# Zain-Jiang/Speech-Editing-Toolkit

Hardware: AMD Instinct MI355X
Metric: diffusion mel-frames/s (100-step p_sample, B=32/GPU, T=800) (higher is better)
Workload: dtype f32 (operands carried as 2 fp16 pieces, 3 MFMA products per term, fp32 accumulate: fp32-equivalent, see roofline.note)

## Files before the change

### speech-editing-toolkit_amd/csrc/common.h

```cpp
#pragma once
#include <hip/hip_runtime.h>
#include <stdint.h>
#include <stdio.h>

#include <atomic>

#include "set_amd.h"

typedef float f32x16 __attribute__((ext_vector_type(16)));
typedef float f32x4 __attribute__((ext_vector_type(4)));

extern thread_local char g_set_err[512];

static inline int set_fail(int code, const char *what, const char *detail) {
    snprintf(g_set_err, sizeof(g_set_err), "%s: %s", what, detail ? detail : "");
    return code;
}
static inline int set_check_launch(const char *what) {
    hipError_t e = hipGetLastError();
    if (e != hipSuccess) return set_fail(SET_E_LAUNCH, what, hipGetErrorString(e));
    return SET_OK;
}
#define SET_REQUIRE(cond, what)                                        \
    do {                                                               \
        if (!(cond)) return set_fail(SET_E_INVALID, what, #cond);      \
    } while (0)
#define SET_HIP(call, what)                                                        \
    do {                                                                           \
        hipError_t e__ = (call);                                                   \
        if (e__ != hipSuccess) return set_fail(SET_E_LAUNCH, what, hipGetErrorString(e__)); \
    } while (0)

struct SetDeviceOnce {
    std::atomic<uint64_t> done{0};
    template <typename F> int run(F &&f) {
        int dev = -1;
        const uint64_t bit = hipGetDevice(&dev) == hipSuccess && dev >= 0 && dev < 64 ? uint64_t(1) << dev : 0;
        if (done.load(std::memory_order_acquire) & bit) return SET_OK;
        const int rc = f();
        if (rc == SET_OK) done.fetch_or(bit, std::memory_order_release);
        return rc;
    }
};
template <typename... K>
static inline int set_lds_optin(SetDeviceOnce &once, int bytes, const char *what, K... kernels) {
    return once.run([&] {
        for (const void *k : {reinterpret_cast<const void *>(kernels)...})
            SET_HIP(hipFuncSetAttribute(k, hipFuncAttributeMaxDynamicSharedMemorySize, bytes), what);
        return SET_OK;
    });
}
static inline hipError_t set_cu_count(int *n_cu) {
    static std::atomic<int> cached[64];
    int dev = 0;
    hipError_t e = hipGetDevice(&dev);
    if (e != hipSuccess) return e;
    const bool slot = dev >= 0 && dev < 64;
    int n = slot ? cached[dev].load(std::memory_order_relaxed) : 0;
    if (n == 0) {
        e = hipDeviceGetAttribute(&n, hipDeviceAttributeMultiprocessorCount, dev);
        if (e != hipSuccess) return e;
        if (slot) cached[dev].store(n, std::memory_order_relaxed);
    }
    *n_cu = n;
    return hipSuccess;
}

const uint64_t *set_seed_delta_ptr();
static __global__ void __launch_bounds__(256) set_zero_words_kernel(unsigned *p, int64_t words) {
    const int64_t i = (int64_t)blockIdx.x * 256 + threadIdx.x;
    if (i < words) p[i] = 0u;
}
static inline bool set_aligned16(const void *a, const void *b, const void *c) {
    return ((reinterpret_cast<uintptr_t>(a) | reinterpret_cast<uintptr_t>(b) | reinterpret_cast<uintptr_t>(c)) & 15) == 0;
}
static inline hipError_t set_zero_async(void *p, size_t bytes, hipStream_t s) {
    const int64_t words = (int64_t)((bytes + 3) / 4);
    hipLaunchKernelGGL(set_zero_words_kernel, dim3((unsigned)((words + 255) / 256)), dim3(256), 0, s, reinterpret_cast<unsigned *>(p), words);
    return hipGetLastError();
}
static inline unsigned set_blocks(int64_t n, int per_block) { return (unsigned)((n + per_block - 1) / per_block); }

__device__ __forceinline__ float dev_softplus(float x) { return x > 20.0f ? x : log1pf(expf(x)); }
__device__ __forceinline__ float dev_sigmoid(float x) { return 1.0f / (1.0f + expf(-x)); }

__device__ __forceinline__ float dev_act(float v, int act, float p) {
    switch (act) {
        case SET_ACT_RELU: return v > 0.0f ? v : 0.0f;
        case SET_ACT_GELU: return 0.5f * v * (1.0f + erff(v * 0.70710678118654752440f));
        case SET_ACT_TANH: return tanhf(v);
        case SET_ACT_SOFTPLUS: return dev_softplus(v);
        case SET_ACT_MISH: return v * tanhf(dev_softplus(v));
        case SET_ACT_LRELU: return v > 0.0f ? v : v * p;
        default: return v;
    }
}
__device__ __forceinline__ float dev_pro(float v, int pro, float p) {
    switch (pro) {
        case SET_PRO_LRELU: return v > 0.0f ? v : v * p;
        case SET_PRO_DIV: return v / p;
        default: return v;
    }
}

__device__ __forceinline__ int mfma32_row(int reg, int lane) { return (reg & 3) + 8 * (reg >> 2) + 4 * (lane >> 5); }
__device__ __forceinline__ f32x16 mfma32(float a, float b, f32x16 c) {
    return __builtin_amdgcn_mfma_f32_32x32x2f32(a, b, c, 0, 0, 0);
}

typedef __amdgpu_buffer_rsrc_t rsrc_t;
__device__ __forceinline__ rsrc_t make_rsrc(const void *p) {
    return __builtin_amdgcn_make_buffer_rsrc(const_cast<void *>(p), (short)0, (int)0x7fffffff, (int)0x00020000);
}
constexpr unsigned BUF_OOB = 0x80000000u;
__device__ __forceinline__ float buf_load(rsrc_t r, unsigned voff, unsigned soff) {
    return __builtin_bit_cast(float, __builtin_amdgcn_raw_buffer_load_b32(r, (int)voff, (int)soff, 0));
}
__device__ __forceinline__ f32x4 buf_load4(rsrc_t r, unsigned voff, unsigned soff) {
    typedef unsigned u32x4 __attribute__((ext_vector_type(4)));
    return __builtin_bit_cast(f32x4, __builtin_amdgcn_raw_buffer_load_b128(r, (int)voff, (int)soff, 0));
}
__device__ __forceinline__ void buf_store4(f32x4 v, rsrc_t r, unsigned voff, unsigned soff) {
    typedef unsigned u32x4 __attribute__((ext_vector_type(4)));
    __builtin_amdgcn_raw_buffer_store_b128(__builtin_bit_cast(u32x4, v), r, (int)voff, (int)soff, 0);
}
__device__ __forceinline__ void buf_store(float v, rsrc_t r, unsigned voff, unsigned soff) {
    __builtin_amdgcn_raw_buffer_store_b32(__builtin_bit_cast(unsigned, v), r, (int)voff, (int)soff, 0);
}
__device__ __forceinline__ f32x4 buf_load4_stream(rsrc_t r, unsigned voff, unsigned soff) {
    typedef unsigned u32x4 __attribute__((ext_vector_type(4)));
    return __builtin_bit_cast(f32x4, __builtin_amdgcn_raw_buffer_load_b128(r, (int)voff, (int)soff, 2));
}
__device__ __forceinline__ void buf_store4_stream(f32x4 v, rsrc_t r, unsigned voff, unsigned soff) {
    typedef unsigned u32x4 __attribute__((ext_vector_type(4)));
    __builtin_amdgcn_raw_buffer_store_b128(__builtin_bit_cast(u32x4, v), r, (int)voff, (int)soff, 16);
}
__device__ __forceinline__ void buf_atomic_add(float v, rsrc_t r, unsigned voff, unsigned soff) {
    (void)__builtin_amdgcn_raw_ptr_buffer_atomic_fadd_f32(v, r, (int)voff, (int)soff, 0);
}
__device__ __forceinline__ void buf_store_agent(float v, rsrc_t r, unsigned voff, unsigned soff) {
    __builtin_amdgcn_raw_buffer_store_b32(__builtin_bit_cast(unsigned, v), r, (int)voff, (int)soff, 16);
}

__device__ __forceinline__ int ld_agent(const int *p) { return __hip_atomic_load(p, __ATOMIC_RELAXED, __HIP_MEMORY_SCOPE_AGENT); }
constexpr unsigned STACK_SPIN_LIMIT = 1u << 22;
constexpr unsigned SPLIT_SPIN_LIMIT = 1u << 20;

__device__ __forceinline__ void split2_f16(float a, float b, unsigned &p0, unsigned &p1) {
    typedef _Float16 h2_t __attribute__((ext_vector_type(2)));
    typedef float f2_t __attribute__((ext_vector_type(2)));
    const f2_t v = {a, b};
    const h2_t h0 = __builtin_convertvector(v, h2_t);
    const h2_t h1 = __builtin_convertvector(v - __builtin_convertvector(h0, f2_t), h2_t);
    p0 = __builtin_bit_cast(unsigned, h0);
    p1 = __builtin_bit_cast(unsigned, h1);
}

template <int RB> struct AVec;
template <> struct AVec<1> { typedef float type; };
template <> struct AVec<2> { typedef float type __attribute__((ext_vector_type(2))); };
template <> struct AVec<4> { typedef float type __attribute__((ext_vector_type(4))); };

template <int RB>
__device__ __forceinline__ float avec_get(const typename AVec<RB>::type &v, int r) {
    if constexpr (RB == 1) return v; else return v[r];
}

template <int RB, int NCB, int GS>
struct KOps {
    typename AVec<RB>::type A[GS];
    float B[GS][NCB];
};

template <int RB, int NCB, int GS, typename Adv>
__device__ __forceinline__ void gemm_groups(f32x16 (&acc)[RB][NCB], const typename AVec<RB>::type *&wp, const float *&bp,
                                            int rstep, int ng, Adv advance) {
    KOps<RB, NCB, GS> P, Q;
    auto load_step = [&](KOps<RB, NCB, GS> &o, int u) {
        o.A[u] = wp[u * 64];
#pragma unroll
        for (int cb = 0; cb < NCB; ++cb) o.B[u][cb] = bp[u * rstep + 32 * cb];
    };
    auto mma_step = [&](const KOps<RB, NCB, GS> &o, int u) {
        __builtin_amdgcn_s_setprio(1);
#pragma unroll
        for (int r = 0; r < RB; ++r)
#pragma unroll
            for (int cb = 0; cb < NCB; ++cb) acc[r][cb] = mfma32(avec_get<RB>(o.A[u], r), o.B[u][cb], acc[r][cb]);
        __builtin_amdgcn_s_setprio(0);
    };
#pragma unroll
    for (int u = 0; u < GS; ++u) load_step(P, u);
    for (int g = 0; g < ng; g += 2) {
        advance(g);
#pragma unroll
        for (int u = 0; u < GS; ++u) {
            load_step(Q, u);
            __builtin_amdgcn_sched_barrier(0);
            mma_step(P, u);
            __builtin_amdgcn_sched_barrier(0);
        }
        if (g + 2 < ng) advance(g + 1);
#pragma unroll
        for (int u = 0; u < GS; ++u) {
            load_step(P, u);
            __builtin_amdgcn_sched_barrier(0);
            mma_step(Q, u);
            __builtin_amdgcn_sched_barrier(0);
        }
    }
}
```

### speech-editing-toolkit_amd/csrc/diffnet.hip

```cpp
#include <stdlib.h>

#include "common.h"
#include "boundary_x2.h"

namespace {

constexpr int DC = 256;
constexpr int NT = 64;
constexpr int KS1 = 3 * DC / 2;
constexpr int KS2 = DC / 2;

__device__ __forceinline__ int urow16(int r) { return (r & 3) + 8 * (r >> 2); }

__device__ __forceinline__ int layer_row(int w, int rb, int i) {
    return (rb < 2 ? 64 * w + 32 * rb : DC + 64 * w + 32 * (rb - 2)) + i;
}

__device__ __forceinline__ float fast_sigmoid(float x) { return __builtin_amdgcn_rcpf(1.0f + __expf(-x)); }
__device__ __forceinline__ float fast_tanh(float x) { return 1.0f - 2.0f * __builtin_amdgcn_rcpf(1.0f + __expf(2.0f * x)); }

struct LayerTile {
    const float *xin;
    float *xout;
    float *skp;
    const float *cpb;
    const float *dstep;
    int64_t d_cs;
    const float *w1p, *b_dil, *w2p, *b_out;
    int T, t0, dil, first;
    uint64_t *dbg;
    int o, nvalid, halo_l, halo_r;
    unsigned x_bs4, cp_bs4;
    float *sy, *sz;
};

__device__ __forceinline__ int wn_pair_q(int p, int d) { return 2 * d * (p / d) + (p % d); }

__device__ __forceinline__ unsigned wn_voff(const LayerTile &a, int q, unsigned slab4) {
    const bool side = q >= a.o;
    return 4u * (unsigned)(a.t0 + q - (side ? a.T : 0)) + (side ? slab4 : 0u);
}

template <int NCB, int GS, bool AGENT = false>
__device__ __forceinline__ void layer_tile(const LayerTile &a, float *smem) {
    constexpr int NTt = 32 * NCB;
    const int tid = threadIdx.x;
    const int lane = tid & 63;
    const int w = __builtin_amdgcn_readfirstlane(tid >> 6);
    const int half = lane >> 5, l31 = lane & 31;
    const int t0 = a.t0;
    const int dil = a.dil;
    const int XW = NTt + 2 * dil;
    const int T = a.T;
    const float *xin = a.xin;
    uint64_t *dbg = a.dbg;
#define PHASE_STAMP(i) \
    if (dbg && tid == 0) dbg[i] = __builtin_amdgcn_s_memtime();
    PHASE_STAMP(0)

    unsigned lo[NCB];
    bool tv[NCB];
#pragma unroll
    for (int cb = 0; cb < NCB; ++cb) {
        lo[cb] = 4u * (unsigned)(4 * half * T + min(t0 + 32 * cb + l31, T - 1));
        tv[cb] = t0 + 32 * cb + l31 < T;
    }
    const unsigned lb = 16u * (unsigned)half;
    const unsigned T4 = 4u * (unsigned)T;
    const rsrc_t rxin = make_rsrc(xin), rskp = make_rsrc(a.skp), rxout = make_rsrc(a.xout), rcp = make_rsrc(a.cpb),
                 rbd = make_rsrc(a.b_dil), rbo = make_rsrc(a.b_out);

    f32x16 acc[4][NCB];
#pragma unroll
    for (int rb = 0; rb < 4; ++rb)
#pragma unroll
        for (int r = 0; r < 16; ++r) {
            const unsigned ur = (unsigned)layer_row(w, rb, urow16(r));
            const float bias = buf_load(rbd, lb, 4u * ur);
#pragma unroll
            for (int cb = 0; cb < NCB; ++cb) acc[rb][cb][r] = bias + buf_load(rcp, lo[cb], ur * T4);
        }
    {
        const int tA = t0 - dil + lane;
        const int tB = t0 - dil + 64 + lane;
        const bool vA = tA >= 0 && tA < T;
        const bool vB = tB >= 0 && tB < T;
        const unsigned cA = 4u * (unsigned)min(max(tA, 0), T - 1), cB = 4u * (unsigned)min(max(tB, 0), T - 1);
        const bool laneA = lane < XW;
        const bool laneB = 64 + lane < XW;
        for (int r0 = 0; r0 < 64; r0 += 16) {
            float xa[16], xb[16], dd[16];
#pragma unroll
            for (int u = 0; u < 16; ++u) {
                const int c = 64 * w + r0 + u;
                xa[u] = buf_load(rxin, cA, (unsigned)c * T4);
                if constexpr (NCB == 2) xb[u] = buf_load(rxin, cB, (unsigned)c * T4);
                dd[u] = a.dstep[(int64_t)c * a.d_cs];
            }
#pragma unroll
            for (int u = 0; u < 16; ++u) {
                const int c = 64 * w + r0 + u;
                if (laneA) smem[c * XW + lane] = vA ? xa[u] + dd[u] : 0.0f;
                if constexpr (NCB == 2) {
                    if (laneB) smem[c * XW + 64 + lane] = vB ? xb[u] + dd[u] : 0.0f;
                }
            }
        }
    }
    __syncthreads();
    PHASE_STAMP(1)

    {
        const f32x4 *wp = reinterpret_cast<const f32x4 *>(a.w1p) + (int64_t)w * KS1 * 64 + lane;
        const float *bp = smem + half * XW + l31;
        const int rstep = 2 * XW;
        constexpr int GPT = 128 / GS;
        gemm_groups<4, NCB, GS>(acc, wp, bp, rstep, KS1 / GS, [&](int g) {
            wp += GS * 64;
            bp += GS * rstep;
            if ((g % GPT) == GPT - 1) bp += dil - 128 * rstep;
        });
    }
    PHASE_STAMP(2)

#pragma unroll
    for (int rb = 0; rb < 2; ++rb)
#pragma unroll
        for (int r = 0; r < 16; ++r)
#pragma unroll
            for (int cb = 0; cb < NCB; ++cb) {
                const float z = fast_sigmoid(acc[rb][cb][r]) * fast_tanh(acc[rb + 2][cb][r]);
                acc[rb][cb][r] = tv[cb] ? z : 0.0f;
            }
    PHASE_STAMP(3)
    __syncthreads();
#pragma unroll
    for (int rb = 0; rb < 2; ++rb)
#pragma unroll
        for (int cb = 0; cb < NCB; ++cb)
#pragma unroll
            for (int r = 0; r < 16; ++r) {
                const int c = 64 * w + 32 * rb + mfma32_row(r, lane);
                smem[c * NTt + cb * 32 + l31] = acc[rb][cb][r];
            }
    __builtin_amdgcn_sched_barrier(0);
    const bool first = a.first != 0;
#pragma unroll
    for (int rb = 0; rb < 4; ++rb) {
#pragma unroll
        for (int r = 0; r < 16; ++r) {
            const unsigned ur = (unsigned)layer_row(w, rb, urow16(r));
            const float bias = buf_load(rbo, lb, 4u * ur);
#pragma unroll
            for (int cb = 0; cb < NCB; ++cb) {
                const float sv = rb < 2 ? buf_load(rxin, lo[cb], ur * T4) : buf_load(rskp, lo[cb], (ur - DC) * T4);
                acc[rb][cb][r] = (rb >= 2 && first) ? bias : bias + sv;
            }
        }
        if (rb == 1) __builtin_amdgcn_sched_barrier(0);
    }
    __syncthreads();
    PHASE_STAMP(4)

    {
        const f32x4 *wp = reinterpret_cast<const f32x4 *>(a.w2p) + (int64_t)w * KS2 * 64 + lane;
        const float *bp = smem + half * NTt + l31;
        constexpr int rstep = 2 * NTt;
        gemm_groups<4, NCB, GS>(acc, wp, bp, rstep, KS2 / GS, [&](int) {
            wp += GS * 64;
            bp += GS * rstep;
        });
    }
    PHASE_STAMP(5)

#pragma unroll
    for (int cb = 0; cb < NCB; ++cb) {
        if (tv[cb]) {
#pragma unroll
            for (int rb = 0; rb < 4; ++rb)
#pragma unroll
                for (int r = 0; r < 16; ++r) {
                    const unsigned ur = (unsigned)layer_row(w, rb, urow16(r));
                    const float v = acc[rb][cb][r] * (rb < 2 ? 0.70710678118654752440f : 1.0f);
                    const unsigned so = rb < 2 ? ur * T4 : (ur - DC) * T4;
                    if constexpr (AGENT) buf_store_agent(v, rb < 2 ? rxout : rskp, lo[cb], so);
                    else buf_store(v, rb < 2 ? rxout : rskp, lo[cb], so);
                }
        }
    }
    PHASE_STAMP(6)
#undef PHASE_STAMP
}

__global__ void __launch_bounds__(256, 2) diffnet_layer_kernel(SetDiffnetLayerArgs a) {
    extern __shared__ __attribute__((aligned(16))) float smem[];
    const int b = blockIdx.y;
    LayerTile lt;
    lt.xin = a.x_in + (int64_t)b * DC * a.T;
    lt.xout = a.x_out + (int64_t)b * DC * a.T;
    lt.skp = a.skip + (int64_t)b * DC * a.T;
    lt.cpb = a.condproj + (int64_t)b * a.cp_bs;
    lt.dstep = a.dstep + (int64_t)b * a.d_bs;
    lt.d_cs = a.d_cs;
    lt.w1p = a.w1p; lt.b_dil = a.b_dil; lt.w2p = a.w2p; lt.b_out = a.b_out;
    lt.T = a.T; lt.t0 = blockIdx.x * NT; lt.dil = a.dil; lt.first = a.first;
    lt.dbg = a.dbg_clock ? a.dbg_clock + ((int64_t)blockIdx.y * gridDim.x + blockIdx.x) * 8 : nullptr;
    layer_tile<2, 4>(lt, smem);
}

constexpr int WN_NT = 64;
constexpr int WN_MAXD = 8;
constexpr int WN_XW = WN_NT + 2 * WN_MAXD;
constexpr int WN_KS = DC / 2;
constexpr int WN_GS = 2;

__device__ __forceinline__ void wino_init(const LayerTile &a, f32x16 (&m)[2][4]) {
    const int lane = threadIdx.x & 63;
    const int w = __builtin_amdgcn_readfirstlane(threadIdx.x >> 6);
    const int half = lane >> 5, l31 = lane & 31;
    const int T = a.T;
    const int qe0 = wn_pair_q(l31, a.dil);
    const int qe = min(qe0, a.nvalid - 1), qo = min(qe0 + a.dil, a.nvalid - 1);
    const unsigned rowh = 16u * (unsigned)half * (unsigned)T;
    const unsigned loe = rowh + wn_voff(a, qe, a.cp_bs4), loo = rowh + wn_voff(a, qo, a.cp_bs4);
    const unsigned lb = 16u * (unsigned)half;
    const rsrc_t rcp = make_rsrc(a.cpb), rb = make_rsrc(a.b_dil);
#pragma unroll
    for (int rf = 0; rf < 2; ++rf) {
        m[rf][1] = (f32x16){0};
        m[rf][2] = (f32x16){0};
#pragma unroll
        for (int r = 0; r < 16; ++r) {
            const unsigned ur = (unsigned)(rf * DC + 32 * w + urow16(r));
            const float bias = buf_load(rb, lb, 4u * ur);
            m[rf][0][r] = bias + buf_load(rcp, loe, 4u * ur * (unsigned)T);
            m[rf][3][r] = -(bias + buf_load(rcp, loo, 4u * ur * (unsigned)T));
        }
    }
}

constexpr int WN_ZS_OFF = DC * WN_XW;

template <bool UNIT_DIL>
__device__ __forceinline__ void wino_main(const LayerTile &a, f32x16 (&m)[2][4], float *smem, uint64_t *ph, int *s_task,
                                          int claimed) {
    typedef float f32x2 __attribute__((ext_vector_type(2)));
    const int tid = threadIdx.x;
#ifdef SET_WINO_PHASES
#define WPH(k) { const uint64_t t_ = __builtin_amdgcn_s_memtime(); ph[k] += t_ - ph[9]; ph[9] = t_; }
#else
#define WPH(k)
#endif
    const int lane = tid & 63;
    const int w = __builtin_amdgcn_readfirstlane(tid >> 6);
    const int half = lane >> 5, l31 = lane & 31;
    const int t0 = a.t0, T = a.T;
    const unsigned T4 = 4u * (unsigned)T;
    float *zs = smem + WN_ZS_OFF;
    constexpr int XW = UNIT_DIL ? WN_NT + 4 : WN_XW;
    const int d = UNIT_DIL ? 1 : a.dil, qe = UNIT_DIL ? 2 * l31 : wn_pair_q(l31, d);
    const bool tve = qe < a.nvalid, tvo = qe + d < a.nvalid;
    const rsrc_t rxin = make_rsrc(a.xin), rskp = make_rsrc(a.skp), rxout = make_rsrc(a.xout);

    {
        const int qA = lane;
        const int qB = lane < d ? lane - d : 64 + lane - d;
        const bool isB = lane < 2 * d;
        const bool vA = qA < a.nvalid;
        const bool vB = isB && (qB < 0 ? (d == 1 ? a.halo_l != 0 : a.t0 + qB >= 0)
                                       : (d == 1 ? a.halo_r != 0 : a.t0 + qB < a.T));
        const unsigned cA = wn_voff(a, min(qA, a.nvalid - 1), a.x_bs4);
        const unsigned cB = vB ? wn_voff(a, qB, a.x_bs4) : cA;
        const int colA = qA + d + (qA >= a.o ? 2 : 0), colB = qB + d + (qB >= a.o ? 2 : 0);
        const bool gap = a.o <= 64;
        for (int r0 = 0; r0 < 32; r0 += 16) {
            float xa[16], xb[16], dd[16];
#pragma unroll
            for (int u = 0; u < 16; ++u) {
                const int c = 32 * w + r0 + u;
                xa[u] = buf_load(rxin, cA, (unsigned)c * T4);
                xb[u] = buf_load(rxin, cB, (unsigned)c * T4);
                dd[u] = a.dstep[(int64_t)c * a.d_cs];
            }
#pragma unroll
            for (int u = 0; u < 16; ++u) {
                const int c = 32 * w + r0 + u;
                smem[c * XW + colA] = vA ? xa[u] + dd[u] : 0.0f;
                if (isB) smem[c * XW + colB] = vB ? xb[u] + dd[u] : 0.0f;
                if (gap && lane >= 32 && lane < 34) smem[c * XW + a.o + lane - 31] = 0.0f;
            }
        }
    }
    __syncthreads();
    WPH(1)

    {
        const rsrc_t rw = make_rsrc(a.w1p);
        const unsigned wv = 32u * (unsigned)lane;
        unsigned ws = (unsigned)w * (WN_KS * 64 * 8 * 4);
        const float *bpf = smem + half * XW + qe + (qe >= a.o ? 2 : 0);
        const f32x2 *bp = reinterpret_cast<const f32x2 *>(bpf);
        struct Ops { f32x4 A[WN_GS][2]; f32x2 D[WN_GS][2]; };
        Ops P, Q;
        auto load_step = [&](Ops &o, int u) {
            o.A[u][0] = buf_load4(rw, wv, ws + (unsigned)u * 2048u);
            o.A[u][1] = buf_load4(rw, wv + 16u, ws + (unsigned)u * 2048u);
            if (UNIT_DIL) {
                o.D[u][0] = bp[u * XW];
                o.D[u][1] = bp[u * XW + 1];
            } else {
                const float *q = bpf + u * 2 * XW;
                o.D[u][0] = (f32x2){q[0], q[d]};
                o.D[u][1] = (f32x2){q[2 * d], q[3 * d]};
            }
        };
        auto mma_step = [&](const Ops &o, int u) {
            const float d0 = o.D[u][0][0], d1 = o.D[u][0][1], d2 = o.D[u][1][0], d3 = o.D[u][1][1];
            const float D1 = d0 - d2, D2 = d1 + d2, D3 = d2 - d1, D4 = d1 - d3;
            __builtin_amdgcn_s_setprio(1);
            m[0][0] = mfma32(o.A[u][0][0], D1, m[0][0]);
            m[0][1] = mfma32(o.A[u][0][1], D2, m[0][1]);
            m[0][2] = mfma32(o.A[u][0][2], D3, m[0][2]);
            m[0][3] = mfma32(o.A[u][0][3], D4, m[0][3]);
            m[1][0] = mfma32(o.A[u][1][0], D1, m[1][0]);
            m[1][1] = mfma32(o.A[u][1][1], D2, m[1][1]);
            m[1][2] = mfma32(o.A[u][1][2], D3, m[1][2]);
            m[1][3] = mfma32(o.A[u][1][3], D4, m[1][3]);
            __builtin_amdgcn_s_setprio(0);
        };
        constexpr int NG = WN_KS / WN_GS;
#pragma unroll
        for (int u = 0; u < WN_GS; ++u) load_step(P, u);
        for (int g = 0; g < NG; g += 2) {
            ws += WN_GS * 2048u;
            bp += WN_GS * XW;
            bpf += WN_GS * 2 * XW;
#pragma unroll
            for (int u = 0; u < WN_GS; ++u) {
                load_step(Q, u);
                __builtin_amdgcn_sched_barrier(0);
                mma_step(P, u);
                __builtin_amdgcn_sched_barrier(0);
            }
            if (g + 2 < NG) { ws += WN_GS * 2048u; bp += WN_GS * XW; bpf += WN_GS * 2 * XW; }
#pragma unroll
            for (int u = 0; u < WN_GS; ++u) {
                load_step(P, u);
                __builtin_amdgcn_sched_barrier(0);
                mma_step(Q, u);
                __builtin_amdgcn_sched_barrier(0);
            }
        }
    }

    WPH(2)
    {
        const bool save = a.sy != nullptr;
        const rsrc_t rsy = make_rsrc(save ? a.sy : a.xin), rsz = make_rsrc(save ? a.sz : a.xin);
        const unsigned rowh_s = 16u * (unsigned)half * (unsigned)T;
        const unsigned se = rowh_s + wn_voff(a, min(qe, a.nvalid - 1), 0u), so_ = rowh_s + wn_voff(a, min(qe + d, a.nvalid - 1), 0u);
#pragma unroll
        for (int r = 0; r < 16; ++r) {
            const float g0 = m[0][0][r] + m[0][1][r] + m[0][2][r], g1 = m[0][1][r] - m[0][2][r] - m[0][3][r];
            const float f0 = m[1][0][r] + m[1][1][r] + m[1][2][r], f1 = m[1][1][r] - m[1][2][r] - m[1][3][r];
            const float z0 = tve ? fast_sigmoid(g0) * fast_tanh(f0) : 0.0f;
            const float z1 = tvo ? fast_sigmoid(g1) * fast_tanh(f1) : 0.0f;
            const int c = 32 * w + mfma32_row(r, lane);
            if (UNIT_DIL) {
                *reinterpret_cast<f32x2 *>(zs + c * WN_NT + qe) = (f32x2){z0, z1};
            } else {
                zs[c * WN_NT + qe] = z0;
                zs[c * WN_NT + qe + d] = z1;
            }
            if (save) {
                const unsigned ur = (unsigned)(32 * w + urow16(r));
                if (tve) {
                    buf_store(g0, rsy, se, ur * T4);
                    buf_store(f0, rsy, se, (ur + DC) * T4);
                    buf_store(z0, rsz, se, ur * T4);
                }
                if (tvo) {
                    buf_store(g1, rsy, so_, ur * T4);
                    buf_store(f1, rsy, so_, (ur + DC) * T4);
                    buf_store(z1, rsz, so_, ur * T4);
                }
            }
        }
    }
    __builtin_amdgcn_sched_barrier(0);

    const unsigned rowh = 16u * (unsigned)half * (unsigned)T;
    const unsigned lo0 = rowh + wn_voff(a, min(l31, a.nvalid - 1), a.x_bs4), lo1 = rowh + wn_voff(a, min(32 + l31, a.nvalid - 1), a.x_bs4);
    const bool tv0 = l31 < a.nvalid, tv1 = 32 + l31 < a.nvalid;
    const bool first = a.first != 0;
    f32x16 prev[2][2];
#pragma unroll
    for (int rb = 0; rb < 2; ++rb)
#pragma unroll
        for (int r = 0; r < 16; ++r) {
            const unsigned ur = (unsigned)(32 * w + urow16(r));
            prev[rb][0][r] = buf_load(rb == 0 ? rxin : rskp, lo0, ur * T4);
            prev[rb][1][r] = buf_load(rb == 0 ? rxin : rskp, lo1, ur * T4);
        }
    __builtin_amdgcn_sched_barrier(0);

    f32x16 acc[2][2];
    {
        const rsrc_t rbo = make_rsrc(a.b_out);
#pragma unroll
        for (int rb = 0; rb < 2; ++rb)
#pragma unroll
            for (int r = 0; r < 16; ++r) {
                const float bias = buf_load(rbo, 16u * (unsigned)half, 4u * (unsigned)(rb * DC + 32 * w + urow16(r)));
                acc[rb][0][r] = bias;
                acc[rb][1][r] = bias;
            }
    }
    if (tid == 0) s_task[0] = claimed;
    __syncthreads();
    WPH(3)
    {
        const AVec<2>::type *wp = reinterpret_cast<const AVec<2>::type *>(a.w2p) + (int64_t)w * WN_KS * 64 + lane;
        const float *bp = zs + half * WN_NT + l31;
        constexpr int rstep = 2 * WN_NT;
        gemm_groups<2, 2, 8>(acc, wp, bp, rstep, WN_KS / 8, [&](int) {
            wp += 8 * 64;
            bp += 8 * rstep;
        });
    }
    WPH(4)
#pragma unroll
    for (int cb = 0; cb < 2; ++cb) {
        if (cb == 0 ? tv0 : tv1) {
            const unsigned so = cb == 0 ? lo0 : lo1;
#pragma unroll
            for (int rb = 0; rb < 2; ++rb)
#pragma unroll
                for (int r = 0; r < 16; ++r) {
                    const unsigned ur = (unsigned)(32 * w + urow16(r));
                    const float v = (rb == 1 && first) ? acc[rb][cb][r] : acc[rb][cb][r] + prev[rb][cb][r];
                    buf_store_agent(v * (rb == 0 ? 0.70710678118654752440f : 1.0f), rb == 0 ? rxout : rskp, so, ur * T4);
                }
        }
    }
    WPH(5)
#undef WPH
}

template <int NCB, int GS, int WPS>
__global__ void __launch_bounds__(256, WPS) diffnet_stack_kernel(SetDiffnetStackArgs a, int tiles_per_utt, int ntiles,
                                                                int ntasks, int task_slot) {
    constexpr int NTt = 32 * NCB;
    extern __shared__ __attribute__((aligned(16))) float smem[];
    int *s_task = reinterpret_cast<int *>(smem + task_slot);
    int *counter = a.sync_ws, *abort_flag = a.sync_ws + 1, *done = a.sync_ws + 4;
    const int tid = threadIdx.x;
    uint64_t wait_ticks = 0, fence_ticks = 0;
    for (;;) {
        __syncthreads();
        if (tid == 0) {
            const uint64_t tw0 = __builtin_amdgcn_s_memtime();
            int n = atomicAdd(counter, 1);
            if (n < ntasks && n >= ntiles) {
                const int l = n / ntiles, i = n - l * ntiles, j = i % tiles_per_utt;
                unsigned spins = 0;
                const int *f0 = done + i, *fl = done + (j > 0 ? i - 1 : i), *fr = done + (j < tiles_per_utt - 1 ? i + 1 : i);
                for (;;) {
                    const int v0 = ld_agent(f0), v1 = ld_agent(fl), v2 = ld_agent(fr);
                    if (min(v0, min(v1, v2)) >= l) break;
                    __builtin_amdgcn_s_sleep(8);
                    if (++spins > STACK_SPIN_LIMIT || ld_agent(abort_flag) != 0) {
                        __hip_atomic_store(abort_flag, 1, __ATOMIC_RELAXED, __HIP_MEMORY_SCOPE_AGENT);
                        if (a.err_flag) __hip_atomic_store(a.err_flag, 1, __ATOMIC_RELAXED, __HIP_MEMORY_SCOPE_AGENT);
                        n = ntasks;
                        break;
                    }
                }
                __builtin_amdgcn_fence(__ATOMIC_ACQUIRE, "agent");
            }
            wait_ticks += __builtin_amdgcn_s_memtime() - tw0;
            *s_task = n;
        }
        __syncthreads();
        const int n = __builtin_amdgcn_readfirstlane(*s_task);
        if (n >= ntasks) {
            if (tid == 0) {
                atomicAdd(a.sync_ws + 2, (int)(wait_ticks >> 10));
                atomicAdd(a.sync_ws + 3, (int)(fence_ticks >> 10));
            }
            break;
        }
        const int l = n / ntiles, i = n - l * ntiles;
        const int b = i / tiles_per_utt, j = i - b * tiles_per_utt;
        LayerTile lt;
        const float *xi = (l & 1) ? a.xb : a.xa;
        float *xo = (l & 1) ? a.xa : a.xb;
        lt.xin = xi + (int64_t)b * DC * a.T;
        lt.xout = xo + (int64_t)b * DC * a.T;
        lt.skp = a.skip + (int64_t)b * DC * a.T;
        lt.cpb = a.condproj + (int64_t)l * a.cp_ls + (int64_t)b * a.cp_bs;
        lt.dstep = a.dstep + (int64_t)l * a.d_ls + (int64_t)b * a.d_bs;
        lt.d_cs = a.d_cs;
        lt.w1p = a.w1p_all + (int64_t)l * (512 * 768);
        lt.w2p = a.w2p_all + (int64_t)l * (512 * 256);
        lt.b_dil = a.b_dil_all + (int64_t)l * 512;
        lt.b_out = a.b_out_all + (int64_t)l * 512;
        lt.T = a.T; lt.t0 = j * NTt; lt.dil = 1 << (l % a.dilation_cycle_length); lt.first = (l == 0);
        lt.dbg = nullptr;
        layer_tile<NCB, GS, true>(lt, smem);
        asm volatile("s_waitcnt vmcnt(0)" ::: "memory");
        __syncthreads();
        if (tid == 0) {
            const uint64_t tf0 = __builtin_amdgcn_s_memtime();
            __hip_atomic_store(done + i, l + 1, __ATOMIC_RELAXED, __HIP_MEMORY_SCOPE_AGENT);
            fence_ticks += __builtin_amdgcn_s_memtime() - tf0;
        }
    }
}

constexpr int SP_XW = 32 + 2 * WN_MAXD;
constexpr int SP_LDS_FLOATS = DC * SP_XW + 64 * 32 + 4;

__device__ __forceinline__ void split_preload(float (&A)[64], const float *wp) {
#pragma unroll
    for (int u = 0; u < 64; ++u) A[u] = wp[u * 64];
}

template <int KS>
__device__ __forceinline__ void split_gemm(f32x16 &acc, const float *wp, float (&Ap)[64], const float *bq, int rstep,
                                           int tap_jump) {
    static_assert(KS % 128 == 0, "two 64-k-step sets per iteration");
    float Aq[64], Bv[8];
#pragma unroll
    for (int u = 0; u < 4; ++u) {
        Bv[u] = *bq;
        bq += rstep;
    }
    for (int g = 0; g < KS / 64; g += 2) {
        const float *wq = wp + (int64_t)(g + 1) * 64 * 64;
#pragma unroll
        for (int u = 0; u < 64; ++u) {
            Aq[u] = wq[u * 64];
            Bv[(u + 4) & 7] = *bq;
            bq += rstep;
            __builtin_amdgcn_sched_barrier(0);
            acc = mfma32(Ap[u], Bv[u & 7], acc);
            __builtin_amdgcn_sched_barrier(0);
        }
        const float *wn = wp + (int64_t)(g + 2 < KS / 64 ? g + 2 : g) * 64 * 64;
#pragma unroll
        for (int u = 0; u < 64; ++u) {
            Ap[u] = wn[u * 64];
            Bv[(u + 4) & 7] = *bq;
            bq += rstep;
            if (u == 59) bq += tap_jump;
            __builtin_amdgcn_sched_barrier(0);
            acc = mfma32(Aq[u], Bv[u & 7], acc);
            __builtin_amdgcn_sched_barrier(0);
        }
    }
}

__device__ uint64_t *g_split_phase_buf = nullptr;

__device__ __forceinline__ bool split_wait(const int *f0, const int *f1, const int *f2, int want, int *abort_flag,
                                           int *err_flag) {
    unsigned spins = 0;
    for (;;) {
        const int v0 = ld_agent(f0), v1 = ld_agent(f1), v2 = ld_agent(f2);
        if (min(v0, min(v1, v2)) >= want) break;
        __builtin_amdgcn_s_sleep(1);
        if (++spins > SPLIT_SPIN_LIMIT || ld_agent(abort_flag) != 0) {
            __hip_atomic_store(abort_flag, 1, __ATOMIC_RELAXED, __HIP_MEMORY_SCOPE_AGENT);
            if (err_flag) __hip_atomic_store(err_flag, 1, __ATOMIC_RELAXED, __HIP_MEMORY_SCOPE_AGENT);
            return false;
        }
    }
    __builtin_amdgcn_fence(__ATOMIC_ACQUIRE, "agent");
    return true;
}

__global__ void __launch_bounds__(256, 2) diffnet_stack_split_kernel(SetDiffnetStackArgs a, int tiles_per_utt, int ntiles,
                                                                    int fault_tile) {
    extern __shared__ __attribute__((aligned(16))) float smem[];
    float *gs = smem + DC * SP_XW;
    int *s_ok = reinterpret_cast<int *>(gs + 64 * 32);
    int *abort_flag = a.sync_ws + 1, *ready = a.sync_ws + 4, *zcnt = a.sync_ws + 4 + ntiles;
    const int tid = threadIdx.x, lane = tid & 63, half = lane >> 5, l31 = lane & 31;
    const int j = __builtin_amdgcn_readfirstlane(tid >> 6);
    const int i = blockIdx.x >> 2, h = blockIdx.x & 3;
    const int b = i / tiles_per_utt, jt = i - b * tiles_per_utt;
    const int T = a.T, t0 = jt * 32;
    const int il = jt > 0 ? i - 1 : i, ir = jt < tiles_per_utt - 1 ? i + 1 : i;
    const unsigned T4 = 4u * (unsigned)T;
    const unsigned lo = 4u * (unsigned)(4 * half * T + min(t0 + l31, T - 1));
    const bool tv = t0 + l31 < T;
    const unsigned lb = 16u * (unsigned)half;
    const rsrc_t rz = make_rsrc(a.z_ws + (int64_t)i * (DC * 32));
    const rsrc_t rskp = make_rsrc(a.skip + (int64_t)b * DC * T);
    const int vr = 4 * h + j;
    uint64_t *dbg = (blockIdx.x == 5 && tid == 0) ? g_split_phase_buf : nullptr;
    uint64_t tprev = dbg ? __builtin_amdgcn_s_memtime() : 0;
#define SP_PHASE(p)                                           \
    if (dbg) {                                                \
        const uint64_t tn = __builtin_amdgcn_s_memtime();     \
        dbg[p] += tn - tprev;                                 \
        tprev = tn;                                           \
    }
    for (int l = 0; l < a.L; ++l) {
        const int dil = 1 << (l % a.dilation_cycle_length), XW = 32 + 2 * dil;
        const rsrc_t rxin = make_rsrc(((l & 1) ? a.xb : a.xa) + (int64_t)b * DC * T);
        const rsrc_t rxout = make_rsrc(((l & 1) ? a.xa : a.xb) + (int64_t)b * DC * T);
        const rsrc_t rcp = make_rsrc(a.condproj + (int64_t)l * a.cp_ls + (int64_t)b * a.cp_bs);
        const rsrc_t rbd = make_rsrc(a.b_dil_all + (int64_t)l * 512), rbo = make_rsrc(a.b_out_all + (int64_t)l * 512);
        const float *dstep = a.dstep + (int64_t)l * a.d_ls + (int64_t)b * a.d_bs;
        f32x16 acc[1][1];
#pragma unroll
        for (int r = 0; r < 16; ++r) {
            const unsigned ur = (unsigned)layer_row(h, j, urow16(r));
            acc[0][0][r] = buf_load(rbd, lb, 4u * ur) + buf_load(rcp, lo, ur * T4);
        }
        float Ap[64];
        const float *wp1 = a.w1s_all + (int64_t)l * (512 * 768) + (int64_t)vr * KS1 * 64 + lane;
        split_preload(Ap, wp1);
        if (tid == 0) *s_ok = (l == 0 || split_wait(ready + i, ready + il, ready + ir, 4 * l, abort_flag, a.err_flag)) ? 1 : 0;
        __syncthreads();
        if (__builtin_amdgcn_readfirstlane(*s_ok) == 0) return;
        SP_PHASE(0)
        {
            const int tA = t0 - dil + lane;
            const bool vA = tA >= 0 && tA < T, laneA = lane < XW;
            const unsigned cA = 4u * (unsigned)min(max(tA, 0), T - 1);
            float xa[64];
            const float dv = dstep[(int64_t)(64 * j + lane) * a.d_cs];
#pragma unroll
            for (int u = 0; u < 64; ++u) xa[u] = buf_load(rxin, cA, (unsigned)(64 * j + u) * T4);
#pragma unroll
            for (int u = 0; u < 64; ++u) {
                const float dd = __builtin_bit_cast(float, __builtin_amdgcn_readlane(__builtin_bit_cast(int, dv), u));
                if (laneA) smem[(64 * j + u) * XW + lane] = vA ? xa[u] + dd : 0.0f;
            }
        }
        __syncthreads();
        SP_PHASE(1)
        split_gemm<KS1>(acc[0][0], wp1, Ap, smem + half * XW + l31, 2 * XW, dil - 128 * 2 * XW);
        SP_PHASE(2)
        if (j >= 2) {
#pragma unroll
            for (int r = 0; r < 16; ++r) gs[(32 * (j - 2) + mfma32_row(r, lane)) * 32 + l31] = fast_tanh(acc[0][0][r]);
        }
        __syncthreads();
        if (j < 2) {
#pragma unroll
            for (int r = 0; r < 16; ++r) {
                const float z = fast_sigmoid(acc[0][0][r]) * gs[(32 * j + mfma32_row(r, lane)) * 32 + l31];
                buf_store_agent(tv ? z : 0.0f, rz, 4u * (unsigned)(4 * half * 32 + l31),
                                4u * 32u * (unsigned)(64 * h + 32 * j + urow16(r)));
            }
        }
        asm volatile("s_waitcnt vmcnt(0)" ::: "memory");
        __syncthreads();
        if (tid == 0) __hip_atomic_fetch_add(zcnt + i, 1, __ATOMIC_RELAXED, __HIP_MEMORY_SCOPE_AGENT);
        SP_PHASE(3)
        {
            const rsrc_t rsv = make_rsrc(j < 2 ? ((l & 1) ? a.xb : a.xa) + (int64_t)b * DC * T : a.skip + (int64_t)b * DC * T);
            float bias[16], sv[16];
#pragma unroll
            for (int r = 0; r < 16; ++r) {
                bias[r] = buf_load(rbo, lb, 4u * (unsigned)layer_row(h, j, urow16(r)));
                sv[r] = buf_load(rsv, lo, (unsigned)(64 * h + 32 * (j & 1) + urow16(r)) * T4);
            }
            if (j >= 2 && l == 0) {
#pragma unroll
                for (int r = 0; r < 16; ++r) acc[0][0][r] = bias[r];
            } else {
#pragma unroll
                for (int r = 0; r < 16; ++r) acc[0][0][r] = bias[r] + sv[r];
            }
        }
        const float *wp2 = a.w2s_all + (int64_t)l * (512 * 256) + (int64_t)vr * KS2 * 64 + lane;
        split_preload(Ap, wp2);
        if (tid == 0) *s_ok = split_wait(zcnt + i, zcnt + i, zcnt + i, 4 * (l + 1), abort_flag, a.err_flag) ? 1 : 0;
        __syncthreads();
        if (__builtin_amdgcn_readfirstlane(*s_ok) == 0) return;
        SP_PHASE(4)
        {
            f32x4 zv[8];
#pragma unroll
            for (int k = 0; k < 8; ++k) zv[k] = buf_load4(rz, 16u * (unsigned)tid, 4096u * (unsigned)k);
#pragma unroll
            for (int k = 0; k < 8; ++k) *reinterpret_cast<f32x4 *>(smem + 4 * tid + 1024 * k) = zv[k];
        }
        __syncthreads();
        SP_PHASE(5)
        split_gemm<KS2>(acc[0][0], wp2, Ap, smem + half * 32 + l31, 64, 0);
        SP_PHASE(6)
        if (tv && j < 2) {
#pragma unroll
            for (int r = 0; r < 16; ++r)
                buf_store_agent(acc[0][0][r] * 0.70710678118654752440f, rxout, lo, (unsigned)layer_row(h, j, urow16(r)) * T4);
        } else if (tv) {
#pragma unroll
            for (int r = 0; r < 16; ++r)
                buf_store(acc[0][0][r], rskp, lo, (unsigned)(layer_row(h, j, urow16(r)) - DC) * T4);
        }
        asm volatile("s_waitcnt vmcnt(0)" ::: "memory");
        __syncthreads();
        if (tid == 0 && !(l == 0 && i == fault_tile && h == 0))
            __hip_atomic_fetch_add(ready + i, 1, __ATOMIC_RELAXED, __HIP_MEMORY_SCOPE_AGENT);
        SP_PHASE(7)
    }
#undef SP_PHASE
}

template <bool UNIT_DIL>
__global__ void __launch_bounds__(512, 2) diffnet_stack_wino_kernel(SetDiffnetStackArgs a, int tiles_per_utt, int ntiles,
                                                                    int ntasks, int concat, int fault_tile) {
    extern __shared__ __attribute__((aligned(16))) float smem[];
    int *s_task = reinterpret_cast<int *>(smem + WN_ZS_OFF + DC * WN_NT);
    int *counter = a.sync_ws, *abort_flag = a.sync_ws + 1, *done = a.sync_ws + 4;
    const int tid = threadIdx.x;
    uint64_t wait_ticks = 0, fence_ticks = 0;
    if (tid == 0) s_task[0] = atomicAdd(counter, 1);
    __syncthreads();
    int n = __builtin_amdgcn_readfirstlane(s_task[0]);
    int l = 0, i = 0, j = 0;
    LayerTile lt;
    auto decode = [&](int task) {
        l = task / ntiles;
        i = task - l * ntiles;
        int b;
        if (concat) {
            const int64_t f0 = (int64_t)WN_NT * i, F = (int64_t)a.B * a.T;
            b = (int)(f0 / a.T);
            j = i;
            lt.t0 = (int)(f0 - (int64_t)b * a.T);
            lt.o = (a.T - lt.t0 <= WN_NT && b + 1 < a.B) ? a.T - lt.t0 : (1 << 20);
            lt.nvalid = (int)min((int64_t)WN_NT, (b + 1 < a.B ? F : (int64_t)(b + 1) * a.T) - f0);
            lt.halo_l = lt.t0 > 0;
            lt.halo_r = f0 + WN_NT < F;
        } else {
            b = i / tiles_per_utt;
            j = i - b * tiles_per_utt;
            lt.t0 = j * WN_NT;
            lt.o = 1 << 20;
            lt.nvalid = min(WN_NT, a.T - lt.t0);
            lt.halo_l = lt.t0 > 0;
            lt.halo_r = lt.t0 + WN_NT < a.T;
        }
        lt.x_bs4 = 4u * (unsigned)DC * (unsigned)a.T;
        lt.cp_bs4 = 4u * (unsigned)a.cp_bs;
        const int64_t slab = (int64_t)a.B * DC * a.T;
        const float *xi = a.x_all ? a.x_all + l * slab : ((l & 1) ? a.xb : a.xa);
        float *xo = a.x_all ? a.x_all + (l + 1) * slab : ((l & 1) ? a.xa : a.xb);
        lt.xin = xi + (int64_t)b * DC * a.T;
        lt.xout = xo + (int64_t)b * DC * a.T;
        lt.skp = a.skip + (int64_t)b * DC * a.T;
        lt.sy = a.save_y ? a.save_y + 2 * l * slab + (int64_t)b * 2 * DC * a.T : nullptr;
        lt.sz = a.save_z ? a.save_z + l * slab + (int64_t)b * DC * a.T : nullptr;
        lt.cpb = a.condproj + (int64_t)l * a.cp_ls + (int64_t)b * a.cp_bs;
        lt.dstep = a.dstep + (int64_t)l * a.d_ls + (int64_t)b * a.d_bs;
        lt.d_cs = a.d_cs;
        lt.w1p = a.w1w_all + (int64_t)l * (512 * 256 * 4);
        lt.w2p = a.w2w_all + (int64_t)l * (512 * 256);
        lt.b_dil = a.b_dil_all + (int64_t)l * 512;
        lt.b_out = a.b_out_all + (int64_t)l * 512;
        lt.T = a.T; lt.dil = UNIT_DIL ? 1 : 1 << (l % a.dilation_cycle_length); lt.first = (l == 0);
        lt.dbg = nullptr;
    };
#ifdef SET_WINO_PHASES
    uint64_t ph[10] = {0, 0, 0, 0, 0, 0, 0, 0, 0, 0};
    ph[9] = __builtin_amdgcn_s_memtime();
#else
    uint64_t *ph = nullptr;
#endif
    int i_done = -1, l_done = 0;
    auto publish = [&]() {
        asm volatile("s_waitcnt vmcnt(0)" ::: "memory");
#ifdef SET_WINO_PHASES
        { const uint64_t t_ = __builtin_amdgcn_s_memtime(); ph[0] += t_ - ph[9]; ph[9] = t_; }
#endif
        __syncthreads();
#ifdef SET_WINO_PHASES
        { const uint64_t t_ = __builtin_amdgcn_s_memtime(); ph[6] += t_ - ph[9]; ph[9] = t_; }
#endif
        if (tid == 0 && i_done >= 0) {
            const uint64_t tf0 = __builtin_amdgcn_s_memtime();
            if (!(l_done == 0 && i_done == fault_tile))
                __hip_atomic_store(done + i_done, l_done + 1, __ATOMIC_RELAXED, __HIP_MEMORY_SCOPE_AGENT);
            fence_ticks += __builtin_amdgcn_s_memtime() - tf0;
        }
    };
    while (n < ntasks) {
        decode(n);
        f32x16 m[2][4];
        wino_init(lt, m);
        __builtin_amdgcn_sched_barrier(0);
        publish();
        int claimed = 0;
        if (tid == 0) {
            int ok_all = 1;
            if (l > 0) {
                const uint64_t tw0 = __builtin_amdgcn_s_memtime();
                unsigned spins = 0;
                const int *f0 = done + i, *fl = done + (j > 0 ? i - 1 : i), *fr = done + (j < tiles_per_utt - 1 ? i + 1 : i);
                for (;;) {
                    const int v0 = ld_agent(f0), v1 = ld_agent(fl), v2 = ld_agent(fr);
                    if (min(v0, min(v1, v2)) >= l) break;
                    __builtin_amdgcn_s_sleep(8);
                    if (++spins > STACK_SPIN_LIMIT || ld_agent(abort_flag) != 0) {
                        __hip_atomic_store(abort_flag, 1, __ATOMIC_RELAXED, __HIP_MEMORY_SCOPE_AGENT);
                        if (a.err_flag) __hip_atomic_store(a.err_flag, 1, __ATOMIC_RELAXED, __HIP_MEMORY_SCOPE_AGENT);
                        ok_all = 0;
                        break;
                    }
                }
                __builtin_amdgcn_fence(__ATOMIC_ACQUIRE, "agent");
                wait_ticks += __builtin_amdgcn_s_memtime() - tw0;
            }
            s_task[1] = ok_all;
            claimed = atomicAdd(counter, 1);
        }
        __syncthreads();
        if (__builtin_amdgcn_readfirstlane(s_task[1]) == 0) {
            i_done = -1;
            break;
        }
#ifdef SET_WINO_PHASES
        { const uint64_t t_ = __builtin_amdgcn_s_memtime(); ph[8] += t_ - ph[9]; ph[9] = t_; }
#endif
        wino_main<UNIT_DIL>(lt, m, smem, ph, s_task, claimed);
        i_done = i;
        l_done = l;
        n = __builtin_amdgcn_readfirstlane(s_task[0]);
    }
    publish();
#ifdef SET_WINO_PHASES
    if (tid == 0)
        for (int k = 0; k < 9; ++k) atomicAdd(a.sync_ws + 4 + ntiles + k, (int)(ph[k] >> 10));
#endif
    if (tid == 0) {
        atomicAdd(a.sync_ws + 2, (int)(wait_ticks >> 10));
        atomicAdd(a.sync_ws + 3, (int)(fence_ticks >> 10));
    }
}

__global__ void __launch_bounds__(256) pack_diffnet_layer_kernel(const float *w_dil, const float *w_out, float *w1p,
                                                                 float *w2p, int64_t wd_ls = 0, int64_t wo_ls = 0) {
    const int64_t idx = (int64_t)blockIdx.x * 256 + threadIdx.x;
    const int64_t n1 = (int64_t)4 * KS1 * 64 * 4, n2 = (int64_t)4 * KS2 * 64 * 4;
    w_dil += (int64_t)blockIdx.y * wd_ls;
    w_out += (int64_t)blockIdx.y * wo_ls;
    w1p += (int64_t)blockIdx.y * n1;
    w2p += (int64_t)blockIdx.y * n2;
    if (idx < n1) {
        const int rb = (int)(idx & 3), lane = (int)((idx >> 2) & 63);
        const int ks = (int)((idx >> 8) % KS1), w = (int)((idx >> 8) / KS1);
        const int tap = ks >> 7, cp = ks & 127;
        const int row = layer_row(w, rb, lane & 31), c = 2 * cp + (lane >> 5);
        w1p[idx] = w_dil[((int64_t)row * DC + c) * 3 + tap];
    } else if (idx < n1 + n2) {
        const int64_t j = idx - n1;
        const int rb = (int)(j & 3), lane = (int)((j >> 2) & 63);
        const int ks = (int)((j >> 8) % KS2), w = (int)((j >> 8) / KS2);
        const int row = layer_row(w, rb, lane & 31), c = 2 * ks + (lane >> 5);
        w2p[j] = w_out[(int64_t)row * DC + c];
    }
}

__global__ void __launch_bounds__(256) pack_diffnet_wino_kernel(const float *w_dil, const float *w_out, float *w1w,
                                                                float *w2w, int64_t wd_ls = 0, int64_t wo_ls = 0) {
    const int64_t idx = (int64_t)blockIdx.x * 256 + threadIdx.x;
    const int64_t n1 = (int64_t)8 * WN_KS * 64 * 8, n2 = (int64_t)8 * WN_KS * 64 * 2;
    w_dil += (int64_t)blockIdx.y * wd_ls;
    w_out += (int64_t)blockIdx.y * wo_ls;
    w1w += (int64_t)blockIdx.y * n1;
    w2w += (int64_t)blockIdx.y * n2;
    if (idx < n1) {
        const int e = (int)(idx & 7), lane = (int)((idx >> 3) & 63);
        const int ks = (int)((idx >> 9) % WN_KS), w = (int)((idx >> 9) / WN_KS);
        const int rf = e >> 2, p = e & 3;
        const int row = rf * DC + 32 * w + (lane & 31), c = 2 * ks + (lane >> 5);
        const float *g = w_dil + ((int64_t)row * DC + c) * 3;
        const double g0 = g[0], g1 = g[1], g2 = g[2];
        const double v = p == 0 ? g0 : (p == 1 ? 0.5 * (g0 + g1 + g2) : (p == 2 ? 0.5 * (g0 - g1 + g2) : g2));
        w1w[idx] = (float)v;
    } else if (idx < n1 + n2) {
        const int64_t j = idx - n1;
        const int rb = (int)(j & 1), lane = (int)((j >> 1) & 63);
        const int ks = (int)((j >> 7) % WN_KS), w = (int)((j >> 7) / WN_KS);
        const int row = rb * DC + 32 * w + (lane & 31), c = 2 * ks + (lane >> 5);
        w2w[j] = w_out[(int64_t)row * DC + c];
    }
}

}

extern "C" int64_t set_diffnet_w1w_size(void) { return (int64_t)512 * 256 * 4; }
extern "C" int set_pack_diffnet_layer_wino(const float *w_dil, const float *w_out, float *w1w, float *w2w, void *stream) {
    SET_REQUIRE(w_dil && w_out && w1w && w2w, "set_pack_diffnet_layer_wino");
    const int64_t total = set_diffnet_w1w_size() + (int64_t)512 * 256;
    hipLaunchKernelGGL(pack_diffnet_wino_kernel, dim3(set_blocks(total, 256)), dim3(256), 0, (hipStream_t)stream, w_dil,
                       w_out, w1w, w2w);
    return set_check_launch("set_pack_diffnet_layer_wino");
}

extern "C" int64_t set_diffnet_w1p_size(void) { return (int64_t)512 * 768; }
extern "C" int64_t set_diffnet_w2p_size(void) { return (int64_t)512 * 256; }

extern "C" int set_pack_diffnet_layers(const float *w_dil, const float *w_out, int64_t wd_ls, int64_t wo_ls, float *w1p, float *w2p,
                                       float *w1w, float *w2w, int32_t L, void *stream) {
    SET_REQUIRE(w_dil && w_out && w1p && w2p && L > 0 && L <= 65535 && (w1w == nullptr) == (w2w == nullptr), "set_pack_diffnet_layers");
    SET_REQUIRE((int64_t)8 * WN_KS * 64 * 8 == set_diffnet_w1w_size() && (int64_t)8 * WN_KS * 64 * 2 == (int64_t)512 * 256 &&
                    (int64_t)4 * KS1 * 64 * 4 == set_diffnet_w1p_size() && (int64_t)4 * KS2 * 64 * 4 == set_diffnet_w2p_size(),
                "set_pack_diffnet_layers(image sizes)");
    const int64_t total = set_diffnet_w1p_size() + set_diffnet_w2p_size();
    hipLaunchKernelGGL(pack_diffnet_layer_kernel, dim3(set_blocks(total, 256), L), dim3(256), 0, (hipStream_t)stream, w_dil, w_out, w1p,
                       w2p, wd_ls, wo_ls);
    int rc = set_check_launch("set_pack_diffnet_layers");
    if (rc != SET_OK || w1w == nullptr) return rc;
    const int64_t totw = set_diffnet_w1w_size() + (int64_t)512 * 256;
    hipLaunchKernelGGL(pack_diffnet_wino_kernel, dim3(set_blocks(totw, 256), L), dim3(256), 0, (hipStream_t)stream, w_dil, w_out, w1w,
                       w2w, wd_ls, wo_ls);
    return set_check_launch("set_pack_diffnet_layers(wino)");
}
extern "C" int set_pack_diffnet_layer(const float *w_dil, const float *w_out, float *w1p, float *w2p, void *stream) {
    SET_REQUIRE(w_dil && w_out && w1p && w2p, "set_pack_diffnet_layer");
    const int64_t total = set_diffnet_w1p_size() + set_diffnet_w2p_size();
    hipLaunchKernelGGL(pack_diffnet_layer_kernel, dim3(set_blocks(total, 256)), dim3(256), 0, (hipStream_t)stream,
                       w_dil, w_out, w1p, w2p);
    return set_check_launch("set_pack_diffnet_layer");
}

extern "C" int set_diffnet_layer(const SetDiffnetLayerArgs *args, void *stream) {
    SET_REQUIRE(args != nullptr, "set_diffnet_layer");
    const SetDiffnetLayerArgs &a = *args;
    SET_REQUIRE(a.x_in && a.condproj && a.dstep && a.w1p && a.b_dil && a.w2p && a.b_out && a.x_out && a.skip,
                "set_diffnet_layer");
    SET_REQUIRE(a.B > 0 && a.T > 0 && a.dil >= 1, "set_diffnet_layer");
    SET_REQUIRE(a.x_in != a.x_out, "set_diffnet_layer(x_in must not alias x_out)");
    if (a.dil > 8) return set_fail(SET_E_UNSUPPORTED, "set_diffnet_layer", "dilation > 8 (LDS tile > 80 KiB)");
    const size_t lds = (size_t)DC * (NT + 2 * a.dil) * sizeof(float);
    static SetDeviceOnce lds_once;
    if (int rc = set_lds_optin(lds_once, 96 * 1024, "set_diffnet_layer(attr)", diffnet_layer_kernel)) return rc;
    dim3 grid((a.T + NT - 1) / NT, a.B);
    hipLaunchKernelGGL(diffnet_layer_kernel, grid, dim3(256), lds, (hipStream_t)stream, a);
    return set_check_launch("set_diffnet_layer");
}

extern "C" int set_debug_split_phase_buffer(uint64_t *buf) {
    SET_HIP(hipMemcpyToSymbol(HIP_SYMBOL(g_split_phase_buf), &buf, sizeof(buf)), "set_debug_split_phase_buffer");
    return SET_OK;
}

extern "C" int64_t set_sizeof_diffnet_stack_args(void) { return (int64_t)sizeof(SetDiffnetStackArgs); }

static bool split_f32_pinned() {
    const char *e = getenv("SET_AMD_SPLIT_F32");
    return e && atoi(e) != 0;
}
static int x3_mode_of_images(int images) { return (images & 4) ? 3 : ((images & 8) ? 2 : 0); }

static int stack_variant(int B, int T, int dcl, bool have_wino, bool have_split, int x3_mode, int n_cu) {
    const bool have_x3 = x3_mode == 2 || x3_mode == 3;
    const int64_t tiles64 = (int64_t)B * ((T + 63) / 64);
    const int64_t split_blocks = 4 * (int64_t)B * ((T + 31) / 32);
    const bool split_one_per_cu = have_x3 && !split_f32_pinned();
    const bool split_fits = have_split && dcl <= 4 && split_blocks <= (split_one_per_cu ? 1 : 2) * (int64_t)n_cu;
    const bool split_pays = split_blocks <= (int64_t)(have_x3 ? 1 : 2) * n_cu;
    int split_env = 1;
    if (const char *e = getenv("SET_AMD_SPLIT")) split_env = atoi(e);
    if (split_fits && (split_env == 2 || (split_env == 1 && !getenv("SET_AMD_WINO") && split_pays))) return 3;
    int x3_env = 1;
    if (const char *e = getenv("SET_AMD_X3")) x3_env = atoi(e);
    if (have_x3 && dcl <= 4 && (x3_env == 2 || (x3_env == 1 && !getenv("SET_AMD_WINO") && tiles64 >= 8)))
        return x3_mode == 3 ? 4 : 5;
    int ncb = tiles64 < 3 * n_cu ? 1 : 2;
    if (const char *e = getenv("SET_AMD_STACK_NCB")) ncb = atoi(e) == 2 ? 2 : 1;
    const bool wino_ok = have_wino && (1 << (dcl - 1)) <= WN_MAXD;
    bool wino = wino_ok && 25 * tiles64 >= 17 * n_cu;
    if (const char *e = getenv("SET_AMD_WINO")) wino = wino_ok && (atoi(e) == 2 || (wino && atoi(e) != 0));
    return wino ? 2 : (ncb == 1 ? 1 : 0);
}
extern "C" int set_diffnet_stack_variant(int B, int T, int dilation_cycle_length, int images) {
    int n_cu = 256;
    (void)set_cu_count(&n_cu);
    return stack_variant(B, T, dilation_cycle_length, (images & 1) != 0, (images & 2) != 0, x3_mode_of_images(images), n_cu);
}

int set_launch_diffnet_stack_x3(const SetDiffnetStackArgs &a, int n_cu, int fault_tile, hipStream_t s);
int set_x3_winograd_selected(int x3_mode, int B, int T, int dilation_cycle_length, int n_cu);
extern "C" int set_diffnet_stack_x3_winograd(int B, int T, int dilation_cycle_length, int images) {
    int n_cu = 256;
    (void)set_cu_count(&n_cu);
    const int x3_mode = x3_mode_of_images(images);
    if (stack_variant(B, T, dilation_cycle_length, (images & 1) != 0, (images & 2) != 0, x3_mode, n_cu) != 5) return 0;
    return set_x3_winograd_selected(x3_mode, B, T, dilation_cycle_length, n_cu);
}
int set_launch_diffnet_stack_split_x2(const SetDiffnetStackArgs &a, int fault_tile, hipStream_t s);

extern "C" int set_diffnet_stack(const SetDiffnetStackArgs *args, void *stream) {
    SET_REQUIRE(args != nullptr, "set_diffnet_stack");
    const SetDiffnetStackArgs &a = *args;
    SET_REQUIRE(a.xa && a.xb && a.skip && a.condproj && a.dstep && a.w1p_all && a.w2p_all && a.b_dil_all &&
                    a.b_out_all && a.sync_ws,
                "set_diffnet_stack");
    SET_REQUIRE(a.B > 0 && a.T > 0 && a.L > 0 && a.dilation_cycle_length >= 1 && a.dilation_cycle_length <= 4,
                "set_diffnet_stack");
    hipStream_t s = (hipStream_t)stream;
    static SetDeviceOnce lds_once;
    if (int rc = set_lds_optin(lds_once, 150 * 1024, "set_diffnet_stack(attr)", diffnet_stack_kernel<1, 8, 2>, diffnet_stack_kernel<2, 4, 2>,
                               diffnet_stack_wino_kernel<true>, diffnet_stack_wino_kernel<false>, diffnet_stack_split_kernel))
        return rc;
    int n_cu = 0;
    SET_HIP(set_cu_count(&n_cu), "set_diffnet_stack");
    const bool plain = !a.x_all && !a.save_y && !a.save_z;
    const int variant = stack_variant(a.B, a.T, a.dilation_cycle_length, a.w1w_all && a.w2w_all,
                                      a.w1s_all && a.w2s_all && a.z_ws && plain, (a.wx3_all && plain) ? a.x3_mode : 0, n_cu);
    int fault_tile = -1;
    if (const char *e = getenv("SET_AMD_FAULT_TILE")) fault_tile = atoi(e);
    if (variant >= 4) return set_launch_diffnet_stack_x3(a, n_cu, fault_tile, s);
    if (variant == 3 && a.wx3_all && a.x3_mode == 2 && !split_f32_pinned())
        return set_launch_diffnet_stack_split_x2(a, fault_tile, s);
    if (variant == 3) {
        const int tiles = (a.T + 31) / 32, nt = a.B * tiles;
        SET_HIP(set_zero_async(a.sync_ws, (size_t)(4 + 2 * nt) * sizeof(int32_t), s), "set_diffnet_stack(memset)");
        hipLaunchKernelGGL(diffnet_stack_split_kernel, dim3(4 * nt), dim3(256), (size_t)SP_LDS_FLOATS * sizeof(float), s, a,
                           tiles, nt, fault_tile);
        return set_check_launch("set_diffnet_stack");
    }
    const bool wino = variant == 2;
    const int ncb = variant == 1 ? 1 : 2;
    const int ntt = 32 * ncb;
    int tiles_per_utt = (a.T + ntt - 1) / ntt;
    int ntiles = a.B * tiles_per_utt;
    bool concat = wino && a.dilation_cycle_length == 1 && a.T % 2 == 0 && a.T >= WN_NT &&
                  (int64_t)a.cp_bs * 4 < (1ll << 31) && a.d_bs == 0 && !a.save_y && !a.save_z;
    if (concat) {
        ntiles = (int)(((int64_t)a.B * a.T + WN_NT - 1) / WN_NT);
        tiles_per_utt = ntiles;
    }
    const int64_t ntasks64 = (int64_t)ntiles * a.L;
    SET_REQUIRE(ntasks64 < (1ll << 30), "set_diffnet_stack(task count)");
    const int max_dil = 1 << (a.dilation_cycle_length - 1);
    const int task_slot = DC * (ntt + 2 * max_dil);
    const size_t lds = (size_t)(task_slot + 4) * sizeof(float);
    SET_HIP(set_zero_async(a.sync_ws, (size_t)(4 + ntiles + (wino ? 12 : 0)) * sizeof(int32_t), s),
            "set_diffnet_stack(memset)");
    const int wps = wino ? 1 : 2;
    int grid = wps * n_cu;
    if (grid > ntiles * 4 / 5) grid = ntiles * 4 / 5;
    if (grid < n_cu) grid = n_cu < ntiles ? n_cu : ntiles;
    if (const char *e = getenv("SET_AMD_STACK_GRID")) grid = atoi(e) > 0 ? atoi(e) : grid;
    if ((int64_t)grid > ntasks64) grid = (int)ntasks64;
    if (grid < 1) grid = 1;
    if (wino) {
        if (a.dilation_cycle_length == 1)
            hipLaunchKernelGGL(diffnet_stack_wino_kernel<true>, dim3(grid), dim3(512),
                               (size_t)(WN_ZS_OFF + DC * WN_NT + 4) * sizeof(float), s, a, tiles_per_utt, ntiles,
                               (int)ntasks64, concat ? 1 : 0, fault_tile);
        else
            hipLaunchKernelGGL(diffnet_stack_wino_kernel<false>, dim3(grid), dim3(512),
                               (size_t)(WN_ZS_OFF + DC * WN_NT + 4) * sizeof(float), s, a, tiles_per_utt, ntiles,
                               (int)ntasks64, 0, fault_tile);
    } else if (ncb == 1)
        hipLaunchKernelGGL((diffnet_stack_kernel<1, 8, 2>), dim3(grid), dim3(256), lds, s, a, tiles_per_utt, ntiles,
                           (int)ntasks64, task_slot);
    else
        hipLaunchKernelGGL((diffnet_stack_kernel<2, 4, 2>), dim3(grid), dim3(256), lds, s, a, tiles_per_utt, ntiles,
                           (int)ntasks64, task_slot);
    return set_check_launch("set_diffnet_stack");
}

namespace {
__global__ void __launch_bounds__(256) gate_kernel(const float *y, float *z, int B, int C, int T) {
    const int64_t i = (int64_t)blockIdx.x * 256 + threadIdx.x;
    if (i >= (int64_t)B * C * T) return;
    const int64_t ct = i % ((int64_t)C * T);
    const int64_t b = i / ((int64_t)C * T);
    const float *yb = y + b * 2 * C * T;
    z[i] = dev_sigmoid(yb[ct]) * tanhf(yb[(int64_t)C * T + ct]);
}
__global__ void __launch_bounds__(256) res_skip_kernel(const float *x_in, const float *o, float *x_out, float *skip,
                                                       int B, int C, int T, int first) {
    const int64_t i = (int64_t)blockIdx.x * 256 + threadIdx.x;
    if (i >= (int64_t)B * C * T) return;
    const int64_t ct = i % ((int64_t)C * T);
    const int64_t b = i / ((int64_t)C * T);
    const float *ob = o + b * 2 * C * T;
    x_out[i] = (x_in[i] + ob[ct]) / 1.41421356237309504880f;
    const float s = ob[(int64_t)C * T + ct];
    skip[i] = first ? s : skip[i] + s;
}
__global__ void __launch_bounds__(256) sinusoid_kernel(const float *t, float *out, int dim, int n) {
    const int64_t i = (int64_t)blockIdx.x * 256 + threadIdx.x;
    if (i >= (int64_t)dim * n) return;
    const int j = (int)(i / n), k = (int)(i % n);
    const int half = dim / 2;
    const int jj = j < half ? j : j - half;
    const float e = (float)(9.210340371976184 / (double)(half - 1));
    const float freq = expf((float)jj * -e);
    const float ang = t[k] * freq;
    out[i] = j < half ? sinf(ang) : cosf(ang);
}


__global__ void __launch_bounds__(256) randn_kernel(float *out, int64_t n, uint64_t seed, uint64_t offset, const uint64_t *seed_delta) {
    const int64_t q = (int64_t)blockIdx.x * 256 + threadIdx.x;
    if (q * 4 >= n) return;
    if (seed_delta) seed += *seed_delta;
    float z[4];
    randn4(seed, offset + (uint64_t)q, z);
#pragma unroll
    for (int k = 0; k < 4; ++k)
        if (q * 4 + k < n) out[q * 4 + k] = z[k];
}

__global__ void __launch_bounds__(256) posterior_kernel(const float *x0, const float *x_t, const float *eps,
                                                        const float *coef4, int64_t coef_bs, float *x_prev,
                                                        int64_t per_batch, int64_t n, uint64_t seed,
                                                        uint64_t offset, const uint64_t *seed_delta) {
    const int64_t q = (int64_t)blockIdx.x * 256 + threadIdx.x;
    if (q * 4 >= n) return;
    if (seed_delta) seed += *seed_delta;
    float z[4];
    if (!eps) randn4(seed, offset + (uint64_t)q, z);
#pragma unroll
    for (int k = 0; k < 4; ++k) {
        const int64_t i = q * 4 + k;
        if (i >= n) break;
        const float *cf = coef4 + (i / per_batch) * coef_bs;
        const float mean = cf[0] * x0[i] + cf[1] * x_t[i];
        const float e = eps ? eps[i] : z[k];
        x_prev[i] = mean + cf[3] * expf(0.5f * cf[2]) * e;
    }
}

__global__ void __launch_bounds__(256) q_sample_kernel(const float *x_start, const float *eps, const float *ab2,
                                                       const float *nonpad, float *x_t, int B, int M, int T) {
    const int64_t i = (int64_t)blockIdx.x * 256 + threadIdx.x;
    if (i >= (int64_t)B * M * T) return;
    const int t = (int)(i % T);
    const int b = (int)(i / ((int64_t)M * T));
    float v = ab2[2 * b] * x_start[i] + ab2[2 * b + 1] * eps[i];
    if (nonpad) v *= nonpad[(int64_t)b * T + t];
    x_t[i] = v;
}

__global__ void __launch_bounds__(64) selftest_mfma_kernel(float *max_err) {
    constexpr int K = 8;
    const int lane = threadIdx.x;
    auto Af = [](int i, int k) { return 0.25f * (float)((i * 7 + k * 3) % 11) - 1.0f; };
    auto Bf = [](int k, int j) { return 0.125f * (float)((k * 5 + j * 13) % 17) - 0.75f; };
    f32x16 acc = {0};
    for (int k0 = 0; k0 < K; k0 += 2) {
        const int k = k0 + (lane >> 5);
        acc = mfma32(Af(lane & 31, k), Bf(k, lane & 31), acc);
    }
    float err = 0.0f;
    for (int r = 0; r < 16; ++r) {
        const int row = mfma32_row(r, lane), col = lane & 31;
        float ref = 0.0f;
        for (int k = 0; k < K; ++k) ref = fmaf(Af(row, k), Bf(k, col), ref);
        err = fmaxf(err, fabsf(ref - acc[r]));
    }
    for (int off = 32; off > 0; off >>= 1) err = fmaxf(err, __shfl_xor(err, off));
    if (lane == 0) *max_err = err;
}
}

extern "C" int set_gate(const float *y, float *z, int32_t B, int32_t C, int32_t T, void *stream) {
    SET_REQUIRE(y && z && B > 0 && C > 0 && T > 0, "set_gate");
    hipLaunchKernelGGL(gate_kernel, dim3(set_blocks((int64_t)B * C * T, 256)), dim3(256), 0, (hipStream_t)stream, y, z,
                       B, C, T);
    return set_check_launch("set_gate");
}
extern "C" int set_res_skip(const float *x_in, const float *o, float *x_out, float *skip, int32_t B, int32_t C,
                            int32_t T, int32_t first, void *stream) {
    SET_REQUIRE(x_in && o && x_out && skip && B > 0 && C > 0 && T > 0, "set_res_skip");
    hipLaunchKernelGGL(res_skip_kernel, dim3(set_blocks((int64_t)B * C * T, 256)), dim3(256), 0, (hipStream_t)stream,
                       x_in, o, x_out, skip, B, C, T, first);
    return set_check_launch("set_res_skip");
}
extern "C" int set_sinusoid_embed(const float *t, float *out, int32_t dim, int32_t n, void *stream) {
    SET_REQUIRE(t && out && dim >= 4 && (dim % 2) == 0 && n > 0, "set_sinusoid_embed");
    hipLaunchKernelGGL(sinusoid_kernel, dim3(set_blocks((int64_t)dim * n, 256)), dim3(256), 0, (hipStream_t)stream, t,
                       out, dim, n);
    return set_check_launch("set_sinusoid_embed");
}
static const uint64_t *g_seed_delta = nullptr;
const uint64_t *set_seed_delta_ptr() { return g_seed_delta; }
extern "C" int set_rng_seed_delta(const uint64_t *dev_word) {
    g_seed_delta = dev_word;
    return SET_OK;
}

extern "C" int set_randn(float *out, int64_t n, uint64_t seed, uint64_t offset, void *stream) {
    SET_REQUIRE(out && n > 0, "set_randn");
    hipLaunchKernelGGL(randn_kernel, dim3(set_blocks((n + 3) / 4, 256)), dim3(256), 0, (hipStream_t)stream, out, n,
                       seed, offset, g_seed_delta);
    return set_check_launch("set_randn");
}
extern "C" int set_posterior_step(const float *x0, const float *x_t, const float *eps, const float *coef4,
                                  int64_t coef_bs, float *x_prev, int32_t B, int64_t per_batch, uint64_t seed,
                                  uint64_t offset, void *stream) {
    SET_REQUIRE(x0 && x_t && coef4 && x_prev && B > 0 && per_batch > 0, "set_posterior_step");
    const int64_t n = (int64_t)B * per_batch;
    hipLaunchKernelGGL(posterior_kernel, dim3(set_blocks((n + 3) / 4, 256)), dim3(256), 0, (hipStream_t)stream, x0,
                       x_t, eps, coef4, coef_bs, x_prev, per_batch, n, seed, offset, g_seed_delta);
    return set_check_launch("set_posterior_step");
}
extern "C" int set_q_sample(const float *x_start, const float *eps, const float *ab2, const float *nonpad, float *x_t,
                            int32_t B, int32_t M, int32_t T, void *stream) {
    SET_REQUIRE(x_start && eps && ab2 && x_t && B > 0 && M > 0 && T > 0, "set_q_sample");
    hipLaunchKernelGGL(q_sample_kernel, dim3(set_blocks((int64_t)B * M * T, 256)), dim3(256), 0, (hipStream_t)stream,
                       x_start, eps, ab2, nonpad, x_t, B, M, T);
    return set_check_launch("set_q_sample");
}
extern "C" int set_selftest_mfma(float *max_err_host, void *stream) {
    SET_REQUIRE(max_err_host != nullptr, "set_selftest_mfma");
    float *d = nullptr;
    SET_HIP(hipMalloc(&d, sizeof(float)), "set_selftest_mfma");
    hipLaunchKernelGGL(selftest_mfma_kernel, dim3(1), dim3(64), 0, (hipStream_t)stream, d);
    int rc = set_check_launch("set_selftest_mfma");
    if (rc == SET_OK) {
        hipError_t e = hipMemcpyAsync(max_err_host, d, sizeof(float), hipMemcpyDeviceToHost, (hipStream_t)stream);
        if (e == hipSuccess) e = hipStreamSynchronize((hipStream_t)stream);
        if (e != hipSuccess) rc = set_fail(SET_E_LAUNCH, "set_selftest_mfma", hipGetErrorString(e));
    }
    (void)hipFree(d);
    return rc;
}

struct BoundaryArgs {
    const float *skip;
    float *x;
    const float *eps;
    const float *coef4;
    const float *w_skip_p, *b_skip, *w_outp_p, *b_outp, *w_in_p, *b_in;
    float *xin_next;
    float inv_div;
    float div;
    uint64_t seed, quad_offset;
    int T, M, MP;
};
constexpr int BD_LD = 64;

__global__ void __launch_bounds__(256, 2) diffnet_boundary_kernel(BoundaryArgs a) {
    extern __shared__ __attribute__((aligned(16))) float smem[];
    const int tid = threadIdx.x, lane = tid & 63;
    const int w = __builtin_amdgcn_readfirstlane(tid >> 6);
    const int half = lane >> 5, l31 = lane & 31;
    const int b = blockIdx.y, t0 = blockIdx.x * 64, T = a.T, M = a.M;
    {
        const rsrc_t rs = make_rsrc(a.skip + (int64_t)b * DC * T);
        const unsigned vo = 4u * (unsigned)min(t0 + lane, T - 1);
        const bool tv = t0 + lane < T;
        for (int r0 = 0; r0 < 64; r0 += 16) {
            float v[16];
#pragma unroll
            for (int u = 0; u < 16; ++u) v[u] = buf_load(rs, vo, 4u * (unsigned)(64 * w + r0 + u) * (unsigned)T);
#pragma unroll
            for (int u = 0; u < 16; ++u) smem[(64 * w + r0 + u) * BD_LD + lane] = tv ? v[u] / a.div : 0.0f;
        }
    }
    __syncthreads();
    f32x16 acc[2][1][2];
#pragma unroll
    for (int i = 0; i < 2; ++i) {
        acc[i][0][0] = (f32x16){0};
        acc[i][0][1] = (f32x16){0};
        const float *wp = a.w_skip_p + (int64_t)(2 * w + i) * (DC / 2) * 64 + lane;
        const float *bp = smem + half * BD_LD + l31;
        gemm_groups<1, 2, 8>(acc[i], wp, bp, 2 * BD_LD, (DC / 2) / 8, [&](int) {
            wp += 8 * 64;
            bp += 8 * 2 * BD_LD;
        });
    }
    __syncthreads();
#pragma unroll
    for (int i = 0; i < 2; ++i)
#pragma unroll
        for (int r = 0; r < 16; ++r) {
            const int row = 32 * (2 * w + i) + mfma32_row(r, lane);
            const float bias = a.b_skip[row];
#pragma unroll
            for (int cb = 0; cb < 2; ++cb) smem[row * BD_LD + 32 * cb + l31] = fmaxf(acc[i][0][cb][r] + bias, 0.0f);
        }
    __syncthreads();
    const int rbn = (M + 31) / 32;
    f32x16 xo[1][2];
    xo[0][0] = (f32x16){0};
    xo[0][1] = (f32x16){0};
    if (w < rbn) {
        const float *wp = a.w_outp_p + (int64_t)w * (DC / 2) * 64 + lane;
        const float *bp = smem + half * BD_LD + l31;
        gemm_groups<1, 2, 8>(xo, wp, bp, 2 * BD_LD, (DC / 2) / 8, [&](int) {
            wp += 8 * 64;
            bp += 8 * 2 * BD_LD;
        });
    }
    __syncthreads();
    if (w < rbn) {
#pragma unroll
        for (int r = 0; r < 16; ++r) {
            const int row = 32 * w + mfma32_row(r, lane);
            const float bias = a.b_outp[min(row, M - 1)];
#pragma unroll
            for (int cb = 0; cb < 2; ++cb) smem[row * BD_LD + 32 * cb + l31] = row < M ? xo[0][cb][r] + bias : 0.0f;
        }
    }
    __syncthreads();
    {
        const float c1 = a.coef4[0], c2 = a.coef4[1], sig = a.coef4[3] * expf(0.5f * a.coef4[2]);
        float *xb = a.x + (int64_t)b * M * T;
        const float *eb = a.eps ? a.eps + (int64_t)b * M * T : nullptr;
        for (int qi = tid; qi < a.MP * 16; qi += 256) {
            const int m = qi >> 4, tq = qi & 15, t = t0 + 4 * tq;
            float *cell = smem + m * BD_LD + 4 * tq;
            if (m < M && t < T) {
                const int64_t i = (int64_t)m * T + t;
                const f32x4 xt = *reinterpret_cast<const f32x4 *>(xb + i);
                float z[4];
                if (eb) {
                    const f32x4 e4 = *reinterpret_cast<const f32x4 *>(eb + i);
                    z[0] = e4[0]; z[1] = e4[1]; z[2] = e4[2]; z[3] = e4[3];
                } else {
                    randn4(a.seed, a.quad_offset + (uint64_t)(((int64_t)b * M * T + i) >> 2), z);
                }
                f32x4 o;
#pragma unroll
                for (int k = 0; k < 4; ++k) {
                    const float mean = c1 * cell[k] + c2 * xt[k];
                    o[k] = mean + sig * z[k];
                }
                *reinterpret_cast<f32x4 *>(xb + i) = o;
                *reinterpret_cast<f32x4 *>(cell) = o;
            } else {
                *reinterpret_cast<f32x4 *>(cell) = (f32x4){0.0f, 0.0f, 0.0f, 0.0f};
            }
        }
    }
    if (!a.xin_next) return;
    __syncthreads();
#pragma unroll
    for (int i = 0; i < 2; ++i) {
        acc[i][0][0] = (f32x16){0};
        acc[i][0][1] = (f32x16){0};
        const float *wp = a.w_in_p + (int64_t)(2 * w + i) * (a.MP / 2) * 64 + lane;
        const float *bp = smem + half * BD_LD + l31;
        gemm_groups<1, 2, 4>(acc[i], wp, bp, 2 * BD_LD, (a.MP / 2) / 4, [&](int) {
            wp += 4 * 64;
            bp += 4 * 2 * BD_LD;
        });
    }
    const rsrc_t ro = make_rsrc(a.xin_next + (int64_t)b * DC * T);
    float bin[2][16];
#pragma unroll
    for (int i = 0; i < 2; ++i)
#pragma unroll
        for (int r = 0; r < 16; ++r) bin[i][r] = (a.b_in + 32 * (2 * w + i) + urow16(r))[4 * half];
#pragma unroll
    for (int cb = 0; cb < 2; ++cb) {
        if (t0 + 32 * cb + l31 < T) {
            const unsigned so = 4u * (unsigned)(4 * half * T + t0 + 32 * cb + l31);
#pragma unroll
            for (int i = 0; i < 2; ++i)
#pragma unroll
                for (int r = 0; r < 16; ++r) {
                    const int ur = 32 * (2 * w + i) + urow16(r);
                    buf_store(fmaxf(acc[i][0][cb][r] + bin[i][r], 0.0f), ro, so, 4u * (unsigned)ur * (unsigned)T);
                }
        }
    }
}

struct BoundaryX2Args {
    BoundaryArgs g;
    const unsigned short *w_skip_x2, *w_outp_x2, *w_in_x2;
    int32_t *err_flag;
};

__global__ void __launch_bounds__(256, 2) diffnet_boundary_x2_kernel(BoundaryX2Args ax) {
    const BoundaryArgs &a = ax.g;
    extern __shared__ __attribute__((aligned(16))) unsigned char bl[];
    const int tid = threadIdx.x, lane = tid & 63;
    const int w = __builtin_amdgcn_readfirstlane(tid >> 6);
    const int half = lane >> 5, l31 = lane & 31;
    const int b = blockIdx.y, t0 = blockIdx.x * 64, T = a.T, M = a.M;
    const unsigned lane16 = 16u * (unsigned)lane;
    const unsigned T4 = 4u * (unsigned)T;
    float amax = 0.0f;
    {
        const int f = lane, cg = w;
        const rsrc_t rs = make_rsrc(a.skip + (int64_t)b * DC * T);
        const unsigned vo = 4u * (unsigned)min(t0 + f, T - 1);
        const bool tv = t0 + f < T;
        for (int c0 = 0; c0 < 64; c0 += 16) {
            float v[16];
#pragma unroll
            for (int u = 0; u < 16; ++u) v[u] = buf_load(rs, vo, (unsigned)(64 * cg + c0 + u) * T4);
#pragma unroll
            for (int q8 = 0; q8 < 2; ++q8) {
                bx_u32x4 u0, u1;
#pragma unroll
                for (int e = 0; e < 4; ++e) {
                    unsigned short p0[2], p1[2];
#pragma unroll
                    for (int k = 0; k < 2; ++k) {
                        const float sv = v[8 * q8 + 2 * e + k] / a.div;
                        const float x = tv ? sv : 0.0f;
                        amax = fmaxf(amax, fabsf(x));
                        bx_split(x, p0[k], p1[k]);
                    }
                    u0[e] = (unsigned)p0[0] | ((unsigned)p0[1] << 16);
                    u1[e] = (unsigned)p1[0] | ((unsigned)p1[1] << 16);
                }
                *reinterpret_cast<bx_u32x4 *>(bl + f * BX_XR + (64 * cg + c0 + 8 * q8) * 2) = u0;
                *reinterpret_cast<bx_u32x4 *>(bl + BX_PIECE + f * BX_XR + (64 * cg + c0 + 8 * q8) * 2) = u1;
            }
        }
    }
    __syncthreads();
    auto bfrag256 = [&](int ks, int cb) { return (unsigned)((cb * 32 + l31) * BX_XR + (ks * 16 + half * 8) * 2); };
    {
        const rsrc_t rw = make_rsrc(ax.w_skip_x2);
        const float inv = reinterpret_cast<const float *>(ax.w_skip_x2 + (DC / 32) * (DC / 16) * 1024)[1];
        f32x16 acc[2][2];
#pragma unroll
        for (int i = 0; i < 2; ++i)
#pragma unroll
            for (int cb = 0; cb < 2; ++cb) acc[i][cb] = (f32x16){0};
        bx_gemm<2>(acc, rw, lane16, 2 * w, DC / 16, DC / 16, bl, BX_PIECE, bfrag256);
        __syncthreads();
#pragma unroll
        for (int i = 0; i < 2; ++i)
#pragma unroll
            for (int cb = 0; cb < 2; ++cb)
#pragma unroll
                for (int g = 0; g < 4; ++g) {
                    unsigned short p0[4], p1[4];
#pragma unroll
                    for (int e = 0; e < 4; ++e) {
                        const int row = 32 * (2 * w + i) + 8 * g + 4 * half + e;
                        const float h = fmaxf(acc[i][cb][4 * g + e] * inv + a.b_skip[row], 0.0f);
                        amax = fmaxf(amax, h);
                        bx_split(h, p0[e], p1[e]);
                    }
                    const unsigned off = (unsigned)((cb * 32 + l31) * BX_XR + (32 * (2 * w + i) + 8 * g + 4 * half) * 2);
                    bx_u32x2 u;
                    u[0] = (unsigned)p0[0] | ((unsigned)p0[1] << 16); u[1] = (unsigned)p0[2] | ((unsigned)p0[3] << 16);
                    *reinterpret_cast<bx_u32x2 *>(bl + off) = u;
                    u[0] = (unsigned)p1[0] | ((unsigned)p1[1] << 16); u[1] = (unsigned)p1[2] | ((unsigned)p1[3] << 16);
                    *reinterpret_cast<bx_u32x2 *>(bl + BX_PIECE + off) = u;
                }
    }
    __syncthreads();
    float *xs = reinterpret_cast<float *>(bl);
    {
        const int rbn = (M + 31) / 32;
        f32x16 xo[1][2];
        xo[0][0] = (f32x16){0};
        xo[0][1] = (f32x16){0};
        const float inv = reinterpret_cast<const float *>(ax.w_outp_x2 + ((M + 31) / 32) * (DC / 16) * 1024)[1];
        if (w < rbn) bx_gemm<1>(xo, make_rsrc(ax.w_outp_x2), lane16, w, DC / 16, DC / 16, bl, BX_PIECE, bfrag256);
        __syncthreads();
        if (w < 3) {
#pragma unroll
            for (int r = 0; r < 16; ++r) {
                const int row = 32 * w + mfma32_row(r, lane);
                const float bias = a.b_outp[min(row, M - 1)];
#pragma unroll
                for (int cb = 0; cb < 2; ++cb) xs[row * 64 + 32 * cb + l31] = (w < rbn && row < M) ? xo[0][cb][r] * inv + bias : 0.0f;
            }
        }
    }
    __syncthreads();
    {
        const float c1 = a.coef4[0], c2 = a.coef4[1], sig = a.coef4[3] * expf(0.5f * a.coef4[2]);
        float *xb = a.x + (int64_t)b * M * T;
        const float *eb = a.eps ? a.eps + (int64_t)b * M * T : nullptr;
        for (int qi = tid; qi < 96 * 16; qi += 256) {
            const int m = qi >> 4, tq = qi & 15, t = t0 + 4 * tq;
            float *cell = xs + m * 64 + 4 * tq;
            if (m < M && t < T) {
                const int64_t i = (int64_t)m * T + t;
                const f32x4 xt = *reinterpret_cast<const f32x4 *>(xb + i);
                float z[4];
                if (eb) {
                    const f32x4 e4 = *reinterpret_cast<const f32x4 *>(eb + i);
                    z[0] = e4[0]; z[1] = e4[1]; z[2] = e4[2]; z[3] = e4[3];
                } else {
                    randn4(a.seed, a.quad_offset + (uint64_t)(((int64_t)b * M * T + i) >> 2), z);
                }
                f32x4 o;
#pragma unroll
                for (int k = 0; k < 4; ++k) {
                    const float mean = c1 * cell[k] + c2 * xt[k];
                    o[k] = mean + sig * z[k];
                }
                *reinterpret_cast<f32x4 *>(xb + i) = o;
                *reinterpret_cast<f32x4 *>(cell) = o;
            } else {
                *reinterpret_cast<f32x4 *>(cell) = (f32x4){0.0f, 0.0f, 0.0f, 0.0f};
            }
        }
    }
    if (!a.xin_next) {
        if (!(amax < 32768.0f) && ax.err_flag) __hip_atomic_store(ax.err_flag, 2, __ATOMIC_RELAXED, __HIP_MEMORY_SCOPE_AGENT);
        return;
    }
    __syncthreads();
    unsigned char *xp = bl + BX_PIECE;
    constexpr unsigned XP_PIECE = 64 * BX_PR;
    {
        const int f = lane, cg = w;
#pragma unroll
        for (int q8 = 0; q8 < 3; ++q8) {
            bx_u32x4 u0, u1;
#pragma unroll
            for (int e = 0; e < 4; ++e) {
                unsigned short p0[2], p1[2];
#pragma unroll
                for (int k = 0; k < 2; ++k) {
                    const float x = xs[(24 * cg + 8 * q8 + 2 * e + k) * 64 + f];
                    amax = fmaxf(amax, fabsf(x));
                    bx_split(x, p0[k], p1[k]);
                }
                u0[e] = (unsigned)p0[0] | ((unsigned)p0[1] << 16);
                u1[e] = (unsigned)p1[0] | ((unsigned)p1[1] << 16);
            }
            *reinterpret_cast<bx_u32x4 *>(xp + f * BX_PR + (24 * cg + 8 * q8) * 2) = u0;
            *reinterpret_cast<bx_u32x4 *>(xp + XP_PIECE + f * BX_PR + (24 * cg + 8 * q8) * 2) = u1;
        }
    }
    if (!(amax < 32768.0f) && ax.err_flag) __hip_atomic_store(ax.err_flag, 2, __ATOMIC_RELAXED, __HIP_MEMORY_SCOPE_AGENT);
    __syncthreads();
    {
        const int ngin = ((M + 31) / 32) * 2;
        const float inv = reinterpret_cast<const float *>(ax.w_in_x2 + (DC / 32) * ngin * 1024)[1];
        f32x16 acc[2][2];
#pragma unroll
        for (int i = 0; i < 2; ++i)
#pragma unroll
            for (int cb = 0; cb < 2; ++cb) acc[i][cb] = (f32x16){0};
        bx_gemm<2>(acc, make_rsrc(ax.w_in_x2), lane16, 2 * w, ngin, ngin, xp, XP_PIECE,
                   [&](int ks, int cb) { return (unsigned)((cb * 32 + l31) * BX_PR + (ks * 16 + half * 8) * 2); });
        const rsrc_t ro = make_rsrc(a.xin_next + (int64_t)b * DC * T);
        float bin[2][16];
#pragma unroll
        for (int i = 0; i < 2; ++i)
#pragma unroll
            for (int r = 0; r < 16; ++r) bin[i][r] = (a.b_in + 32 * (2 * w + i) + urow16(r))[4 * half];
#pragma unroll
        for (int cb = 0; cb < 2; ++cb) {
            if (t0 + 32 * cb + l31 < T) {
                const unsigned so = 4u * (unsigned)(4 * half * T + t0 + 32 * cb + l31);
#pragma unroll
                for (int i = 0; i < 2; ++i)
#pragma unroll
                    for (int r = 0; r < 16; ++r) {
                        const int ur = 32 * (2 * w + i) + urow16(r);
                        buf_store(fmaxf(acc[i][cb][r] * inv + bin[i][r], 0.0f), ro, so, 4u * (unsigned)ur * (unsigned)T);
                    }
            }
        }
    }
}

static bool boundary_fusable(const SetDiffLoopArgs &a) {
    if (const char *e = getenv("SET_AMD_FUSED_BOUNDARY"))
        if (atoi(e) == 0) return false;
    return a.T % 4 == 0 && a.M <= 96 && a.M >= 2 && ((a.M + 15) / 16 * 16 / 2) % 8 == 0;
}

static int launch_boundary(const SetDiffLoopArgs &a, int Bg, const float *skip, float *x, const float *eps, int sid,
                           uint64_t quad_offset, float *xin_next, bool x2, hipStream_t s) {
    static SetDeviceOnce lds_once;
    if (int rc = set_lds_optin(lds_once, 80 * 1024, "boundary(attr)", diffnet_boundary_kernel, diffnet_boundary_x2_kernel)) return rc;
    BoundaryArgs g = {};
    g.skip = skip; g.x = x; g.eps = eps; g.coef4 = a.coef4 + 4 * sid;
    g.w_skip_p = a.w_skip_p; g.b_skip = a.b_skip; g.w_outp_p = a.w_outp_p; g.b_outp = a.b_outp;
    g.w_in_p = a.w_in_p; g.b_in = a.b_in; g.xin_next = xin_next;
    g.div = sqrtf((float)a.L); g.seed = a.seed; g.quad_offset = quad_offset;
    g.T = a.T; g.M = a.M; g.MP = (a.M + 15) / 16 * 16;
    if (x2) {
        BoundaryX2Args gx = {};
        gx.g = g;
        gx.w_skip_x2 = reinterpret_cast<const unsigned short *>(a.w_skip_x2);
        gx.w_outp_x2 = reinterpret_cast<const unsigned short *>(a.w_outp_x2);
        gx.w_in_x2 = reinterpret_cast<const unsigned short *>(a.w_in_x2);
        gx.err_flag = a.err_flag;
        hipLaunchKernelGGL(diffnet_boundary_x2_kernel, dim3((a.T + 63) / 64, Bg), dim3(256), (size_t)2 * BX_PIECE, s, gx);
    } else {
        hipLaunchKernelGGL(diffnet_boundary_kernel, dim3((a.T + 63) / 64, Bg), dim3(256), (size_t)DC * BD_LD * sizeof(float), s, g);
    }
    return set_check_launch("set_diffusion_loop(boundary)");
}

static SetConv1dArgs conv1x1_args(const float *in, const float *wp, const float *bias, float *out, int B, int Cin,
                                  int Cout, int T) {
    SetConv1dArgs c = {};
    c.in = in; c.w = wp; c.bias = bias; c.out = out;
    c.in_bs = (int64_t)Cin * T; c.in_cs = T; c.out_bs = (int64_t)Cout * T; c.out_cs = T;
    c.B = B; c.Cin = Cin; c.Cout = Cout; c.K = 1; c.dil = 1; c.pad = 0;
    c.T_in = T; c.T_iter = T; c.T_out = T; c.out_stride = 1; c.out_off = 0;
    c.alpha = 1.0f; c.impl = SET_IMPL_MFMA;
    return c;
}

static hipStream_t g_aux_streams[8] = {nullptr};
static int aux_stream(int i, hipStream_t *out) {
    if (!g_aux_streams[i]) SET_HIP(hipStreamCreateWithFlags(&g_aux_streams[i], hipStreamNonBlocking), "aux stream");
    *out = g_aux_streams[i];
    return SET_OK;
}

static int diffusion_chain(const SetDiffLoopArgs &a, int g, int b0, int Bg, hipStream_t s, hipEvent_t *ev) {
    const int T = a.T, M = a.M, L = a.L;
    const int64_t per_batch = (int64_t)M * T;
    float *x = a.x + (int64_t)b0 * per_batch;
    float *ws_x0 = a.ws_x0 + (int64_t)b0 * DC * T, *ws_x1 = a.ws_x1 + (int64_t)b0 * DC * T;
    float *ws_skip = a.ws_skip + (int64_t)b0 * DC * T, *ws_h = a.ws_h + (int64_t)b0 * DC * T;
    float *ws_x0pred = a.ws_x0pred + (int64_t)b0 * per_batch;
    const float *condproj = a.condproj ? a.condproj + (int64_t)b0 * L * 512 * T : nullptr;
    const int tiles_per_utt = (T + NT - 1) / NT;
    int32_t *sync_ws = a.sync_ws ? a.sync_ws + 16 * (int64_t)g + 2 * (int64_t)b0 * ((T + 31) / 32) : nullptr;
    const uint64_t quads_before = (uint64_t)((int64_t)b0 * per_batch / 4);
    const uint64_t quads_total = (uint64_t)(((int64_t)a.B * per_batch + 3) / 4);
    int rc = SET_OK;
    const bool fused_boundary = boundary_fusable(a);
    const bool bf16_loop = a.img16_all != nullptr;
    int n_cu = 0;
    SET_HIP(set_cu_count(&n_cu), "set_diffusion_loop");
    bool boundary_x2 = false;
    if (a.persistent && !bf16_loop && fused_boundary && a.w_skip_x2 && a.w_outp_x2 && a.w_in_x2 && a.wx3_all && a.x3_mode == 2 &&
        a.M <= 96) {
        const int v = stack_variant(Bg, T, a.dilation_cycle_length, a.w1w_all && a.w2w_all, a.w1s_all && a.w2s_all && a.z_ws,
                                    a.x3_mode, n_cu);
        boundary_x2 = v == 5 || (v == 3 && !split_f32_pinned());
    }
    if (bf16_loop && fused_boundary && a.w_skip_x2 && a.w_outp_x2 && a.w_in_x2 && a.M <= 96) boundary_x2 = true;
    if (const char *e = getenv("SET_AMD_BOUNDARY_X2")) boundary_x2 = boundary_x2 && atoi(e) != 0;
    for (int k = 0; k < a.steps && rc == SET_OK; ++k) {
        const int sid = a.steps - 1 - k;
        if (!fused_boundary || k == 0) {
            SetConv1dArgs cin = conv1x1_args(x, a.w_in_p, a.b_in, ws_x0, Bg, M, DC, T);
            cin.act = SET_ACT_RELU;
            rc = set_conv1d(&cin, s);
            if (rc != SET_OK) break;
        }
        float *cur = ws_x0, *nxt = ws_x1;
        if (ev) (void)hipEventRecord(ev[2 * k], s);
        if (a.persistent && !bf16_loop) {
            SetDiffnetStackArgs sa = {};
            sa.xa = ws_x0; sa.xb = ws_x1; sa.skip = ws_skip;
            sa.condproj = condproj; sa.cp_bs = (int64_t)L * 512 * T; sa.cp_ls = (int64_t)512 * T;
            sa.dstep = a.dstep + sid; sa.d_bs = 0; sa.d_cs = a.steps; sa.d_ls = (int64_t)DC * a.steps;
            sa.w1p_all = a.w1p_all; sa.w2p_all = a.w2p_all; sa.b_dil_all = a.b_dil_all; sa.b_out_all = a.b_out_all;
            sa.w1w_all = a.w1w_all; sa.w2w_all = a.w2w_all;
            sa.w1s_all = a.w1s_all; sa.w2s_all = a.w2s_all; sa.wx3_all = a.wx3_all; sa.x3_mode = a.x3_mode;
            sa.z_ws = a.z_ws ? a.z_ws + (int64_t)b0 * DC * 32 * ((T + 31) / 32) : nullptr;
            sa.err_flag = a.err_flag;
            sa.sync_ws = sync_ws;
            sa.B = Bg; sa.T = T; sa.L = L; sa.dilation_cycle_length = a.dilation_cycle_length;
            rc = set_diffnet_stack(&sa, s);
        }
        int fuse = 1;
        if (bf16_loop && a.bf16_ws && a.dilation_cycle_length <= 2) {
            fuse = set_diffnet_layers_bf16_plan(Bg, T, L, a.dilation_cycle_length);
            if (const char *e = getenv("SET_AMD_BF16_FUSE")) fuse = atoi(e) < 1 ? 1 : (atoi(e) > 16 ? 16 : atoi(e));
            if (fuse > 1 && a.bf16_ws_floats < set_diffnet_layers_bf16_scratch_floats(a.B, T, 0, fuse, a.dilation_cycle_length)) fuse = 1;
        }
        for (int l = 0; l < L && rc == SET_OK && bf16_loop && fuse > 1; l += fuse) {
            SetDiffnetLayersBf16Args fa = {};
            fa.x_in = cur; fa.x_out = nxt; fa.skip = ws_skip;
            fa.cond = a.cond + (int64_t)b0 * 192 * T;
            fa.dstep = a.dstep + sid; fa.d_bs = 0; fa.d_cs = a.steps; fa.d_ls = (int64_t)DC * a.steps;
            fa.img = reinterpret_cast<const uint16_t *>(a.img16_all) + (int64_t)l * set_diffnet_layer_bf16_image_size();
            fa.b_dil = a.b_dil_all + (int64_t)l * 512; fa.b_cond = a.b_cond_all + (int64_t)l * 512; fa.b_out = a.b_out_all + (int64_t)l * 512;
            const int64_t per_utt = set_diffnet_layers_bf16_scratch_floats(1, T, 0, fuse, a.dilation_cycle_length);
            fa.scratch = a.bf16_ws + (int64_t)b0 * per_utt; fa.scratch_floats = (int64_t)Bg * per_utt;
            fa.B = Bg; fa.T = T; fa.l0 = l; fa.nl = L - l < fuse ? L - l : fuse; fa.dilation_cycle_length = a.dilation_cycle_length;
            fa.first = (l == 0);
            rc = set_diffnet_layers_fwd_bf16(&fa, s);
            float *tmp = cur; cur = nxt; nxt = tmp;
        }
        for (int l = 0; l < L && rc == SET_OK && bf16_loop && fuse == 1; ++l) {
            SetDiffnetLayerBf16Args la = {};
            la.x_in = cur; la.x_out = nxt; la.skip = ws_skip;
            la.cond = a.cond + (int64_t)b0 * 192 * T;
            la.dstep = a.dstep + (int64_t)l * DC * a.steps + sid;
            la.d_bs = 0; la.d_cs = a.steps;
            la.img = reinterpret_cast<const uint16_t *>(a.img16_all) + (int64_t)l * set_diffnet_layer_bf16_image_size();
            la.b_dil = a.b_dil_all + (int64_t)l * 512; la.b_cond = a.b_cond_all + (int64_t)l * 512;
            la.b_out = a.b_out_all + (int64_t)l * 512;
            la.B = Bg; la.T = T; la.dil = 1 << (l % a.dilation_cycle_length); la.first = (l == 0);
            rc = set_diffnet_layer_fwd_bf16(&la, s);
            float *tmp = cur; cur = nxt; nxt = tmp;
        }
        for (int l = 0; l < L && rc == SET_OK && !a.persistent && !bf16_loop; ++l) {
            SetDiffnetLayerArgs la = {};
            la.x_in = cur; la.x_out = nxt; la.skip = ws_skip;
            la.condproj = condproj + (int64_t)l * 512 * T;
            la.cp_bs = (int64_t)L * 512 * T;
            la.dstep = a.dstep + (int64_t)l * DC * a.steps + sid;
            la.d_bs = 0; la.d_cs = a.steps;
            la.w1p = a.w1p_all + (int64_t)l * (512 * 768); la.b_dil = a.b_dil_all + (int64_t)l * 512;
            la.w2p = a.w2p_all + (int64_t)l * (512 * 256); la.b_out = a.b_out_all + (int64_t)l * 512;
            la.B = Bg; la.T = T; la.dil = 1 << (l % a.dilation_cycle_length); la.first = (l == 0);
            rc = set_diffnet_layer(&la, s);
            float *tmp = cur; cur = nxt; nxt = tmp;
        }
        if (ev) (void)hipEventRecord(ev[2 * k + 1], s);
        if (rc != SET_OK) break;
        const float *eps = a.noise ? a.noise + (int64_t)k * a.B * per_batch + (int64_t)b0 * per_batch : nullptr;
        if (fused_boundary) {
            rc = launch_boundary(a, Bg, ws_skip, x, eps, sid, (uint64_t)(k + 1) * quads_total + quads_before,
                                 k + 1 < a.steps ? ws_x0 : nullptr, boundary_x2, s);
            continue;
        }
        SetConv1dArgs cs = conv1x1_args(ws_skip, a.w_skip_p, a.b_skip, ws_h, Bg, DC, DC, T);
        cs.pro = SET_PRO_DIV; cs.pro_param = sqrtf((float)L); cs.act = SET_ACT_RELU;
        rc = set_conv1d(&cs, s);
        if (rc != SET_OK) break;
        SetConv1dArgs co = conv1x1_args(ws_h, a.w_outp_p, a.b_outp, ws_x0pred, Bg, DC, M, T);
        rc = set_conv1d(&co, s);
        if (rc != SET_OK) break;
        rc = set_posterior_step(ws_x0pred, x, eps, a.coef4 + 4 * sid, 0, x, Bg, per_batch, a.seed,
                                (uint64_t)(k + 1) * quads_total + quads_before, s);
    }
    return rc;
}

extern "C" int set_diffusion_loop(const SetDiffLoopArgs *args, void *stream) {
    SET_REQUIRE(args != nullptr, "set_diffusion_loop");
    const SetDiffLoopArgs &a = *args;
    SET_REQUIRE(a.B > 0 && a.T > 0 && a.M > 0 && a.L > 0 && a.steps > 0 && a.dilation_cycle_length >= 1,
                "set_diffusion_loop");
    SET_REQUIRE(a.x && a.dstep && a.coef4 && a.w_in_p && a.b_in && a.b_dil_all && a.b_out_all && a.w_skip_p && a.b_skip &&
                    a.w_outp_p && a.b_outp, "set_diffusion_loop");
    if (a.img16_all) {
        SET_REQUIRE(a.cond && a.b_cond_all, "set_diffusion_loop(bf16 loop needs cond and b_cond_all)");
    } else {
        SET_REQUIRE(a.condproj && a.w1p_all && a.w2p_all, "set_diffusion_loop");
        SET_REQUIRE(!a.persistent || a.sync_ws, "set_diffusion_loop(persistent needs sync_ws)");
    }
    SET_REQUIRE(a.ws_x0 && a.ws_x1 && a.ws_skip && a.ws_h && a.ws_x0pred, "set_diffusion_loop");
    hipStream_t s = (hipStream_t)stream;
    const int64_t per_batch = (int64_t)a.M * a.T;
    int G = a.n_groups < 1 ? 1 : (a.n_groups > 8 ? 8 : a.n_groups);
    if (G > a.B) G = a.B;
    if (per_batch % 4 != 0) G = 1;
    const bool timing = a.layer_span_ms != nullptr;
    hipEvent_t *ev = nullptr;
    if (timing) {
        ev = new hipEvent_t[(size_t)2 * a.steps * G];
        for (int i = 0; i < 2 * a.steps * G; ++i) SET_HIP(hipEventCreate(&ev[i]), "set_diffusion_loop(event)");
    }
    hipEvent_t loop_ev[2] = {nullptr, nullptr};
    if (a.loop_ms) {
        SET_HIP(hipEventCreate(&loop_ev[0]), "set_diffusion_loop(event)");
        SET_HIP(hipEventCreate(&loop_ev[1]), "set_diffusion_loop(event)");
        (void)hipEventRecord(loop_ev[0], s);
    }
    int rc = SET_OK;
    if (G == 1) {
        rc = diffusion_chain(a, 0, 0, a.B, s, ev);
    } else {
        hipEvent_t fork = nullptr, join[8] = {nullptr};
        SET_HIP(hipEventCreateWithFlags(&fork, hipEventDisableTiming), "set_diffusion_loop(fork)");
        SET_HIP(hipEventRecord(fork, s), "set_diffusion_loop(fork)");
        for (int g = 0; g < G && rc == SET_OK; ++g) {
            const int b0 = (int)((int64_t)a.B * g / G), b1 = (int)((int64_t)a.B * (g + 1) / G);
            hipStream_t sg;
            rc = aux_stream(g, &sg);
            if (rc != SET_OK) break;
            SET_HIP(hipStreamWaitEvent(sg, fork, 0), "set_diffusion_loop(fork wait)");
            rc = diffusion_chain(a, g, b0, b1 - b0, sg, ev ? ev + (size_t)2 * a.steps * g : nullptr);
            SET_HIP(hipEventCreateWithFlags(&join[g], hipEventDisableTiming), "set_diffusion_loop(join)");
            SET_HIP(hipEventRecord(join[g], sg), "set_diffusion_loop(join)");
            SET_HIP(hipStreamWaitEvent(s, join[g], 0), "set_diffusion_loop(join wait)");
        }
        (void)hipEventDestroy(fork);
        for (int g = 0; g < G; ++g)
            if (join[g]) (void)hipEventDestroy(join[g]);
    }
    if (a.loop_ms) (void)hipEventRecord(loop_ev[1], s);
    if (timing || a.loop_ms) {
        if (rc == SET_OK) {
            hipError_t e = hipStreamSynchronize(s);
            if (e != hipSuccess) rc = set_fail(SET_E_LAUNCH, "set_diffusion_loop(sync)", hipGetErrorString(e));
        }
        if (rc == SET_OK && timing) {
            for (int k = 0; k < a.steps; ++k) {
                float acc_ms = 0.0f;
                for (int g = 0; g < G; ++g) {
                    float ms = 0.0f;
                    (void)hipEventElapsedTime(&ms, ev[(size_t)2 * a.steps * g + 2 * k], ev[(size_t)2 * a.steps * g + 2 * k + 1]);
                    acc_ms += ms;
                }
                a.layer_span_ms[k] = acc_ms / (float)G;
            }
        }
        if (rc == SET_OK && a.loop_ms) (void)hipEventElapsedTime(a.loop_ms, loop_ev[0], loop_ev[1]);
    }
    if (ev) {
        for (int i = 0; i < 2 * a.steps * G; ++i) (void)hipEventDestroy(ev[i]);
        delete[] ev;
    }
    if (loop_ev[0]) { (void)hipEventDestroy(loop_ev[0]); (void)hipEventDestroy(loop_ev[1]); }
    return rc;
}

extern "C" int64_t set_sizeof_conv1d_args(void) { return (int64_t)sizeof(SetConv1dArgs); }
extern "C" int64_t set_sizeof_diffnet_layer_args(void) { return (int64_t)sizeof(SetDiffnetLayerArgs); }
extern "C" int64_t set_sizeof_diff_loop_args(void) { return (int64_t)sizeof(SetDiffLoopArgs); }
```

### speech-editing-toolkit_amd/csrc/diffnet_x3.hip

```cpp
#include <stdio.h>
#include <stdlib.h>

#include "common.h"

typedef __bf16 bf16x8_t __attribute__((ext_vector_type(8)));
typedef unsigned u32x4_t __attribute__((ext_vector_type(4)));
typedef unsigned u32x2_t __attribute__((ext_vector_type(2)));

__device__ uint64_t *g_x3_phase_buf = nullptr;
#ifndef SET_X3_PROBE
#define SET_X3_PROBE 0
#endif

namespace {

constexpr int XC = 256;
constexpr int X_MAXD = 8;
constexpr int XR = XC * 2 + 16;
constexpr int X_KS1 = 48;
constexpr int X_KS2 = 16;
constexpr float RSQRT2 = 0.70710678118654752440f;

__device__ __forceinline__ unsigned short f2bf(float x) { return __builtin_bit_cast(unsigned short, (__bf16)x); }
__device__ __forceinline__ float bf2f(unsigned short u) { return __builtin_bit_cast(float, (unsigned)u << 16); }
__device__ __forceinline__ void split3(float a, unsigned short &p0, unsigned short &p1, unsigned short &p2) {
    p0 = f2bf(a);
    const float r1 = a - bf2f(p0);
    p1 = f2bf(r1);
    p2 = f2bf(r1 - bf2f(p1));
}
typedef _Float16 f16x8_t __attribute__((ext_vector_type(8)));
__device__ __forceinline__ unsigned short f2h(float x) { return __builtin_bit_cast(unsigned short, (_Float16)x); }
__device__ __forceinline__ float h2f(unsigned short u) { return (float)__builtin_bit_cast(_Float16, u); }

struct SplitBf16x3 {
    static constexpr int NP = 3, NPROD = 6, MODE = 3, PF = 2, PF2 = 1;
    static __device__ __forceinline__ constexpr int qa(int t) { return t == 0 ? 2 : (t == 1 || t == 3) ? 1 : 0; }
    static __device__ __forceinline__ constexpr int qb(int t) { return t == 2 ? 2 : (t == 1 || t == 4) ? 1 : 0; }
    static __device__ __forceinline__ void split(float a, unsigned short (&p)[3]) { split3(a, p[0], p[1], p[2]); }
    static __device__ __forceinline__ f32x16 mma(u32x4_t a, u32x4_t b, f32x16 c) {
        return __builtin_amdgcn_mfma_f32_32x32x16_bf16(__builtin_bit_cast(bf16x8_t, a), __builtin_bit_cast(bf16x8_t, b), c, 0, 0, 0);
    }
};
struct SplitF16x2 {
    static constexpr int NP = 2, NPROD = 3, MODE = 2, PF = 4, PF2 = 2;
    static __device__ __forceinline__ constexpr int qa(int t) { return t == 0 ? 1 : 0; }
    static __device__ __forceinline__ constexpr int qb(int t) { return t == 1 ? 1 : 0; }
    static __device__ __forceinline__ void split(float a, unsigned short (&p)[2]) {
        p[0] = f2h(a);
        p[1] = f2h(a - h2f(p[0]));
    }
    static __device__ __forceinline__ void split2(float a, float b, unsigned (&p)[2]) { split2_f16(a, b, p[0], p[1]); }
    static __device__ __forceinline__ f32x16 mma(u32x4_t a, u32x4_t b, f32x16 c) {
        return __builtin_amdgcn_mfma_f32_32x32x16_f16(__builtin_bit_cast(f16x8_t, a), __builtin_bit_cast(f16x8_t, b), c, 0, 0, 0);
    }
};
template <typename S> constexpr int64_t x_n1() { return 8LL * X_KS1 * 2 * S::NP * 512; }
template <typename S> constexpr int64_t x_n2() { return 8LL * X_KS2 * 2 * S::NP * 512; }
constexpr int X_KSV = 32;
template <typename S> constexpr int64_t x_nv() { return S::MODE == 2 ? 8LL * X_KSV * 4 * S::NP * 512 + 8 : 0; }
template <typename S> constexpr int64_t x_nimg() { return x_n1<S>() + x_n2<S>() + 8 + x_nv<S>(); }
__device__ __forceinline__ u32x4_t buf_load_u4(rsrc_t r, unsigned voff, unsigned soff) {
    return __builtin_amdgcn_raw_buffer_load_b128(r, (int)voff, (int)soff, 0);
}
__device__ __forceinline__ float fsig(float x) { return __builtin_amdgcn_rcpf(1.0f + __expf(-x)); }
__device__ __forceinline__ float ftanh(float x) { return 1.0f - 2.0f * __builtin_amdgcn_rcpf(1.0f + __expf(2.0f * x)); }
__device__ __forceinline__ int urow(int r) { return (r & 3) + 8 * (r >> 2); }
constexpr int X_NT = 2;
__device__ __forceinline__ float buf_load_nt(rsrc_t r, unsigned voff, unsigned soff) {
    return __builtin_bit_cast(float, __builtin_amdgcn_raw_buffer_load_b32(r, (int)voff, (int)soff, X_NT));
}

template <typename S>
__global__ void __launch_bounds__(256) pack_layer_x3_kernel(const float *wdil, const float *wout, unsigned short *img, float s1, float s2) {
    const int64_t idx = (int64_t)blockIdx.x * 256 + threadIdx.x;
    constexpr int64_t n1 = x_n1<S>() / S::NP, n2 = x_n2<S>() / S::NP;
    constexpr int64_t nv = x_nv<S>() > 0 ? (x_nv<S>() - 8) / S::NP : 0;
    if (idx == 0) {
        float *tail = reinterpret_cast<float *>(img + x_n1<S>() + x_n2<S>());
        tail[0] = s1; tail[1] = 1.0f / s1; tail[2] = s2; tail[3] = 1.0f / s2;
        if (nv > 0) {
            float *tw = reinterpret_cast<float *>(img + x_nimg<S>() - 8);
            tw[0] = 0.5f * s1; tw[1] = 1.0f / (0.5f * s1); tw[2] = 0.0f; tw[3] = 0.0f;
        }
    }
    if (idx >= n1 + n2 + nv) return;
    if (idx >= n1 + n2) {
        int64_t r = idx - n1 - n2;
        const int e = r & 7; r >>= 3;
        const int l = r & 63; r >>= 6;
        const int mb = r & 3; r >>= 2;
        const int ks = (int)(r % X_KSV), w = (int)(r / X_KSV);
        const int row = (mb >= 2 ? XC : 0) + 32 * w + 16 * (mb & 1) + (l & 15), k = 8 * (l >> 4) + e;
        const int plane = ks >> 3, c = 32 * (ks & 7) + k;
        const float *g = wdil + ((int64_t)row * XC + c) * 3;
        const double g0 = g[0], g1 = g[1], gg2 = g[2];
        const double u = plane == 0 ? 0.5 * (g0 + g1 + gg2) : (plane == 1 ? 0.5 * (g0 - g1 + gg2) : (plane == 2 ? g0 : -gg2));
        unsigned short p[S::NP];
        S::split((0.5f * s1) * (float)u, p);
        unsigned short *base = img + x_n1<S>() + x_n2<S>() + 8 + ((((int64_t)w * X_KSV + ks) * 4 + mb) * S::NP) * 512 + l * 8 + e;
#pragma unroll
        for (int q = 0; q < S::NP; ++q) base[q * 512] = p[q];
        return;
    }
    const bool g2 = idx >= n1;
    int64_t r = g2 ? idx - n1 : idx;
    const int e = r & 7; r >>= 3;
    const int l = r & 63; r >>= 6;
    const int rb = r & 1; r >>= 1;
    const int nks = g2 ? X_KS2 : X_KS1;
    const int ks = (int)(r % nks), w = (int)(r / nks);
    const int row = (rb ? XC : 0) + 32 * w + (l & 31), k = 8 * (l >> 5) + e;
    const float v = g2 ? s2 * wout[(int64_t)row * XC + 16 * ks + k] : s1 * wdil[((int64_t)row * XC + 16 * (ks % 16) + k) * 3 + ks / 16];
    unsigned short p[S::NP];
    S::split(v, p);
    unsigned short *base = img + (g2 ? x_n1<S>() : 0) + ((((int64_t)w * nks + ks) * 2 + rb) * S::NP) * 512 + l * 8 + e;
#pragma unroll
    for (int q = 0; q < S::NP; ++q) base[q * 512] = p[q];
}

template <typename S, int NKS, int NU, int NCB, int PF, typename BF>
__device__ __forceinline__ void gemm_x3(f32x16 (&acc)[NU][2][NCB], rsrc_t img, unsigned lane16, unsigned abase, unsigned ustride,
                                        const unsigned char *lds, unsigned piece_bytes, BF bfrag) {
    constexpr int NP = S::NP;
    static_assert(NKS % PF == 0, "k-steps must be a multiple of the prefetch distance");
    u32x4_t A[PF][NU][2][NP];
#pragma unroll
    for (int p = 0; p < PF; ++p)
#pragma unroll
        for (int u = 0; u < NU; ++u)
#pragma unroll
            for (int rb = 0; rb < 2; ++rb)
#pragma unroll
                for (int q = 0; q < NP; ++q)
                    A[p][u][rb][q] = buf_load_u4(img, lane16, abase + (unsigned)u * ustride + (unsigned)(((p * 2 + rb) * NP + q) * 1024));
    for (int kb = 0; kb < NKS; kb += PF) {
#pragma unroll
        for (int p = 0; p < PF; ++p) {
            const int ks = kb + p;
            u32x4_t Bv[NCB][NP];
#pragma unroll
            for (int cb = 0; cb < NCB; ++cb) {
                const unsigned bo = bfrag(ks, cb);
#pragma unroll
                for (int q = 0; q < NP; ++q) Bv[cb][q] = *reinterpret_cast<const u32x4_t *>(lds + q * piece_bytes + bo);
            }
            __builtin_amdgcn_sched_barrier(0);
            __builtin_amdgcn_s_setprio(1);
#pragma unroll
            for (int t = 0; t < S::NPROD; ++t)
#pragma unroll
                for (int u = 0; u < NU; ++u)
#pragma unroll
                    for (int rb = 0; rb < 2; ++rb)
#pragma unroll
                        for (int cb = 0; cb < NCB; ++cb)
                            acc[u][rb][cb] = S::mma(A[p][u][rb][S::qa(t)], Bv[cb][S::qb(t)], acc[u][rb][cb]);
            __builtin_amdgcn_s_setprio(0);
            const int kn = min(ks + PF, NKS - 1);
#pragma unroll
            for (int u = 0; u < NU; ++u)
#pragma unroll
                for (int rb = 0; rb < 2; ++rb)
#pragma unroll
                    for (int q = 0; q < NP; ++q)
                        A[p][u][rb][q] = buf_load_u4(img, lane16, abase + (unsigned)u * ustride + (unsigned)(((kn * 2 + rb) * NP + q) * 1024));
            __builtin_amdgcn_sched_barrier(0);
        }
    }
}

template <typename S, int NCB>
constexpr size_t x3_lds_bytes(int max_dil) {
    return (size_t)S::NP * (size_t)(NCB * (32 + 2 * max_dil) * XR) + NCB * XC * sizeof(float) + 16;
}

struct X3Tile {
    const float *xin;
    float *xout, *skp;
    const float *cp;
    const float *dstep;
    int64_t cp_bs, d_bs, d_cs;
    const unsigned short *img;
    const float *b_dil, *b_out;
    int32_t *err_flag;
    int T, dil, first;
    int q0, nbu, Q;
};

struct X3Col {
    int b, t0;
    bool ok;
};
__device__ __forceinline__ X3Col x3_col(const X3Tile &a, int cb) {
    const int q = a.q0 + cb, qc = min(q, a.Q - 1);
    X3Col c;
    c.b = qc / a.nbu;
    c.t0 = (qc - c.b * a.nbu) * 32;
    c.ok = q < a.Q;
    return c;
}

template <int NP>
__device__ __forceinline__ void pack8(const unsigned short (&p)[8][NP], u32x4_t (&u)[NP]) {
#pragma unroll
    for (int q = 0; q < NP; ++q)
#pragma unroll
        for (int e = 0; e < 4; ++e) u[q][e] = (unsigned)p[2 * e][q] | ((unsigned)p[2 * e + 1][q] << 16);
}

template <int NU, int NCB>
__device__ __forceinline__ void x3_init(const X3Tile &a, f32x16 (&acc)[NU][2][NCB]) {
    const int lane = threadIdx.x & 63;
    const int w = __builtin_amdgcn_readfirstlane(threadIdx.x >> 6);
    const int half = lane >> 5, l31 = lane & 31;
    const int T = a.T;
    const unsigned T4 = 4u * (unsigned)T;
#pragma unroll
    for (int cb = 0; cb < NCB; ++cb) {
        const X3Col c = x3_col(a, cb);
        const rsrc_t rcp = make_rsrc(a.cp + (int64_t)c.b * a.cp_bs);
        const unsigned vo4 = 4u * (unsigned)(4 * half * T + min(c.t0 + l31, T - 1));
#pragma unroll
        for (int u = 0; u < NU; ++u)
#pragma unroll
            for (int rb = 0; rb < 2; ++rb) {
                const float *bd = a.b_dil + (rb ? XC : 0) + 32 * (NU * w + u);
#pragma unroll
                for (int r = 0; r < 16; ++r) {
                    const unsigned ur = (unsigned)((rb ? XC : 0) + 32 * (NU * w + u) + urow(r));
                    const float blo = bd[urow(r)], bhi = bd[urow(r) + 4];
                    acc[u][rb][cb][r] = (half ? bhi : blo) + buf_load_nt(rcp, vo4, ur * T4);
                }
            }
    }
}

template <typename S, int NU, int NCB>
__device__ __forceinline__ void x3_main(const X3Tile &a, f32x16 (&acc)[NU][2][NCB], unsigned char *lds, unsigned piece_bytes, uint64_t *dbg,
                                        uint64_t &tprev) {
#define X3_PHASE(p)                                           \
    if (dbg) {                                                \
        const uint64_t tn = __builtin_amdgcn_s_memtime();     \
        dbg[p] += tn - tprev;                                 \
        tprev = tn;                                           \
    }
    X3_PHASE(0)
    constexpr int NP = S::NP;
    constexpr int NW = 8 / NU, NT = 64 * NW;
    const int tid = threadIdx.x, lane = tid & 63;
    const int w = __builtin_amdgcn_readfirstlane(tid >> 6);
    const int half = lane >> 5, l31 = lane & 31;
    const int T = a.T, d = a.dil;
    const int RB = 32 + 2 * d;
    float *dsh = reinterpret_cast<float *>(lds + NP * piece_bytes);
    const unsigned T4 = 4u * (unsigned)T;
    const rsrc_t rw = make_rsrc(a.img);
    const unsigned lane16 = 16u * (unsigned)lane;
    auto row0 = [&](int u, int rb) { return (rb ? XC : 0) + 32 * (NU * w + u); };
    const float *sc = reinterpret_cast<const float *>(a.img + x_n1<S>() + x_n2<S>());
    const float s1 = sc[0], is1 = sc[1], s2 = sc[2], is2 = sc[3];
    bool tv[NCB];
    unsigned vo4[NCB];
    int64_t ub[NCB];
#pragma unroll
    for (int cb = 0; cb < NCB; ++cb) {
        const X3Col c = x3_col(a, cb);
        const int t = c.t0 + l31;
        tv[cb] = c.ok && t < T;
        vo4[cb] = 4u * (unsigned)(4 * half * T + min(t, T - 1));
        ub[cb] = (int64_t)c.b * XC * T;
    }

    {
        constexpr int NCG = (NW / NCB) * 2, CHG = XC / NCG, CPT = CHG < 32 ? CHG : 32, NPASS = CHG / CPT;
        const int cbs = w % NCB, fr = lane & 31, cg = (w / NCB) * 2 + (lane >> 5);
        const X3Col c = x3_col(a, cbs);
        const rsrc_t rx = make_rsrc(a.xin + (int64_t)c.b * XC * T);
#pragma unroll
        for (int i0 = 0; i0 < XC * NCB; i0 += NT) {
            const int idx = i0 + tid;
            if (NT <= XC * NCB || idx < XC * NCB) {
                const X3Col cd = x3_col(a, idx >> 8);
                dsh[idx] = a.dstep[(int64_t)cd.b * a.d_bs + (int64_t)(idx & 255) * a.d_cs];
            }
        }
        float amax = 0.0f;
        auto put = [&](int jj, int ch0, const float (&v)[CPT], bool valid) {
#pragma unroll
            for (int q8 = 0; q8 < CPT / 8; ++q8) {
                unsigned short p[8][NP];
                const f32x4 d0 = *reinterpret_cast<const f32x4 *>(dsh + XC * cbs + ch0 + 8 * q8);
                const f32x4 d1 = *reinterpret_cast<const f32x4 *>(dsh + XC * cbs + ch0 + 8 * q8 + 4);
#pragma unroll
                for (int e = 0; e < 8; ++e) {
                    const int ch = 8 * q8 + e;
                    const float xs = v[ch] + (e < 4 ? d0[e & 3] : d1[e & 3]);
                    const float xv = valid ? xs : 0.0f;
                    if constexpr (S::MODE == 2) amax = fmaxf(amax, fabsf(xv));
                    S::split(xv, p[e]);
                }
                u32x4_t u[NP];
                pack8<NP>(p, u);
#pragma unroll
                for (int q = 0; q < NP; ++q)
                    *reinterpret_cast<u32x4_t *>(lds + q * piece_bytes + (cbs * RB + jj) * XR + (ch0 + 8 * q8) * 2) = u[q];
            }
        };
        const int t = c.t0 - d + fr, th = c.t0 - d + 32 + fr;
        const bool tvx = c.ok && t >= 0 && t < T, has_h = fr < 2 * d, tvh = c.ok && th >= 0 && th < T;
#pragma unroll
        for (int ps = 0; ps < NPASS; ++ps) {
            const int ch0 = CHG * cg + CPT * ps;
            const unsigned cgo = (unsigned)ch0 * T4;
            const unsigned vox = 4u * (unsigned)min(max(t, 0), T - 1) + cgo, voh = 4u * (unsigned)min(max(th, 0), T - 1) + cgo;
            float vx[CPT], vh[CPT];
#pragma unroll
            for (int k = 0; k < CPT; ++k) vx[k] = buf_load(rx, vox, (unsigned)k * T4);
            if (has_h) {
#pragma unroll
                for (int k = 0; k < CPT; ++k) vh[k] = buf_load(rx, voh, (unsigned)k * T4);
            }
            if (ps == 0) __syncthreads();
            put(fr, ch0, vx, tvx);
            if (has_h) put(32 + fr, ch0, vh, tvh);
        }
        if constexpr (S::MODE == 2) {
            if (!(amax < 32768.0f) && a.err_flag) __hip_atomic_store(a.err_flag, 2, __ATOMIC_RELAXED, __HIP_MEMORY_SCOPE_AGENT);
        }
    }
    if constexpr (NU != 1) x3_init<NU, NCB>(a, acc);
#pragma unroll
    for (int u = 0; u < NU; ++u)
#pragma unroll
        for (int rb = 0; rb < 2; ++rb)
#pragma unroll
            for (int cb = 0; cb < NCB; ++cb)
#pragma unroll
                for (int r = 0; r < 16; ++r) acc[u][rb][cb][r] *= s1;
    __syncthreads();
    X3_PHASE(1)

    gemm_x3<S, X_KS1, NU, NCB, (NU == 1 ? S::PF : S::PF2)>(
        acc, rw, lane16, (unsigned)(NU * w * X_KS1 * 2 * NP * 1024), (unsigned)(X_KS1 * 2 * NP * 1024), lds, piece_bytes, [&](int ks, int cb) {
            return (unsigned)((cb * RB + l31 + (ks >> 4) * d) * XR + ((ks & 15) * 16 + half * 8) * 2);
        });
    X3_PHASE(2)

    float xres[NU][NCB][16];
    auto load_xres = [&]() {
#pragma unroll
        for (int cb = 0; cb < NCB; ++cb) {
            const rsrc_t rx = make_rsrc(a.xin + ub[cb]);
#pragma unroll
            for (int u = 0; u < NU; ++u)
#pragma unroll
                for (int r = 0; r < 16; ++r) xres[u][cb][r] = buf_load(rx, vo4[cb], (unsigned)(row0(u, 0) + urow(r)) * T4);
        }
    };
    if constexpr (NU == 1) load_xres();
    __syncthreads();
    X3_PHASE(8)
#pragma unroll
    for (int u = 0; u < NU; ++u)
#pragma unroll
        for (int cb = 0; cb < NCB; ++cb)
#pragma unroll
            for (int g = 0; g < 4; ++g) {
                unsigned short p[4][NP];
#pragma unroll
                for (int e = 0; e < 4; ++e) {
                    const int r = 4 * g + e;
                    const float zz = fsig(acc[u][0][cb][r] * is1) * ftanh(acc[u][1][cb][r] * is1);
                    const float z = tv[cb] ? zz : 0.0f;
                    S::split(z, p[e]);
                }
                const unsigned off = (unsigned)((cb * 32 + l31) * XR + (32 * (NU * w + u) + 8 * g + 4 * half) * 2);
#pragma unroll
                for (int q = 0; q < NP; ++q) {
                    u32x2_t uu;
                    uu[0] = (unsigned)p[0][q] | ((unsigned)p[1][q] << 16);
                    uu[1] = (unsigned)p[2][q] | ((unsigned)p[3][q] << 16);
                    *reinterpret_cast<u32x2_t *>(lds + q * piece_bytes + off) = uu;
                }
            }
    X3_PHASE(9)
    if constexpr (NU != 1) load_xres();
#pragma unroll
    for (int u = 0; u < NU; ++u)
#pragma unroll
        for (int rb = 0; rb < 2; ++rb) {
            const float *bo = a.b_out + row0(u, rb);
#pragma unroll
            for (int r = 0; r < 16; ++r) {
                const float blo = bo[urow(r)], bhi = bo[urow(r) + 4];
                const float bias = half ? bhi : blo;
#pragma unroll
                for (int cb = 0; cb < NCB; ++cb) acc[u][rb][cb][r] = (rb == 0 ? bias + xres[u][cb][r] : bias) * s2;
            }
        }
    float sk[NU][NCB][16];
    auto load_sk = [&]() {
#pragma unroll
        for (int cb = 0; cb < NCB; ++cb) {
            const rsrc_t rsk = make_rsrc(a.skp + ub[cb]);
#pragma unroll
            for (int u = 0; u < NU; ++u)
#pragma unroll
                for (int r = 0; r < 16; ++r) sk[u][cb][r] = buf_load_nt(rsk, vo4[cb], (unsigned)(32 * (NU * w + u) + urow(r)) * T4);
        }
    };
    if constexpr (NU == 1) load_sk();
    X3_PHASE(10)
    __syncthreads();
    X3_PHASE(3)

    gemm_x3<S, X_KS2, NU, NCB, (NU == 1 ? S::PF : S::PF2)>(
        acc, rw, lane16, (unsigned)(x_n1<S>() * 2 + NU * w * X_KS2 * 2 * NP * 1024), (unsigned)(X_KS2 * 2 * NP * 1024), lds, piece_bytes,
        [&](int ks, int cb) { return (unsigned)((cb * 32 + l31) * XR + (ks * 16 + half * 8) * 2); });
    X3_PHASE(4)

#pragma unroll
    for (int cb = 0; cb < NCB; ++cb) {
        if (tv[cb]) {
            const rsrc_t rxo = make_rsrc(a.xout + ub[cb]);
#pragma unroll
            for (int u = 0; u < NU; ++u)
#pragma unroll
                for (int r = 0; r < 16; ++r)
                    buf_store_agent((acc[u][0][cb][r] * is2) * RSQRT2, rxo, vo4[cb], (unsigned)(row0(u, 0) + urow(r)) * T4);
        }
    }
    const bool first = a.first != 0;
    if constexpr (NU != 1) {
        if (!first) load_sk();
    }
#pragma unroll
    for (int cb = 0; cb < NCB; ++cb) {
        if (tv[cb]) {
            const rsrc_t rsk = make_rsrc(a.skp + ub[cb]);
#pragma unroll
            for (int u = 0; u < NU; ++u)
#pragma unroll
                for (int r = 0; r < 16; ++r)
                    buf_store_agent(first ? acc[u][1][cb][r] * is2 : acc[u][1][cb][r] * is2 + sk[u][cb][r], rsk, vo4[cb],
                                    (unsigned)(32 * (NU * w + u) + urow(r)) * T4);
        }
    }
}
#undef X3_PHASE

template <typename S, int NU, int NCB>
__global__ void __launch_bounds__(512 / NU, NU) diffnet_stack_x3_kernel(SetDiffnetStackArgs a, int tiles_per_utt, int ntiles, int ntasks,
                                                                        unsigned piece_bytes, int fault_tile) {
    extern __shared__ __attribute__((aligned(16))) unsigned char lds[];
    int *s_task = reinterpret_cast<int *>(lds + S::NP * piece_bytes + NCB * XC * sizeof(float));
    int *counter = a.sync_ws, *abort_flag = a.sync_ws + 1, *done = a.sync_ws + 4;
    const int tid = threadIdx.x;
    uint64_t *dbg = (SET_X3_PROBE && blockIdx.x == 0 && tid == 0) ? g_x3_phase_buf : nullptr;
    uint64_t tprev = dbg ? __builtin_amdgcn_s_memtime() : 0;
    if (tid == 0) s_task[0] = atomicAdd(counter, 1);
    __syncthreads();
    int n = __builtin_amdgcn_readfirstlane(s_task[0]);
    int i_done = -1, l_done = 0;
    while (n < ntasks) {
        const int l = n / ntiles, i = n - l * ntiles, j = i;
        X3Tile lt;
        lt.xin = (l & 1) ? a.xb : a.xa;
        lt.xout = (l & 1) ? a.xa : a.xb;
        lt.skp = a.skip;
        lt.cp = a.condproj + (int64_t)l * a.cp_ls; lt.cp_bs = a.cp_bs;
        lt.dstep = a.dstep + (int64_t)l * a.d_ls; lt.d_bs = a.d_bs; lt.d_cs = a.d_cs;
        lt.img = reinterpret_cast<const unsigned short *>(a.wx3_all) + (int64_t)l * x_nimg<S>();
        lt.b_dil = a.b_dil_all + (int64_t)l * 512;
        lt.b_out = a.b_out_all + (int64_t)l * 512;
        lt.err_flag = a.err_flag;
        lt.T = a.T; lt.dil = 1 << (l % a.dilation_cycle_length); lt.first = (l == 0);
        lt.nbu = (a.T + 31) / 32; lt.Q = a.B * lt.nbu; lt.q0 = i * NCB;
        f32x16 acc[NU][2][NCB];
        if constexpr (NU == 1) x3_init<NU, NCB>(lt, acc);
        __builtin_amdgcn_sched_barrier(0);
        const int *f0 = done + i, *fl = done + (j > 0 ? i - 1 : i), *fr = done + (j < tiles_per_utt - 1 ? i + 1 : i);
        int peek = l, claimed = 0;
        if (tid == 0) {
            if (l > 0) peek = min(ld_agent(f0), min(ld_agent(fl), ld_agent(fr)));
            claimed = atomicAdd(counter, 1);
        }
        if (dbg) { const uint64_t tn = __builtin_amdgcn_s_memtime(); dbg[11] += tn - tprev; tprev = tn; }
        asm volatile("s_waitcnt vmcnt(0)" ::: "memory");
        if (dbg) { const uint64_t tn = __builtin_amdgcn_s_memtime(); dbg[12] += tn - tprev; tprev = tn; }
        if (tid == 0) {
            if (peek >= l) __builtin_amdgcn_fence(__ATOMIC_ACQUIRE, "agent");
            s_task[0] = claimed;
            s_task[1] = peek >= l ? 1 : 2;
        }
        __syncthreads();
        if (tid == 0 && i_done >= 0 && !(l_done == 0 && i_done == fault_tile))
            __hip_atomic_store(done + i_done, l_done + 1, __ATOMIC_RELAXED, __HIP_MEMORY_SCOPE_AGENT);
        i_done = -1;
        if (__builtin_amdgcn_readfirstlane(s_task[1]) == 2) {
            if (tid == 0) {
                int ok = 1;
                unsigned spins = 0;
                for (;;) {
                    const int v0 = ld_agent(f0), v1 = ld_agent(fl), v2 = ld_agent(fr);
                    if (min(v0, min(v1, v2)) >= l) break;
                    __builtin_amdgcn_s_sleep(8);
                    if (++spins > STACK_SPIN_LIMIT || ld_agent(abort_flag) != 0) {
                        __hip_atomic_store(abort_flag, 1, __ATOMIC_RELAXED, __HIP_MEMORY_SCOPE_AGENT);
                        if (a.err_flag) __hip_atomic_store(a.err_flag, 1, __ATOMIC_RELAXED, __HIP_MEMORY_SCOPE_AGENT);
                        ok = 0;
                        break;
                    }
                }
                __builtin_amdgcn_fence(__ATOMIC_ACQUIRE, "agent");
                s_task[2] = ok;
            }
            __syncthreads();
            if (__builtin_amdgcn_readfirstlane(s_task[2]) == 0) break;
        }
        const int n_next = __builtin_amdgcn_readfirstlane(s_task[0]);
        x3_main<S, NU, NCB>(lt, acc, lds, piece_bytes, dbg, tprev);
        i_done = i;
        l_done = l;
        n = n_next;
        if (dbg) {
            const uint64_t tn = __builtin_amdgcn_s_memtime();
            dbg[5] += tn - tprev;
            dbg[7] += 1;
            tprev = tn;
        }
    }
    asm volatile("s_waitcnt vmcnt(0)" ::: "memory");
    __syncthreads();
    if (tid == 0 && i_done >= 0 && !(l_done == 0 && i_done == fault_tile))
        __hip_atomic_store(done + i_done, l_done + 1, __ATOMIC_RELAXED, __HIP_MEMORY_SCOPE_AGENT);
}

template <typename S, int NU, int NCB>
int launch_x3(const SetDiffnetStackArgs &a, int n_cu, int fault_tile, hipStream_t s) {
    static SetDeviceOnce lds_once;
    if (int rc = set_lds_optin(lds_once, 160 * 1024, "set_diffnet_stack(x3 attr)", diffnet_stack_x3_kernel<S, NU, NCB>)) return rc;
    const int Q = a.B * ((a.T + 31) / 32);
    const int ntiles = (Q + NCB - 1) / NCB, tiles_per_utt = ntiles;
    const int64_t ntasks64 = (int64_t)ntiles * a.L;
    SET_REQUIRE(ntasks64 < (1ll << 30), "set_diffnet_stack(task count)");
    SET_REQUIRE((int64_t)2 * XC * a.T * 4 < ((int64_t)1 << 31), "set_diffnet_stack(split-operand kernel: T too large)");
    const int max_dil = 1 << (a.dilation_cycle_length - 1);
    const unsigned piece_bytes = (unsigned)(NCB * (32 + 2 * max_dil) * XR);
    const size_t ldsz = x3_lds_bytes<S, NCB>(max_dil);
    SET_HIP(set_zero_async(a.sync_ws, (size_t)(4 + ntiles) * sizeof(int32_t), s), "set_diffnet_stack(memset)");
    int grid = NU * n_cu;
    if (grid > ntiles * 4 / 5) grid = ntiles * 4 / 5;
    if (const char *e = getenv("SET_AMD_STACK_GRID")) grid = atoi(e) > 0 ? atoi(e) : grid;
    if ((int64_t)grid > ntasks64) grid = (int)ntasks64;
    if (grid < 1) grid = 1;
    hipLaunchKernelGGL((diffnet_stack_x3_kernel<S, NU, NCB>), dim3(grid), dim3(512 / NU), ldsz, s, a, tiles_per_utt, ntiles, (int)ntasks64,
                       piece_bytes, fault_tile);
    return set_check_launch("set_diffnet_stack");
}

typedef unsigned u32x2w_t __attribute__((ext_vector_type(2)));
typedef float f32x2 __attribute__((ext_vector_type(2)));
__device__ __forceinline__ f32x2 buf_load2(rsrc_t r, unsigned voff, unsigned soff) {
    return __builtin_bit_cast(f32x2, __builtin_amdgcn_raw_buffer_load_b64(r, (int)voff, (int)soff, 0));
}
__device__ __forceinline__ f32x2 buf_load2_nt(rsrc_t r, unsigned voff, unsigned soff) {
    return __builtin_bit_cast(f32x2, __builtin_amdgcn_raw_buffer_load_b64(r, (int)voff, (int)soff, X_NT));
}

constexpr int XRV = XC * 2 + 32;
template <int NB> constexpr unsigned xv_piece() { return 16 * NB * XRV; }
template <int NB> constexpr unsigned xv_plane() { return 2 * xv_piece<NB>(); }
template <int NB> constexpr unsigned xv_zpiece() { return 32 * NB * XR; }
template <int NB> constexpr unsigned xv_tile() { return 2 * xv_plane<NB>() > 2 * xv_zpiece<NB>() ? 2 * xv_plane<NB>() : 2 * xv_zpiece<NB>(); }
constexpr int XV_PF = 2;
constexpr int XV_PF2 = 2;
constexpr int X3V_FLAG_UNIT = 8;

__device__ __forceinline__ f32x4 mma16(u32x4_t a, u32x4_t b, f32x4 c) {
    return __builtin_amdgcn_mfma_f32_16x16x32_f16(__builtin_bit_cast(f16x8_t, a), __builtin_bit_cast(f16x8_t, b), c, 0, 0, 0);
}
__device__ __forceinline__ float row_prev(float v) {
    return __builtin_bit_cast(float, __builtin_amdgcn_update_dpp(0, __builtin_bit_cast(int, v), 0x111, 0xf, 0xf, false));
}
__device__ __forceinline__ float row_next(float v) {
    return __builtin_bit_cast(float, __builtin_amdgcn_update_dpp(0, __builtin_bit_cast(int, v), 0x101, 0xf, 0xf, false));
}

template <int NB>
__device__ __forceinline__ void x3v_init(const X3Tile &a, f32x4 (&PQ)[2][4][NB]) {
    typedef SplitF16x2 S;
    int tid = threadIdx.x;
    asm volatile("" : "+v"(tid));
    const int lane = tid & 63;
    const int w = __builtin_amdgcn_readfirstlane(tid >> 6);
    const int l15 = lane & 15, kg = lane >> 4;
    const int T = a.T;
    const unsigned T4 = 4u * (unsigned)T;
    const float hs = 0.5f * reinterpret_cast<const float *>(a.img + x_nimg<S>() - 8)[0];
    f32x4 bias[4];
#pragma unroll
    for (int mb = 0; mb < 4; ++mb) bias[mb] = *reinterpret_cast<const f32x4 *>(a.b_dil + (mb >= 2 ? XC : 0) + 32 * w + 16 * (mb & 1) + 4 * kg);
#pragma unroll
    for (int nb = 0; nb < NB; ++nb) {
        const X3Col c = x3_col(a, nb);
        const rsrc_t rcp = make_rsrc(a.cp + (int64_t)c.b * a.cp_bs);
        const unsigned vo = 4u * (unsigned)(4 * kg * T + min(c.t0 + 2 * l15, T - 2));
#pragma unroll
        for (int mb = 0; mb < 4; ++mb) {
            const unsigned row0 = (unsigned)((mb >= 2 ? XC : 0) + 32 * w + 16 * (mb & 1));
#pragma unroll
            for (int i = 0; i < 4; ++i) {
                const f32x2 v = buf_load2_nt(rcp, vo, (row0 + (unsigned)i) * T4);
                const float e = bias[mb][i] + v[0], o = bias[mb][i] + v[1];
                PQ[0][mb][nb][i] = hs * (e + o);
                PQ[1][mb][nb][i] = hs * (e - o);
            }
        }
    }
}

template <int NB, int PH>
__device__ __forceinline__ void x3v_stage_load(const X3Tile &a, int w, int lane, f32x2 (&x12)[NB][8], float (&xh)[NB][8]) {
    const int l15 = lane & 15, cs = lane >> 4;
    const int ch0 = 32 * w + 8 * cs;
    const int T = a.T;
    const unsigned T4 = 4u * (unsigned)T;
    const bool edge = l15 == 0 || l15 == 15;
#pragma unroll
    for (int nb = 0; nb < NB; ++nb) {
        const X3Col c = x3_col(a, nb);
        const rsrc_t rx = make_rsrc(a.xin + (int64_t)c.b * XC * T);
        const int t = c.t0 + 2 * l15;
        const unsigned vox = 4u * (unsigned)min(t, T - 2) + (unsigned)ch0 * T4;
#pragma unroll
        for (int k = 0; k < 8; ++k) x12[nb][k] = buf_load2(rx, vox, (unsigned)k * T4);
        if (PH == 1) {
            const int th = l15 == 0 ? c.t0 - 1 : c.t0 + 32;
            const unsigned voh = 4u * (unsigned)min(max(th, 0), T - 1) + (unsigned)ch0 * T4;
            if (edge) {
#pragma unroll
                for (int k = 0; k < 8; ++k) xh[nb][k] = buf_load(rx, voh, (unsigned)k * T4);
            }
        }
    }
}
template <int NB, int PH>
__device__ __forceinline__ float x3v_stage_store(const X3Tile &a, unsigned char *lds, const float *dsh, int w, int lane, const f32x2 (&x12)[NB][8],
                                                 const float (&xh)[NB][8]) {
    typedef SplitF16x2 S;
    const int l15 = lane & 15, cs = lane >> 4;
    const int ch0 = 32 * w + 8 * cs;
    const int T = a.T;
    const bool edge = l15 == 0 || l15 == 15;
    float amax = 0.0f;
#pragma unroll
    for (int nb = 0; nb < NB; ++nb) {
        const X3Col c = x3_col(a, nb);
        const int t = c.t0 + 2 * l15, th = l15 == 0 ? c.t0 - 1 : c.t0 + 32;
        const bool v12 = c.ok && t < T, vh = c.ok && edge && th >= 0 && th < T;
        const f32x4 dA = *reinterpret_cast<const f32x4 *>(dsh + nb * XC + ch0);
        const f32x4 dB = *reinterpret_cast<const f32x4 *>(dsh + nb * XC + ch0 + 4);
        u32x4_t u[2][2];
#pragma unroll
        for (int e2 = 0; e2 < 4; ++e2) {
            float V[2][2];
#pragma unroll
            for (int h = 0; h < 2; ++h) {
                const int e = 2 * e2 + h;
                const float ds = e < 4 ? dA[e & 3] : dB[e & 3];
                const float d1 = v12 ? x12[nb][e][0] + ds : 0.0f, d2 = v12 ? x12[nb][e][1] + ds : 0.0f;
                if (PH == 0) {
                    V[0][h] = d1 + d2;
                    V[1][h] = d2 - d1;
                } else {
                    float d0 = row_prev(d2), d3 = row_next(d1);
                    const float hv = vh ? xh[nb][e] + ds : 0.0f;
                    d0 = l15 == 0 ? hv : d0;
                    d3 = l15 == 15 ? hv : d3;
                    V[0][h] = d0 - d2;
                    V[1][h] = d1 - d3;
                }
            }
#pragma unroll
            for (int j = 0; j < 2; ++j) {
                amax = fmaxf(fmaxf(amax, fabsf(V[j][0])), fabsf(V[j][1]));
                unsigned pw[2];
                S::split2(V[j][0], V[j][1], pw);
                u[j][0][e2] = pw[0];
                u[j][1][e2] = pw[1];
            }
        }
#pragma unroll
        for (int j = 0; j < 2; ++j)
#pragma unroll
            for (int q = 0; q < 2; ++q) *reinterpret_cast<u32x4_t *>(lds + j * xv_plane<NB>() + q * xv_piece<NB>() + (16 * nb + l15) * XRV + ch0 * 2) = u[j][q];
    }
    return amax;
}

template <int NB, int PFV>
__device__ __forceinline__ void x3v_plane(f32x4 (&acc)[4][NB], u32x4_t (&A)[PFV][4][2], rsrc_t img, unsigned lane16, unsigned abase, int seg,
                                          const unsigned char *bplane, unsigned boff) {
    typedef SplitF16x2 S;
    const int ks_last = 16 * (seg >> 1) + 15;
    for (int kb = 0; kb < 8; kb += PFV) {
#pragma unroll
        for (int p = 0; p < PFV; ++p) {
            const int kc = kb + p, ks = 8 * seg + kc;
            u32x4_t Bv[NB][2];
#pragma unroll
            for (int nb = 0; nb < NB; ++nb)
#pragma unroll
                for (int q = 0; q < 2; ++q) Bv[nb][q] = *reinterpret_cast<const u32x4_t *>(bplane + q * xv_piece<NB>() + boff + (unsigned)(nb * 16 * XRV) + (unsigned)kc * 64u);
            __builtin_amdgcn_sched_barrier(0);
            __builtin_amdgcn_s_setprio(1);
#pragma unroll
            for (int t = 0; t < S::NPROD; ++t)
#pragma unroll
                for (int mb = 0; mb < 4; ++mb)
#pragma unroll
                    for (int nb = 0; nb < NB; ++nb) acc[mb][nb] = mma16(A[p][mb][S::qa(t)], Bv[nb][S::qb(t)], acc[mb][nb]);
            __builtin_amdgcn_s_setprio(0);
            const int kn = min(ks + PFV, ks_last);
#pragma unroll
            for (int mb = 0; mb < 4; ++mb)
#pragma unroll
                for (int q = 0; q < 2; ++q) A[p][mb][q] = buf_load_u4(img, lane16, abase + (unsigned)(((kn * 4 + mb) * 2 + q) * 1024));
            __builtin_amdgcn_sched_barrier(0);
        }
    }
}

template <int NB>
__device__ __forceinline__ void x3v_main(const X3Tile &a, f32x4 (&PQ)[2][4][NB], unsigned char *lds, uint64_t *dbg, uint64_t &tprev, uint64_t (&ts)[32]) {
#if SET_X3_PROBE == 2
#define X3V_PHASE(p)                                  \
    {                                                 \
        __builtin_amdgcn_sched_barrier(0);            \
        ts[8 + (p)] = __builtin_amdgcn_s_memtime();   \
        __builtin_amdgcn_sched_barrier(0);            \
    }
#else
#define X3V_PHASE(p)                                          \
    if (dbg) {                                                \
        const uint64_t tn = __builtin_amdgcn_s_memtime();     \
        dbg[p] += tn - tprev;                                 \
        tprev = tn;                                           \
    }
#endif
#if SET_X3_PROBE == 2
#define X3V_TS(p) X3V_PHASE(p)
#else
#define X3V_TS(p)
#endif
    X3V_PHASE(0)
    typedef SplitF16x2 S;
    constexpr int PFV = XV_PF;
    int tid = threadIdx.x;
    asm volatile("" : "+v"(tid));
    const int lane = tid & 63;
    const int w = __builtin_amdgcn_readfirstlane(tid >> 6);
    const int l15 = lane & 15, kg = lane >> 4;
    const int half = lane >> 5, l31 = lane & 31;
    const int T = a.T;
    const unsigned T4 = 4u * (unsigned)T;
    const unsigned lane16 = 16u * (unsigned)lane;
    float *dsh = reinterpret_cast<float *>(lds + xv_tile<NB>());
    const rsrc_t rw = make_rsrc(a.img);
    const float *sc = reinterpret_cast<const float *>(a.img + x_n1<S>() + x_n2<S>());
    const float s2 = sc[2], is2 = sc[3];
    const float is1w = reinterpret_cast<const float *>(a.img + x_nimg<S>() - 8)[1];
    const float cg2 = is1w * -1.4426950408889634f, cf2 = is1w * 2.8853900817779268f;
    const unsigned abase = (unsigned)((x_n1<S>() + x_n2<S>() + 8) * 2) + (unsigned)(w * X_KSV * 4 * 2 * 1024);
    const unsigned boff = (unsigned)(l15 * XRV + kg * 16);
    u32x4_t A[PFV][4][2];
    f32x2 x12[NB][8];
    float xh[NB][8];
    x3v_stage_load<NB, 0>(a, w, lane, x12, xh);
    float amax = x3v_stage_store<NB, 0>(a, lds, dsh, w, lane, x12, xh);
#pragma unroll
    for (int p = 0; p < PFV; ++p)
#pragma unroll
        for (int mb = 0; mb < 4; ++mb)
#pragma unroll
            for (int q = 0; q < 2; ++q) A[p][mb][q] = buf_load_u4(rw, lane16, abase + (unsigned)(((p * 4 + mb) * 2 + q) * 1024));
    X3V_TS(12)
    __syncthreads();
    X3V_PHASE(1)
    x3v_plane<NB, PFV>(PQ[0], A, rw, lane16, abase, 0, lds, boff);
    x3v_plane<NB, PFV>(PQ[1], A, rw, lane16, abase, 1, lds + xv_plane<NB>(), boff);
    X3V_PHASE(2)
    x3v_stage_load<NB, 1>(a, w, lane, x12, xh);
    __builtin_amdgcn_sched_barrier(0);
#pragma unroll
    for (int mb = 0; mb < 4; ++mb)
#pragma unroll
        for (int nb = 0; nb < NB; ++nb)
#pragma unroll
            for (int i = 0; i < 4; ++i) {
                const float pp = PQ[0][mb][nb][i], qq = PQ[1][mb][nb][i];
                PQ[0][mb][nb][i] = pp + qq;
                PQ[1][mb][nb][i] = pp - qq;
            }
    __syncthreads();
    X3V_TS(13)
    amax = fmaxf(amax, x3v_stage_store<NB, 1>(a, lds, dsh, w, lane, x12, xh));
    if (!(amax < 32768.0f) && a.err_flag) __hip_atomic_store(a.err_flag, 2, __ATOMIC_RELAXED, __HIP_MEMORY_SCOPE_AGENT);
#pragma unroll
    for (int p = 0; p < PFV; ++p)
#pragma unroll
        for (int mb = 0; mb < 4; ++mb)
#pragma unroll
            for (int q = 0; q < 2; ++q) A[p][mb][q] = buf_load_u4(rw, lane16, abase + (unsigned)((((16 + p) * 4 + mb) * 2 + q) * 1024));
    X3V_TS(14)
    __syncthreads();
    X3V_PHASE(3)
    x3v_plane<NB, PFV>(PQ[0], A, rw, lane16, abase, 2, lds, boff);
    x3v_plane<NB, PFV>(PQ[1], A, rw, lane16, abase, 3, lds + xv_plane<NB>(), boff);
    X3V_PHASE(4)
    bool tv[NB];
    unsigned vo4[NB];
    int64_t ub[NB];
#pragma unroll
    for (int cb = 0; cb < NB; ++cb) {
        const X3Col c = x3_col(a, cb);
        const int t = c.t0 + l31;
        tv[cb] = c.ok && t < T;
        vo4[cb] = 4u * (unsigned)(4 * half * T + min(t, T - 1));
        ub[cb] = (int64_t)c.b * XC * T;
    }
    float xres[NB][16];
#pragma unroll
    for (int cb = 0; cb < NB; ++cb) {
        const rsrc_t rx = make_rsrc(a.xin + ub[cb]);
#pragma unroll
        for (int r = 0; r < 16; ++r) xres[cb][r] = buf_load(rx, vo4[cb], (unsigned)(32 * w + urow(r)) * T4);
    }
    __syncthreads();
    X3V_TS(15)
#pragma unroll
    for (int nb = 0; nb < NB; ++nb) {
        const X3Col c = x3_col(a, nb);
        const bool tvp = c.ok && c.t0 + 2 * l15 < T;
#pragma unroll
        for (int eo = 0; eo < 2; ++eo)
#pragma unroll
            for (int m = 0; m < 2; ++m) {
                float zz[4];
#pragma unroll
                for (int i = 0; i < 4; ++i) {
                    const float u = __builtin_amdgcn_exp2f(PQ[eo][m][nb][i] * cg2);
                    const float v = __builtin_amdgcn_exp2f(fminf(PQ[eo][m + 2][nb][i] * cf2, 64.0f));
                    const float g = (v - 1.0f) * __builtin_amdgcn_rcpf((1.0f + u) * (1.0f + v));
                    zz[i] = tvp ? g : 0.0f;
                }
                unsigned plo[2], phi[2];
                S::split2(zz[0], zz[1], plo);
                S::split2(zz[2], zz[3], phi);
                const unsigned off = (unsigned)((32 * nb + 2 * l15 + eo) * XR + (32 * w + 16 * m + 4 * kg) * 2);
#pragma unroll
                for (int q = 0; q < 2; ++q) {
                    u32x2w_t uu;
                    uu[0] = plo[q];
                    uu[1] = phi[q];
                    *reinterpret_cast<u32x2w_t *>(lds + q * xv_zpiece<NB>() + off) = uu;
                }
            }
    }
    f32x16 acc[1][2][NB];
#pragma unroll
    for (int rb = 0; rb < 2; ++rb) {
        const float *bo = a.b_out + (rb ? XC : 0) + 32 * w;
#pragma unroll
        for (int r = 0; r < 16; ++r) {
            const float blo = bo[urow(r)], bhi = bo[urow(r) + 4];
            const float bias = half ? bhi : blo;
#pragma unroll
            for (int cb = 0; cb < NB; ++cb) acc[0][rb][cb][r] = (rb == 0 ? bias + xres[cb][r] : bias) * s2;
        }
    }
    X3V_TS(16)
    __syncthreads();
    X3V_PHASE(8)
    gemm_x3<S, X_KS2, 1, NB, XV_PF2>(acc, rw, lane16, (unsigned)(x_n1<S>() * 2 + w * X_KS2 * 2 * 2 * 1024), (unsigned)(X_KS2 * 2 * 2 * 1024), lds,
                                     xv_zpiece<NB>(), [&](int ks, int cb) { return (unsigned)((cb * 32 + l31) * XR + (ks * 16 + half * 8) * 2); });
    X3V_PHASE(9)
    const bool first = a.first != 0;
    float sk[NB][16];
    if (!first) {
#pragma unroll
        for (int cb = 0; cb < NB; ++cb) {
            const rsrc_t rsk = make_rsrc(a.skp + ub[cb]);
#pragma unroll
            for (int r = 0; r < 16; ++r) sk[cb][r] = buf_load_nt(rsk, vo4[cb], (unsigned)(32 * w + urow(r)) * T4);
        }
    }
#pragma unroll
    for (int cb = 0; cb < NB; ++cb) {
        if (tv[cb]) {
            const rsrc_t rxo = make_rsrc(a.xout + ub[cb]);
#pragma unroll
            for (int r = 0; r < 16; ++r) buf_store_agent((acc[0][0][cb][r] * is2) * RSQRT2, rxo, vo4[cb], (unsigned)(32 * w + urow(r)) * T4);
        }
    }
    X3V_TS(17)
#pragma unroll
    for (int cb = 0; cb < NB; ++cb) {
        if (tv[cb]) {
            const rsrc_t rsk = make_rsrc(a.skp + ub[cb]);
#pragma unroll
            for (int r = 0; r < 16; ++r)
                buf_store_agent(first ? acc[0][1][cb][r] * is2 : acc[0][1][cb][r] * is2 + sk[cb][r], rsk, vo4[cb], (unsigned)(32 * w + urow(r)) * T4);
        }
    }
    X3V_PHASE(10)
}
#undef X3V_PHASE
#undef X3V_TS

#if SET_X3_PROBE == 2
#ifndef X3V_TL_TASK
#define X3V_TL_TASK 10
#endif
#define X3V_KTS(p)                                \
    {                                             \
        __builtin_amdgcn_sched_barrier(0);        \
        ts[p] = __builtin_amdgcn_s_memtime();     \
        __builtin_amdgcn_sched_barrier(0);        \
    }
#else
#define X3V_KTS(p)
#endif
template <int NB>
__global__ void __launch_bounds__(512, 1) diffnet_stack_x3v_kernel(SetDiffnetStackArgs a, int ntiles, int ntasks, int fault_tile) {
    typedef SplitF16x2 S;
    extern __shared__ __attribute__((aligned(16))) unsigned char lds[];
    int *s_task = reinterpret_cast<int *>(lds + xv_tile<NB>() + NB * XC * sizeof(float));
    int *counter = a.sync_ws, *abort_flag = a.sync_ws + 1, *done = a.sync_ws + 4;
    const int tid = threadIdx.x;
    uint64_t *dbg = (SET_X3_PROBE == 1 && blockIdx.x == 0 && tid == 0) ? g_x3_phase_buf : nullptr;
    uint64_t tprev = dbg ? __builtin_amdgcn_s_memtime() : 0;
    if (tid == 0) s_task[0] = atomicAdd(counter, 1);
    __syncthreads();
    int n = __builtin_amdgcn_readfirstlane(s_task[0]);
    int i_done = -1, l_done = 0;
    uint64_t ts[32] = {};
    int n_mine = 0;
    (void)n_mine;
    while (n < ntasks) {
        const int l = n / ntiles, i = n - l * ntiles;
        X3Tile lt;
        lt.xin = (l & 1) ? a.xb : a.xa;
        lt.xout = (l & 1) ? a.xa : a.xb;
        lt.skp = a.skip;
        lt.cp = a.condproj + (int64_t)l * a.cp_ls; lt.cp_bs = a.cp_bs;
        lt.dstep = a.dstep + (int64_t)l * a.d_ls; lt.d_bs = a.d_bs; lt.d_cs = a.d_cs;
        lt.img = reinterpret_cast<const unsigned short *>(a.wx3_all) + (int64_t)l * x_nimg<S>();
        lt.b_dil = a.b_dil_all + (int64_t)l * 512;
        lt.b_out = a.b_out_all + (int64_t)l * 512;
        lt.err_flag = a.err_flag;
        lt.T = a.T; lt.dil = 1; lt.first = (l == 0);
        lt.nbu = (a.T + 31) / 32; lt.Q = a.B * lt.nbu; lt.q0 = i * NB;
        f32x4 PQ[2][4][NB];
        X3V_KTS(0)
        if (i_done >= 0) {
            asm volatile("s_waitcnt vmcnt(0)" ::: "memory");
            if ((tid & 63) == 0 && !(l_done == 0 && i_done == fault_tile))
                (void)__hip_atomic_fetch_add(done + i_done, 1, __ATOMIC_RELAXED, __HIP_MEMORY_SCOPE_AGENT);
            i_done = -1;
        }
        __builtin_amdgcn_sched_barrier(0);
        float dsv[(NB * XC + 511) / 512];
#pragma unroll
        for (int j = 0; j < (NB * XC + 511) / 512; ++j) {
            const int idx = min(tid + 512 * j, NB * XC - 1);
            dsv[j] = lt.dstep[(int64_t)x3_col(lt, idx >> 8).b * lt.d_bs + (int64_t)(idx & (XC - 1)) * lt.d_cs];
        }
        x3v_init<NB>(lt, PQ);
        __builtin_amdgcn_sched_barrier(0);
        const int *f0 = done + i, *fl = done + (i > 0 ? i - 1 : i), *fr = done + (i < ntiles - 1 ? i + 1 : i);
        int peek = l, claimed = 0;
        if (tid == 0) {
            if (l > 0) peek = min(ld_agent(f0), min(ld_agent(fl), ld_agent(fr))) / X3V_FLAG_UNIT;
            claimed = atomicAdd(counter, 1);
        }
        X3V_KTS(1)
        asm volatile("s_waitcnt vmcnt(0)" ::: "memory");
        X3V_KTS(2)
        {
            float *dsh = reinterpret_cast<float *>(lds + xv_tile<NB>());
#pragma unroll
            for (int j = 0; j < (NB * XC + 511) / 512; ++j)
                if (tid + 512 * j < NB * XC) dsh[tid + 512 * j] = dsv[j];
        }
        if (tid == 0) {
            if (peek >= l) __builtin_amdgcn_fence(__ATOMIC_ACQUIRE, "agent");
            s_task[0] = claimed;
            s_task[1] = peek >= l ? 1 : 2;
        }
        __syncthreads();
        X3V_KTS(3)
        if (__builtin_amdgcn_readfirstlane(s_task[1]) == 2) {
            if (tid == 0) {
                int ok = 1;
                unsigned spins = 0;
                for (;;) {
                    const int v0 = ld_agent(f0), v1 = ld_agent(fl), v2 = ld_agent(fr);
                    if (min(v0, min(v1, v2)) >= l * X3V_FLAG_UNIT) break;
                    __builtin_amdgcn_s_sleep(8);
                    if (++spins > STACK_SPIN_LIMIT || ld_agent(abort_flag) != 0) {
                        __hip_atomic_store(abort_flag, 1, __ATOMIC_RELAXED, __HIP_MEMORY_SCOPE_AGENT);
                        if (a.err_flag) __hip_atomic_store(a.err_flag, 1, __ATOMIC_RELAXED, __HIP_MEMORY_SCOPE_AGENT);
                        ok = 0;
                        break;
                    }
                }
                __builtin_amdgcn_fence(__ATOMIC_ACQUIRE, "agent");
                s_task[2] = ok;
            }
            __syncthreads();
            if (__builtin_amdgcn_readfirstlane(s_task[2]) == 0) break;
        }
        const int n_next = __builtin_amdgcn_readfirstlane(s_task[0]);
        X3V_KTS(4)
        x3v_main<NB>(lt, PQ, lds, dbg, tprev, ts);
#if SET_X3_PROBE == 2
        if (++n_mine == X3V_TL_TASK && (tid == 0 || tid == 448) && g_x3_phase_buf) {
            const rsrc_t rt = make_rsrc(g_x3_phase_buf);
            const unsigned row = (unsigned)(2 * blockIdx.x + (tid ? 1 : 0)) * 128u;
#pragma unroll
            for (int k = 0; k < 32; ++k) __builtin_amdgcn_raw_buffer_store_b32((unsigned)(ts[k] - ts[0]), rt, (int)(row + 4 * k), 0, 0);
            __builtin_amdgcn_raw_buffer_store_b32((unsigned)n, rt, (int)(row + 20), 0, 0);
            __builtin_amdgcn_raw_buffer_store_b32((unsigned)s_task[1], rt, (int)(row + 24), 0, 0);
            __builtin_amdgcn_raw_buffer_store_b32((unsigned)ts[0], rt, (int)(row + 28), 0, 0);
        } else if (n_mine == X3V_TL_TASK + 1 && (tid == 0 || tid == 448) && g_x3_phase_buf) {
            __builtin_amdgcn_raw_buffer_store_b32((unsigned)ts[0], make_rsrc(g_x3_phase_buf), (int)((unsigned)(2 * blockIdx.x + (tid ? 1 : 0)) * 128u + 124u), 0, 0);
        }
#endif
        i_done = i;
        l_done = l;
        n = n_next;
        if (dbg) {
            const uint64_t tn = __builtin_amdgcn_s_memtime();
            dbg[5] += tn - tprev;
            dbg[7] += 1;
            tprev = tn;
        }
    }
    asm volatile("s_waitcnt vmcnt(0)" ::: "memory");
    if ((tid & 63) == 0 && i_done >= 0 && !(l_done == 0 && i_done == fault_tile))
        (void)__hip_atomic_fetch_add(done + i_done, 1, __ATOMIC_RELAXED, __HIP_MEMORY_SCOPE_AGENT);
}

template <int NB>
int launch_x3v(const SetDiffnetStackArgs &a, int n_cu, int fault_tile, hipStream_t s) {
    static SetDeviceOnce lds_once;
    if (int rc = set_lds_optin(lds_once, 160 * 1024, "set_diffnet_stack(x3v attr)", diffnet_stack_x3v_kernel<NB>)) return rc;
    const int Q = a.B * ((a.T + 31) / 32);
    const int ntiles = (Q + NB - 1) / NB;
    const int64_t ntasks64 = (int64_t)ntiles * a.L;
    SET_REQUIRE(ntasks64 < (1ll << 30), "set_diffnet_stack(task count)");
    SET_REQUIRE((int64_t)2 * XC * a.T * 4 < ((int64_t)1 << 31), "set_diffnet_stack(split-operand kernel: T too large)");
    SET_REQUIRE(a.dilation_cycle_length == 1 && a.T % 2 == 0, "set_diffnet_stack(x3v: dilation 1 and even T only)");
    const size_t ldsz = (size_t)xv_tile<NB>() + NB * XC * sizeof(float) + 16;
    SET_HIP(set_zero_async(a.sync_ws, (size_t)(4 + ntiles) * sizeof(int32_t), s), "set_diffnet_stack(memset)");
    int grid = n_cu;
    if (NB == 2 && grid > ntiles * 4 / 5) grid = ntiles * 4 / 5;
    if (const char *e = getenv("SET_AMD_STACK_GRID")) grid = atoi(e) > 0 ? atoi(e) : grid;
    if ((int64_t)grid > ntasks64) grid = (int)ntasks64;
    if (grid < 1) grid = 1;
    hipLaunchKernelGGL(diffnet_stack_x3v_kernel<NB>, dim3(grid), dim3(512), ldsz, s, a, ntiles, (int)ntasks64, fault_tile);
    return set_check_launch("set_diffnet_stack");
}


constexpr int SX_PF = 8;

__device__ __forceinline__ float buf_load_sc1(rsrc_t r, unsigned voff, unsigned soff) {
    return __builtin_bit_cast(float, __builtin_amdgcn_raw_buffer_load_b32(r, (int)voff, (int)soff, 16));
}
__device__ __forceinline__ u32x4_t buf_load_u4_sc1(rsrc_t r, unsigned voff, unsigned soff) {
    return __builtin_amdgcn_raw_buffer_load_b128(r, (int)voff, (int)soff, 16);
}

__device__ __forceinline__ bool sx_wait(const int *f0, const int *f1, const int *f2, int want, int *abort_flag, int *err_flag, bool fence = true) {
    unsigned spins = 0;
    for (;;) {
        const int v0 = ld_agent(f0), v1 = ld_agent(f1), v2 = ld_agent(f2);
        if (min(v0, min(v1, v2)) >= want) break;
        __builtin_amdgcn_s_sleep(1);
        if (++spins > SPLIT_SPIN_LIMIT || ld_agent(abort_flag) != 0) {
            __hip_atomic_store(abort_flag, 1, __ATOMIC_RELAXED, __HIP_MEMORY_SCOPE_AGENT);
            if (err_flag) __hip_atomic_store(err_flag, 1, __ATOMIC_RELAXED, __HIP_MEMORY_SCOPE_AGENT);
            return false;
        }
    }
    if (fence) __builtin_amdgcn_fence(__ATOMIC_ACQUIRE, "agent");
    return true;
}

template <int NKS, typename BF>
__device__ __forceinline__ void sx_gemm(f32x16 &acc, u32x4_t (&A)[SX_PF][2], rsrc_t img, unsigned lane16, unsigned abase,
                                        const unsigned char *lds, unsigned piece_bytes, BF bfrag) {
    unsigned bo = bfrag(0);
    u32x4_t b0 = *reinterpret_cast<const u32x4_t *>(lds + bo);
    u32x4_t b1 = *reinterpret_cast<const u32x4_t *>(lds + piece_bytes + bo);
#pragma unroll 1
    for (int kb = 0; kb < NKS; kb += SX_PF) {
#pragma unroll
        for (int p = 0; p < SX_PF; ++p) {
            const int ks = kb + p;
            const unsigned bn = bfrag(min(ks + 1, NKS - 1));
            const u32x4_t nb0 = *reinterpret_cast<const u32x4_t *>(lds + bn);
            const u32x4_t nb1 = *reinterpret_cast<const u32x4_t *>(lds + piece_bytes + bn);
            acc = SplitF16x2::mma(A[p][1], b0, acc);
            acc = SplitF16x2::mma(A[p][0], b1, acc);
            acc = SplitF16x2::mma(A[p][0], b0, acc);
            const int kn = min(ks + SX_PF, NKS - 1);
            A[p][0] = buf_load_u4(img, lane16, abase + (unsigned)(kn * 4 * 1024));
            A[p][1] = buf_load_u4(img, lane16, abase + (unsigned)((kn * 4 + 1) * 1024));
            b0 = nb0;
            b1 = nb1;
            __builtin_amdgcn_sched_barrier(0);
        }
    }
}
__device__ __forceinline__ void sx_preload(u32x4_t (&A)[SX_PF][2], rsrc_t img, unsigned lane16, unsigned abase) {
#pragma unroll
    for (int p = 0; p < SX_PF; ++p) {
        A[p][0] = buf_load_u4(img, lane16, abase + (unsigned)(p * 4 * 1024));
        A[p][1] = buf_load_u4(img, lane16, abase + (unsigned)((p * 4 + 1) * 1024));
    }
}

__global__ void __launch_bounds__(256, 1) diffnet_stack_split_x2_kernel(SetDiffnetStackArgs a, int tiles_per_utt, int ntiles,
                                                                         unsigned piece_bytes, int fault_tile, int nofence) {
    typedef SplitF16x2 S;
    extern __shared__ __attribute__((aligned(16))) unsigned char lds[];
    float *gs = reinterpret_cast<float *>(lds + 2 * piece_bytes);
    float *dsh = gs + 64 * 32;
    int *s_ok = reinterpret_cast<int *>(dsh + XC);
    int *abort_flag = a.sync_ws + 1, *ready = a.sync_ws + 4, *zcnt = a.sync_ws + 4 + ntiles;
    const int tid = threadIdx.x, lane = tid & 63, half = lane >> 5, l31 = lane & 31;
    const int j = __builtin_amdgcn_readfirstlane(tid >> 6);
    if ((int)blockIdx.x >= 4 * ntiles) {
        const int hp = blockIdx.x & 3;
        for (int l = 1; l < a.L; ++l) {
            unsigned spins = 0;
            while (l >= 2 && ld_agent(ready) < 4 * (l - 1)) {
                __builtin_amdgcn_s_sleep(8);
                if (++spins > SPLIT_SPIN_LIMIT || ld_agent(abort_flag) != 0) return;
            }
            const unsigned char *img = reinterpret_cast<const unsigned char *>(a.wx3_all) + (int64_t)l * x_nimg<S>() * 2;
            const rsrc_t r1 = make_rsrc(img + (size_t)(2 * hp) * X_KS1 * 4 * 1024);
            const rsrc_t r2 = make_rsrc(img + x_n1<S>() * 2 + (size_t)(2 * hp) * X_KS2 * 4 * 1024);
            for (unsigned off = 16u * tid; off < 2u * X_KS1 * 4 * 1024; off += 8u * 4096u) {
#pragma unroll
                for (unsigned q = 0; q < 8; ++q) {
                    const u32x4_t v = buf_load_u4(r1, off + q * 4096u, 0u);
                    asm volatile("" ::"v"(v));
                }
            }
            for (unsigned off = 16u * tid; off < 2u * X_KS2 * 4 * 1024; off += 8u * 4096u) {
#pragma unroll
                for (unsigned q = 0; q < 8; ++q) {
                    const u32x4_t v = buf_load_u4(r2, off + q * 4096u, 0u);
                    asm volatile("" ::"v"(v));
                }
            }
        }
        return;
    }
    const int i = blockIdx.x >> 2, h = blockIdx.x & 3;
    const int b = i / tiles_per_utt, jt = i - b * tiles_per_utt;
    const int T = a.T, t0 = jt * 32;
    const int il = jt > 0 ? i - 1 : i, ir = jt < tiles_per_utt - 1 ? i + 1 : i;
    const unsigned T4 = 4u * (unsigned)T;
    const int w8 = 2 * h + (j & 1), rb = j >> 1;
    const int ch0 = 32 * w8;
    const int tq = t0 + l31;
    const bool tv = tq < T;
    const unsigned vo4 = 4u * (unsigned)(4 * half * T + min(tq, T - 1));
    const unsigned lane16 = 16u * (unsigned)lane;
    unsigned short *zt = reinterpret_cast<unsigned short *>(a.z_ws) + (int64_t)i * (2 * 32 * XC);
    const rsrc_t rz = make_rsrc(zt);
    const rsrc_t rsk = make_rsrc(a.skip + (int64_t)b * XC * T);
    uint64_t *dbg = (SET_X3_PROBE && blockIdx.x == 5 && tid == 0) ? g_x3_phase_buf : nullptr;
    uint64_t tprev = dbg ? __builtin_amdgcn_s_memtime() : 0;
#define SX_PHASE(p)                                           \
    if (dbg) {                                                \
        const uint64_t tn = __builtin_amdgcn_s_memtime();     \
        dbg[p] += tn - tprev;                                 \
        tprev = tn;                                           \
    }
    for (int l = 0; l < a.L; ++l) {
        const int d = 1 << (l % a.dilation_cycle_length);
        const unsigned short *img = reinterpret_cast<const unsigned short *>(a.wx3_all) + (int64_t)l * x_nimg<S>();
        const rsrc_t rw = make_rsrc(img);
        const float *sc = reinterpret_cast<const float *>(img + x_n1<S>() + x_n2<S>());
        const float s1 = sc[0], is1 = sc[1], s2 = sc[2], is2 = sc[3];
        const rsrc_t rxin = make_rsrc(((l & 1) ? a.xb : a.xa) + (int64_t)b * XC * T);
        const rsrc_t rxout = make_rsrc(((l & 1) ? a.xa : a.xb) + (int64_t)b * XC * T);
        const rsrc_t rcp = make_rsrc(a.condproj + (int64_t)l * a.cp_ls + (int64_t)b * a.cp_bs);
        const float *dstep = a.dstep + (int64_t)l * a.d_ls + (int64_t)b * a.d_bs;
        const float *bd = a.b_dil_all + (int64_t)l * 512 + rb * XC + ch0, *bo = a.b_out_all + (int64_t)l * 512 + rb * XC + ch0;
        u32x4_t A[SX_PF][2];
        const unsigned ab1 = (unsigned)(((w8 * X_KS1) * 2 + rb) * 2 * 1024);
        sx_preload(A, rw, lane16, ab1);
        f32x16 acc;
#pragma unroll
        for (int r = 0; r < 16; ++r) {
            const float blo = bd[urow(r)], bhi = bd[urow(r) + 4];
            acc[r] = (half ? bhi : blo) + buf_load(rcp, vo4, (unsigned)(rb * XC + ch0 + urow(r)) * T4);
        }
        if (tid == 0) *s_ok = (l == 0 || sx_wait(ready + i, ready + il, ready + ir, 4 * l, abort_flag, a.err_flag, !nofence)) ? 1 : 0;
        __syncthreads();
        if (__builtin_amdgcn_readfirstlane(*s_ok) == 0) return;
        SX_PHASE(0)
        {
            const int f = tid & 31, cg = tid >> 5;
            dsh[tid] = dstep[(int64_t)tid * a.d_cs];
            float amax = 0.0f;
            auto put = [&](int row, const float (&v)[32], bool valid) {
#pragma unroll
                for (int q8 = 0; q8 < 4; ++q8) {
                    unsigned short p[8][2];
                    const f32x4 d0 = *reinterpret_cast<const f32x4 *>(dsh + 32 * cg + 8 * q8);
                    const f32x4 d1 = *reinterpret_cast<const f32x4 *>(dsh + 32 * cg + 8 * q8 + 4);
#pragma unroll
                    for (int e = 0; e < 8; ++e) {
                        const float xs = v[8 * q8 + e] + (e < 4 ? d0[e & 3] : d1[e & 3]);
                        const float xv = valid ? xs : 0.0f;
                        amax = fmaxf(amax, fabsf(xv));
                        S::split(xv, p[e]);
                    }
                    u32x4_t u[2];
                    pack8<2>(p, u);
                    *reinterpret_cast<u32x4_t *>(lds + row * XR + (32 * cg + 8 * q8) * 2) = u[0];
                    *reinterpret_cast<u32x4_t *>(lds + piece_bytes + row * XR + (32 * cg + 8 * q8) * 2) = u[1];
                }
            };
            const int t = t0 - d + f, th = t0 - d + 32 + f;
            const bool tvx = t >= 0 && t < T, has_h = f < 2 * d, tvh = th >= 0 && th < T;
            const unsigned vox = 4u * (unsigned)min(max(t, 0), T - 1), voh = 4u * (unsigned)min(max(th, 0), T - 1);
            float vx[32], vh[32];
            if (nofence) {
#pragma unroll
                for (int k = 0; k < 32; ++k) vx[k] = buf_load_sc1(rxin, vox, (unsigned)(32 * cg + k) * T4);
                if (has_h) {
#pragma unroll
                    for (int k = 0; k < 32; ++k) vh[k] = buf_load_sc1(rxin, voh, (unsigned)(32 * cg + k) * T4);
                }
            } else {
#pragma unroll
                for (int k = 0; k < 32; ++k) vx[k] = buf_load(rxin, vox, (unsigned)(32 * cg + k) * T4);
                if (has_h) {
#pragma unroll
                    for (int k = 0; k < 32; ++k) vh[k] = buf_load(rxin, voh, (unsigned)(32 * cg + k) * T4);
                }
            }
            __syncthreads();
            put(f, vx, tvx);
            if (has_h) put(32 + f, vh, tvh);
            if (!(amax < 32768.0f) && a.err_flag) __hip_atomic_store(a.err_flag, 2, __ATOMIC_RELAXED, __HIP_MEMORY_SCOPE_AGENT);
        }
#pragma unroll
        for (int r = 0; r < 16; ++r) acc[r] *= s1;
        __syncthreads();
        SX_PHASE(1)
        sx_gemm<X_KS1>(acc, A, rw, lane16, ab1, lds, piece_bytes, [&](int ks) {
            return (unsigned)((l31 + (ks >> 4) * d) * XR + ((ks & 15) * 16 + half * 8) * 2);
        });
        SX_PHASE(2)
        if (rb == 1) {
#pragma unroll
            for (int r = 0; r < 16; ++r) gs[(32 * (j & 1) + urow(r) + 4 * half) * 32 + l31] = ftanh(acc[r] * is1);
        }
        __syncthreads();
        if (rb == 0) {
#pragma unroll
            for (int g = 0; g < 4; ++g) {
                unsigned short p[4][2];
#pragma unroll
                for (int e = 0; e < 4; ++e) {
                    const int r = 4 * g + e;
                    const float zz = fsig(acc[r] * is1) * gs[(32 * (j & 1) + urow(r) + 4 * half) * 32 + l31];
                    S::split(tv ? zz : 0.0f, p[e]);
                }
                const unsigned off = (unsigned)(l31 * (XC * 2) + (ch0 + 8 * g + 4 * half) * 2);
#pragma unroll
                for (int q = 0; q < 2; ++q) {
                    u32x2_t u;
                    u[0] = (unsigned)p[0][q] | ((unsigned)p[1][q] << 16);
                    u[1] = (unsigned)p[2][q] | ((unsigned)p[3][q] << 16);
                    __builtin_amdgcn_raw_buffer_store_b64(u, rz, (int)(off + (unsigned)q * (32u * XC * 2u)), 0, 16);
                }
            }
        }
        asm volatile("s_waitcnt vmcnt(0)" ::: "memory");
        __syncthreads();
        if (tid == 0) __hip_atomic_fetch_add(zcnt + i, 1, __ATOMIC_RELAXED, __HIP_MEMORY_SCOPE_AGENT);
        SX_PHASE(3)
        const unsigned ab2 = (unsigned)(x_n1<S>() * 2 + ((w8 * X_KS2) * 2 + rb) * 2 * 1024);
        sx_preload(A, rw, lane16, ab2);
        float prev[16];
        {
            const rsrc_t rp = make_rsrc(rb == 0 ? ((l & 1) ? a.xb : a.xa) + (int64_t)b * XC * T : a.skip + (int64_t)b * XC * T);
#pragma unroll
            for (int r = 0; r < 16; ++r) prev[r] = buf_load(rp, vo4, (unsigned)(ch0 + urow(r)) * T4);
        }
#pragma unroll
        for (int r = 0; r < 16; ++r) {
            const float blo = bo[urow(r)], bhi = bo[urow(r) + 4];
            const float bias = half ? bhi : blo;
            acc[r] = (rb == 0 ? bias + prev[r] : bias) * s2;
        }
        if (tid == 0) *s_ok = sx_wait(zcnt + i, zcnt + i, zcnt + i, 4 * (l + 1), abort_flag, a.err_flag, !nofence) ? 1 : 0;
        __syncthreads();
        if (__builtin_amdgcn_readfirstlane(*s_ok) == 0) return;
        SX_PHASE(4)
        {
            u32x4_t zv[8];
#pragma unroll
            for (int k = 0; k < 8; ++k)
                zv[k] = nofence ? buf_load_u4_sc1(rz, 16u * (unsigned)tid, 4096u * (unsigned)k) : buf_load_u4(rz, 16u * (unsigned)tid, 4096u * (unsigned)k);
#pragma unroll
            for (int k = 0; k < 8; ++k) {
                const int unit = tid + 256 * k;
                const int q = unit >> 10, fr = (unit >> 5) & 31, part = unit & 31;
                *reinterpret_cast<u32x4_t *>(lds + q * piece_bytes + fr * XR + part * 16) = zv[k];
            }
        }
        __syncthreads();
        SX_PHASE(5)
        sx_gemm<X_KS2>(acc, A, rw, lane16, ab2, lds, piece_bytes, [&](int ks) {
            return (unsigned)(l31 * XR + (ks * 16 + half * 8) * 2);
        });
        SX_PHASE(6)
        if (tv && rb == 0) {
#pragma unroll
            for (int r = 0; r < 16; ++r) buf_store_agent((acc[r] * is2) * RSQRT2, rxout, vo4, (unsigned)(ch0 + urow(r)) * T4);
        } else if (tv) {
            const bool first = l == 0;
#pragma unroll
            for (int r = 0; r < 16; ++r)
                buf_store(first ? acc[r] * is2 : acc[r] * is2 + prev[r], rsk, vo4, (unsigned)(ch0 + urow(r)) * T4);
        }
        asm volatile("s_waitcnt vmcnt(0)" ::: "memory");
        __syncthreads();
        if (tid == 0 && !(l == 0 && i == fault_tile && h == 0))
            __hip_atomic_fetch_add(ready + i, 1, __ATOMIC_RELAXED, __HIP_MEMORY_SCOPE_AGENT);
        SX_PHASE(7)
    }
#undef SX_PHASE
}

}

int set_launch_diffnet_stack_split_x2(const SetDiffnetStackArgs &a, int fault_tile, hipStream_t s) {
    static SetDeviceOnce lds_once;
    if (int rc = set_lds_optin(lds_once, 80 * 1024, "set_diffnet_stack(split x2 attr)", diffnet_stack_split_x2_kernel)) return rc;
    const int tiles = (a.T + 31) / 32, nt = a.B * tiles;
    const int max_dil = 1 << (a.dilation_cycle_length - 1);
    const unsigned piece_bytes = (unsigned)((32 + 2 * max_dil) * XR);
    const size_t ldsz = (size_t)2 * piece_bytes + (64 * 32 + XC) * sizeof(float) + 16;
    SET_HIP(set_zero_async(a.sync_ws, (size_t)(4 + 2 * nt) * sizeof(int32_t), s), "set_diffnet_stack(memset)");
    int n_cu = 0;
    (void)set_cu_count(&n_cu);
    const int extra = (4 * nt + 8 <= n_cu && a.L > 1) ? 8 : 0;
    const int nofence = 1;
    hipLaunchKernelGGL(diffnet_stack_split_x2_kernel, dim3(4 * nt + extra), dim3(256), ldsz, s, a, tiles, nt, piece_bytes, fault_tile, nofence);
    return set_check_launch("set_diffnet_stack");
}

extern "C" int set_debug_x3_phase_buffer(uint64_t *buf) {
    SET_HIP(hipMemcpyToSymbol(HIP_SYMBOL(g_x3_phase_buf), &buf, sizeof(buf)), "set_debug_x3_phase_buffer");
    return SET_OK;
}

extern "C" int64_t set_diffnet_layer_x3_image_size(int32_t mode) {
    return mode == 2 ? x_nimg<SplitF16x2>() : (mode == 3 ? x_nimg<SplitBf16x3>() : -1);
}

extern "C" int set_pack_diffnet_layer_x3(const float *w_dil, const float *w_out, void *img, int32_t mode, int32_t k1, int32_t k2,
                                         void *stream) {
    SET_REQUIRE(w_dil && w_out && img && (mode == 2 || mode == 3), "set_pack_diffnet_layer_x3");
    SET_REQUIRE(k1 >= -60 && k1 <= 60 && k2 >= -60 && k2 <= 60, "set_pack_diffnet_layer_x3(scale exponents)");
    const float s1 = ldexpf(1.0f, k1), s2 = ldexpf(1.0f, k2);
    unsigned short *im = reinterpret_cast<unsigned short *>(img);
    if (mode == 2)
        hipLaunchKernelGGL(pack_layer_x3_kernel<SplitF16x2>, dim3(set_blocks((x_nimg<SplitF16x2>() - 16) / 2, 256)), dim3(256), 0,
                           (hipStream_t)stream, w_dil, w_out, im, s1, s2);
    else
        hipLaunchKernelGGL(pack_layer_x3_kernel<SplitBf16x3>, dim3(set_blocks((x_nimg<SplitBf16x3>() - 8) / 3, 256)), dim3(256), 0,
                           (hipStream_t)stream, w_dil, w_out, im, s1, s2);
    return set_check_launch("set_pack_diffnet_layer_x3");
}

int set_x3_winograd_selected(int x3_mode, int B, int T, int dilation_cycle_length, int n_cu) {
    if (x3_mode != 2 || dilation_cycle_length != 1 || T % 2 != 0) return 0;
    const int64_t tiles64 = (int64_t)B * ((T + 63) / 64);
    bool narrow = 5 * tiles64 < 3 * (int64_t)n_cu;
    if (const char *e = getenv("SET_AMD_X3_TILE")) narrow = atoi(e) == 32;
    if (narrow) return 0;
    if (const char *e = getenv("SET_AMD_X3_WINO")) {
        const int v = atoi(e);
        if (v <= 0) return 0;
        if (v == 2 || v == 3) return v;
    }
    const int64_t tiles96 = ((int64_t)B * ((T + 31) / 32) + 2) / 3;
    return tiles96 >= (int64_t)n_cu ? 3 : 2;
}

int set_launch_diffnet_stack_x3(const SetDiffnetStackArgs &a, int n_cu, int fault_tile, hipStream_t s) {
    SET_REQUIRE(a.x3_mode == 2 || a.x3_mode == 3, "set_diffnet_stack(x3_mode must be 2 = f16x2 or 3 = bf16x3)");
    const int64_t tiles64 = (int64_t)a.B * ((a.T + 63) / 64);
    bool narrow = 5 * tiles64 < 3 * (int64_t)n_cu;
    if (const char *e = getenv("SET_AMD_X3_TILE")) narrow = atoi(e) == 32;
    const bool al8 = ((reinterpret_cast<uintptr_t>(a.condproj) | reinterpret_cast<uintptr_t>(a.xa) | reinterpret_cast<uintptr_t>(a.xb)) & 7) == 0 &&
                     ((a.cp_bs | a.cp_ls) & 1) == 0;
    const int wino = al8 ? set_x3_winograd_selected(a.x3_mode, a.B, a.T, a.dilation_cycle_length, n_cu) : 0;
    if (wino == 3) return launch_x3v<3>(a, n_cu, fault_tile, s);
    if (wino == 2) return launch_x3v<2>(a, n_cu, fault_tile, s);
    if (a.x3_mode == 2)
        return narrow ? launch_x3<SplitF16x2, 1, 1>(a, n_cu, fault_tile, s) : launch_x3<SplitF16x2, 1, 2>(a, n_cu, fault_tile, s);
    return narrow ? launch_x3<SplitBf16x3, 1, 1>(a, n_cu, fault_tile, s) : launch_x3<SplitBf16x3, 1, 2>(a, n_cu, fault_tile, s);
}
```

Measured before the change: 177,100.

## Skip dead residual output in last layer, fold sync clear, stage Winograd input once

In the persistent f32 loop, the last residual layer's x output is never consumed, so the x3v kernel now skips loading the residual input, skips the residual half of the output GEMM, and skips storing x for that layer. The separate sync-workspace zeroing kernel is folded into the boundary kernel, where one block clears the words ahead of the next step. The Winograd input staging now computes all four transformed planes in one pass with a third LDS plane, which drops the second global load of the input tile. These changes cost more LDS and register pressure and add a cross-kernel ordering dependency on the sync workspace.

After: 172,000. 2.9% lower.

```diff
diff --git a/speech-editing-toolkit_amd/csrc/common.h b/speech-editing-toolkit_amd/csrc/common.h
--- a/speech-editing-toolkit_amd/csrc/common.h
+++ b/speech-editing-toolkit_amd/csrc/common.h
@@ -79,6 +79,8 @@
     hipLaunchKernelGGL(set_zero_words_kernel, dim3((unsigned)((words + 255) / 256)), dim3(256), 0, s, reinterpret_cast<unsigned *>(p), words);
     return hipGetLastError();
 }
+constexpr int SET_STACK_DEAD_X = 1;
+constexpr int SET_STACK_SYNC_CLEAR = 2;
 static inline unsigned set_blocks(int64_t n, int per_block) { return (unsigned)((n + per_block - 1) / per_block); }
 
 __device__ __forceinline__ float dev_softplus(float x) { return x > 20.0f ? x : log1pf(expf(x)); }
diff --git a/speech-editing-toolkit_amd/csrc/diffnet.hip b/speech-editing-toolkit_amd/csrc/diffnet.hip
--- a/speech-editing-toolkit_amd/csrc/diffnet.hip
+++ b/speech-editing-toolkit_amd/csrc/diffnet.hip
@@ -988,7 +988,7 @@
     return stack_variant(B, T, dilation_cycle_length, (images & 1) != 0, (images & 2) != 0, x3_mode_of_images(images), n_cu);
 }
 
-int set_launch_diffnet_stack_x3(const SetDiffnetStackArgs &a, int n_cu, int fault_tile, hipStream_t s);
+int set_launch_diffnet_stack_x3(const SetDiffnetStackArgs &a, int n_cu, int fault_tile, int flags, hipStream_t s);
 int set_x3_winograd_selected(int x3_mode, int B, int T, int dilation_cycle_length, int n_cu);
 extern "C" int set_diffnet_stack_x3_winograd(int B, int T, int dilation_cycle_length, int images) {
     int n_cu = 256;
@@ -999,7 +999,7 @@
 }
 int set_launch_diffnet_stack_split_x2(const SetDiffnetStackArgs &a, int fault_tile, hipStream_t s);
 
-extern "C" int set_diffnet_stack(const SetDiffnetStackArgs *args, void *stream) {
+static int diffnet_stack_launch(const SetDiffnetStackArgs *args, int flags, void *stream) {
     SET_REQUIRE(args != nullptr, "set_diffnet_stack");
     const SetDiffnetStackArgs &a = *args;
     SET_REQUIRE(a.xa && a.xb && a.skip && a.condproj && a.dstep && a.w1p_all && a.w2p_all && a.b_dil_all &&
@@ -1019,7 +1019,7 @@
                                       a.w1s_all && a.w2s_all && a.z_ws && plain, (a.wx3_all && plain) ? a.x3_mode : 0, n_cu);
     int fault_tile = -1;
     if (const char *e = getenv("SET_AMD_FAULT_TILE")) fault_tile = atoi(e);
-    if (variant >= 4) return set_launch_diffnet_stack_x3(a, n_cu, fault_tile, s);
+    if (variant >= 4) return set_launch_diffnet_stack_x3(a, n_cu, fault_tile, flags, s);
     if (variant == 3 && a.wx3_all && a.x3_mode == 2 && !split_f32_pinned())
         return set_launch_diffnet_stack_split_x2(a, fault_tile, s);
     if (variant == 3) {
@@ -1072,6 +1072,8 @@
     return set_check_launch("set_diffnet_stack");
 }
 
+extern "C" int set_diffnet_stack(const SetDiffnetStackArgs *args, void *stream) { return diffnet_stack_launch(args, 0, stream); }
+
 namespace {
 __global__ void __launch_bounds__(256) gate_kernel(const float *y, float *z, int B, int C, int T) {
     const int64_t i = (int64_t)blockIdx.x * 256 + threadIdx.x;
@@ -1379,10 +1381,14 @@
     BoundaryArgs g;
     const unsigned short *w_skip_x2, *w_outp_x2, *w_in_x2;
     int32_t *err_flag;
+    int32_t *zero_ws;
+    int zero_words;
 };
 
 __global__ void __launch_bounds__(256, 2) diffnet_boundary_x2_kernel(BoundaryX2Args ax) {
     const BoundaryArgs &a = ax.g;
+    if (ax.zero_ws && blockIdx.x == gridDim.x - 1 && blockIdx.y == gridDim.y - 1)
+        for (int i = threadIdx.x; i < ax.zero_words; i += 256) ax.zero_ws[i] = 0;
     extern __shared__ __attribute__((aligned(16))) unsigned char bl[];
     const int tid = threadIdx.x, lane = tid & 63;
     const int w = __builtin_amdgcn_readfirstlane(tid >> 6);
@@ -1575,7 +1581,7 @@
 }
 
 static int launch_boundary(const SetDiffLoopArgs &a, int Bg, const float *skip, float *x, const float *eps, int sid,
-                           uint64_t quad_offset, float *xin_next, bool x2, hipStream_t s) {
+                           uint64_t quad_offset, float *xin_next, bool x2, int32_t *zero_ws, int zero_words, hipStream_t s) {
     static SetDeviceOnce lds_once;
     if (int rc = set_lds_optin(lds_once, 80 * 1024, "boundary(attr)", diffnet_boundary_kernel, diffnet_boundary_x2_kernel)) return rc;
     BoundaryArgs g = {};
@@ -1591,6 +1597,7 @@
         gx.w_outp_x2 = reinterpret_cast<const unsigned short *>(a.w_outp_x2);
         gx.w_in_x2 = reinterpret_cast<const unsigned short *>(a.w_in_x2);
         gx.err_flag = a.err_flag;
+        gx.zero_ws = zero_ws; gx.zero_words = zero_words;
         hipLaunchKernelGGL(diffnet_boundary_x2_kernel, dim3((a.T + 63) / 64, Bg), dim3(256), (size_t)2 * BX_PIECE, s, gx);
     } else {
         hipLaunchKernelGGL(diffnet_boundary_kernel, dim3((a.T + 63) / 64, Bg), dim3(256), (size_t)DC * BD_LD * sizeof(float), s, g);
@@ -1642,6 +1649,10 @@
     }
     if (bf16_loop && fused_boundary && a.w_skip_x2 && a.w_outp_x2 && a.w_in_x2 && a.M <= 96) boundary_x2 = true;
     if (const char *e = getenv("SET_AMD_BOUNDARY_X2")) boundary_x2 = boundary_x2 && atoi(e) != 0;
+    bool dead_x = a.persistent && !bf16_loop, sync_fold = a.persistent && !bf16_loop && boundary_x2 && sync_ws;
+    if (const char *e = getenv("SET_AMD_STACK_DEAD_X")) dead_x = dead_x && atoi(e) != 0;
+    if (const char *e = getenv("SET_AMD_STACK_SYNC_FOLD")) sync_fold = sync_fold && atoi(e) != 0;
+    const int sync_words = 4 + Bg * ((T + 31) / 32);
     for (int k = 0; k < a.steps && rc == SET_OK; ++k) {
         const int sid = a.steps - 1 - k;
         if (!fused_boundary || k == 0) {
@@ -1664,7 +1675,7 @@
             sa.err_flag = a.err_flag;
             sa.sync_ws = sync_ws;
             sa.B = Bg; sa.T = T; sa.L = L; sa.dilation_cycle_length = a.dilation_cycle_length;
-            rc = set_diffnet_stack(&sa, s);
+            rc = diffnet_stack_launch(&sa, (dead_x ? SET_STACK_DEAD_X : 0) | (sync_fold && k > 0 ? SET_STACK_SYNC_CLEAR : 0), s);
         }
         int fuse = 1;
         if (bf16_loop && a.bf16_ws && a.dilation_cycle_length <= 2) {
@@ -1717,7 +1728,7 @@
         const float *eps = a.noise ? a.noise + (int64_t)k * a.B * per_batch + (int64_t)b0 * per_batch : nullptr;
         if (fused_boundary) {
             rc = launch_boundary(a, Bg, ws_skip, x, eps, sid, (uint64_t)(k + 1) * quads_total + quads_before,
-                                 k + 1 < a.steps ? ws_x0 : nullptr, boundary_x2, s);
+                                 k + 1 < a.steps ? ws_x0 : nullptr, boundary_x2, sync_fold && k + 1 < a.steps ? sync_ws : nullptr, sync_words, s);
             continue;
         }
         SetConv1dArgs cs = conv1x1_args(ws_skip, a.w_skip_p, a.b_skip, ws_h, Bg, DC, DC, T);
diff --git a/speech-editing-toolkit_amd/csrc/diffnet_x3.hip b/speech-editing-toolkit_amd/csrc/diffnet_x3.hip
--- a/speech-editing-toolkit_amd/csrc/diffnet_x3.hip
+++ b/speech-editing-toolkit_amd/csrc/diffnet_x3.hip
@@ -165,6 +165,42 @@
 #pragma unroll
                     for (int q = 0; q < NP; ++q)
                         A[p][u][rb][q] = buf_load_u4(img, lane16, abase + (unsigned)u * ustride + (unsigned)(((kn * 2 + rb) * NP + q) * 1024));
+            __builtin_amdgcn_sched_barrier(0);
+        }
+    }
+}
+
+template <typename S, int NKS, int NCB, int PF, typename BF>
+__device__ __forceinline__ void gemm_x3_skip(f32x16 (&acc)[NCB], rsrc_t img, unsigned lane16, unsigned abase, const unsigned char *lds,
+                                             unsigned piece_bytes, BF bfrag) {
+    constexpr int NP = S::NP;
+    static_assert(NKS % PF == 0, "k-steps must be a multiple of the prefetch distance");
+    u32x4_t A[PF][NP];
+#pragma unroll
+    for (int p = 0; p < PF; ++p)
+#pragma unroll
+        for (int q = 0; q < NP; ++q) A[p][q] = buf_load_u4(img, lane16, abase + (unsigned)(((p * 2 + 1) * NP + q) * 1024));
+    for (int kb = 0; kb < NKS; kb += PF) {
+#pragma unroll
+        for (int p = 0; p < PF; ++p) {
+            const int ks = kb + p;
+            u32x4_t Bv[NCB][NP];
+#pragma unroll
+            for (int cb = 0; cb < NCB; ++cb) {
+                const unsigned bo = bfrag(ks, cb);
+#pragma unroll
+                for (int q = 0; q < NP; ++q) Bv[cb][q] = *reinterpret_cast<const u32x4_t *>(lds + q * piece_bytes + bo);
+            }
+            __builtin_amdgcn_sched_barrier(0);
+            __builtin_amdgcn_s_setprio(1);
+#pragma unroll
+            for (int t = 0; t < S::NPROD; ++t)
+#pragma unroll
+                for (int cb = 0; cb < NCB; ++cb) acc[cb] = S::mma(A[p][S::qa(t)], Bv[cb][S::qb(t)], acc[cb]);
+            __builtin_amdgcn_s_setprio(0);
+            const int kn = min(ks + PF, NKS - 1);
+#pragma unroll
+            for (int q = 0; q < NP; ++q) A[p][q] = buf_load_u4(img, lane16, abase + (unsigned)(((kn * 2 + 1) * NP + q) * 1024));
             __builtin_amdgcn_sched_barrier(0);
         }
     }
@@ -573,7 +609,7 @@
 template <int NB> constexpr unsigned xv_piece() { return 16 * NB * XRV; }
 template <int NB> constexpr unsigned xv_plane() { return 2 * xv_piece<NB>(); }
 template <int NB> constexpr unsigned xv_zpiece() { return 32 * NB * XR; }
-template <int NB> constexpr unsigned xv_tile() { return 2 * xv_plane<NB>() > 2 * xv_zpiece<NB>() ? 2 * xv_plane<NB>() : 2 * xv_zpiece<NB>(); }
+template <int NB> constexpr unsigned xv_tile() { return 3 * xv_plane<NB>() > 2 * xv_zpiece<NB>() ? 3 * xv_plane<NB>() : 2 * xv_zpiece<NB>(); }
 constexpr int XV_PF = 2;
 constexpr int XV_PF2 = 2;
 constexpr int X3V_FLAG_UNIT = 8;
@@ -621,7 +657,7 @@
     }
 }
 
-template <int NB, int PH>
+template <int NB>
 __device__ __forceinline__ void x3v_stage_load(const X3Tile &a, int w, int lane, f32x2 (&x12)[NB][8], float (&xh)[NB][8]) {
     const int l15 = lane & 15, cs = lane >> 4;
     const int ch0 = 32 * w + 8 * cs;
@@ -636,19 +672,17 @@
         const unsigned vox = 4u * (unsigned)min(t, T - 2) + (unsigned)ch0 * T4;
 #pragma unroll
         for (int k = 0; k < 8; ++k) x12[nb][k] = buf_load2(rx, vox, (unsigned)k * T4);
-        if (PH == 1) {
-            const int th = l15 == 0 ? c.t0 - 1 : c.t0 + 32;
-            const unsigned voh = 4u * (unsigned)min(max(th, 0), T - 1) + (unsigned)ch0 * T4;
-            if (edge) {
-#pragma unroll
-                for (int k = 0; k < 8; ++k) xh[nb][k] = buf_load(rx, voh, (unsigned)k * T4);
-            }
-        }
-    }
-}
-template <int NB, int PH>
+        const int th = l15 == 0 ? c.t0 - 1 : c.t0 + 32;
+        const unsigned voh = 4u * (unsigned)min(max(th, 0), T - 1) + (unsigned)ch0 * T4;
+        if (edge) {
+#pragma unroll
+            for (int k = 0; k < 8; ++k) xh[nb][k] = buf_load(rx, voh, (unsigned)k * T4);
+        }
+    }
+}
+template <int NB>
 __device__ __forceinline__ float x3v_stage_store(const X3Tile &a, unsigned char *lds, const float *dsh, int w, int lane, const f32x2 (&x12)[NB][8],
-                                                 const float (&xh)[NB][8]) {
+                                                 const float (&xh)[NB][8], u32x4_t (&v3)[NB][2]) {
     typedef SplitF16x2 S;
     const int l15 = lane & 15, cs = lane >> 4;
     const int ch0 = 32 * w + 8 * cs;
@@ -662,29 +696,26 @@
         const bool v12 = c.ok && t < T, vh = c.ok && edge && th >= 0 && th < T;
         const f32x4 dA = *reinterpret_cast<const f32x4 *>(dsh + nb * XC + ch0);
         const f32x4 dB = *reinterpret_cast<const f32x4 *>(dsh + nb * XC + ch0 + 4);
-        u32x4_t u[2][2];
+        u32x4_t u[4][2];
 #pragma unroll
         for (int e2 = 0; e2 < 4; ++e2) {
-            float V[2][2];
+            float V[4][2];
 #pragma unroll
             for (int h = 0; h < 2; ++h) {
                 const int e = 2 * e2 + h;
                 const float ds = e < 4 ? dA[e & 3] : dB[e & 3];
                 const float d1 = v12 ? x12[nb][e][0] + ds : 0.0f, d2 = v12 ? x12[nb][e][1] + ds : 0.0f;
-                if (PH == 0) {
-                    V[0][h] = d1 + d2;
-                    V[1][h] = d2 - d1;
-                } else {
-                    float d0 = row_prev(d2), d3 = row_next(d1);
-                    const float hv = vh ? xh[nb][e] + ds : 0.0f;
-                    d0 = l15 == 0 ? hv : d0;
-                    d3 = l15 == 15 ? hv : d3;
-                    V[0][h] = d0 - d2;
-                    V[1][h] = d1 - d3;
-                }
-            }
-#pragma unroll
-            for (int j = 0; j < 2; ++j) {
+                float d0 = row_prev(d2), d3 = row_next(d1);
+                const float hv = vh ? xh[nb][e] + ds : 0.0f;
+                d0 = l15 == 0 ? hv : d0;
+                d3 = l15 == 15 ? hv : d3;
+                V[0][h] = d1 + d2;
+                V[1][h] = d2 - d1;
+                V[2][h] = d0 - d2;
+                V[3][h] = d1 - d3;
+            }
+#pragma unroll
+            for (int j = 0; j < 4; ++j) {
                 amax = fmaxf(fmaxf(amax, fabsf(V[j][0])), fabsf(V[j][1]));
                 unsigned pw[2];
                 S::split2(V[j][0], V[j][1], pw);
@@ -693,11 +724,22 @@
             }
         }
 #pragma unroll
-        for (int j = 0; j < 2; ++j)
+        for (int j = 0; j < 3; ++j)
 #pragma unroll
             for (int q = 0; q < 2; ++q) *reinterpret_cast<u32x4_t *>(lds + j * xv_plane<NB>() + q * xv_piece<NB>() + (16 * nb + l15) * XRV + ch0 * 2) = u[j][q];
+        v3[nb][0] = u[3][0];
+        v3[nb][1] = u[3][1];
     }
     return amax;
+}
+template <int NB>
+__device__ __forceinline__ void x3v_stage_store_v3(unsigned char *lds, int slot, int w, int lane, const u32x4_t (&v3)[NB][2]) {
+    const int l15 = lane & 15, cs = lane >> 4;
+    const int ch0 = 32 * w + 8 * cs;
+#pragma unroll
+    for (int nb = 0; nb < NB; ++nb)
+#pragma unroll
+        for (int q = 0; q < 2; ++q) *reinterpret_cast<u32x4_t *>(lds + slot * xv_plane<NB>() + q * xv_piece<NB>() + (16 * nb + l15) * XRV + ch0 * 2) = v3[nb][q];
 }
 
 template <int NB, int PFV>
@@ -734,7 +776,7 @@
 }
 
 template <int NB>
-__device__ __forceinline__ void x3v_main(const X3Tile &a, f32x4 (&PQ)[2][4][NB], unsigned char *lds, uint64_t *dbg, uint64_t &tprev, uint64_t (&ts)[32]) {
+__device__ __forceinline__ void x3v_main(const X3Tile &a, const bool deadx, f32x4 (&PQ)[2][4][NB], unsigned char *lds, uint64_t *dbg, uint64_t &tprev, uint64_t (&ts)[32]) {
 #if SET_X3_PROBE == 2
 #define X3V_PHASE(p)                                  \
     {                                                 \
@@ -778,8 +820,10 @@
     u32x4_t A[PFV][4][2];
     f32x2 x12[NB][8];
     float xh[NB][8];
-    x3v_stage_load<NB, 0>(a, w, lane, x12, xh);
-    float amax = x3v_stage_store<NB, 0>(a, lds, dsh, w, lane, x12, xh);
+    u32x4_t v3[NB][2];
+    x3v_stage_load<NB>(a, w, lane, x12, xh);
+    const float amax = x3v_stage_store<NB>(a, lds, dsh, w, lane, x12, xh, v3);
+    if (!(amax < 32768.0f) && a.err_flag) __hip_atomic_store(a.err_flag, 2, __ATOMIC_RELAXED, __HIP_MEMORY_SCOPE_AGENT);
 #pragma unroll
     for (int p = 0; p < PFV; ++p)
 #pragma unroll
@@ -792,8 +836,6 @@
     x3v_plane<NB, PFV>(PQ[0], A, rw, lane16, abase, 0, lds, boff);
     x3v_plane<NB, PFV>(PQ[1], A, rw, lane16, abase, 1, lds + xv_plane<NB>(), boff);
     X3V_PHASE(2)
-    x3v_stage_load<NB, 1>(a, w, lane, x12, xh);
-    __builtin_amdgcn_sched_barrier(0);
 #pragma unroll
     for (int mb = 0; mb < 4; ++mb)
 #pragma unroll
@@ -806,8 +848,7 @@
             }
     __syncthreads();
     X3V_TS(13)
-    amax = fmaxf(amax, x3v_stage_store<NB, 1>(a, lds, dsh, w, lane, x12, xh));
-    if (!(amax < 32768.0f) && a.err_flag) __hip_atomic_store(a.err_flag, 2, __ATOMIC_RELAXED, __HIP_MEMORY_SCOPE_AGENT);
+    x3v_stage_store_v3<NB>(lds, 0, w, lane, v3);
 #pragma unroll
     for (int p = 0; p < PFV; ++p)
 #pragma unroll
@@ -817,8 +858,8 @@
     X3V_TS(14)
     __syncthreads();
     X3V_PHASE(3)
-    x3v_plane<NB, PFV>(PQ[0], A, rw, lane16, abase, 2, lds, boff);
-    x3v_plane<NB, PFV>(PQ[1], A, rw, lane16, abase, 3, lds + xv_plane<NB>(), boff);
+    x3v_plane<NB, PFV>(PQ[0], A, rw, lane16, abase, 2, lds + 2 * xv_plane<NB>(), boff);
+    x3v_plane<NB, PFV>(PQ[1], A, rw, lane16, abase, 3, lds, boff);
     X3V_PHASE(4)
     bool tv[NB];
     unsigned vo4[NB];
@@ -832,11 +873,13 @@
         ub[cb] = (int64_t)c.b * XC * T;
     }
     float xres[NB][16];
-#pragma unroll
-    for (int cb = 0; cb < NB; ++cb) {
-        const rsrc_t rx = make_rsrc(a.xin + ub[cb]);
-#pragma unroll
-        for (int r = 0; r < 16; ++r) xres[cb][r] = buf_load(rx, vo4[cb], (unsigned)(32 * w + urow(r)) * T4);
+    if (!deadx) {
+#pragma unroll
+        for (int cb = 0; cb < NB; ++cb) {
+            const rsrc_t rx = make_rsrc(a.xin + ub[cb]);
+#pragma unroll
+            for (int r = 0; r < 16; ++r) xres[cb][r] = buf_load(rx, vo4[cb], (unsigned)(32 * w + urow(r)) * T4);
+        }
     }
     __syncthreads();
     X3V_TS(15)
@@ -884,8 +927,12 @@
     X3V_TS(16)
     __syncthreads();
     X3V_PHASE(8)
-    gemm_x3<S, X_KS2, 1, NB, XV_PF2>(acc, rw, lane16, (unsigned)(x_n1<S>() * 2 + w * X_KS2 * 2 * 2 * 1024), (unsigned)(X_KS2 * 2 * 2 * 1024), lds,
-                                     xv_zpiece<NB>(), [&](int ks, int cb) { return (unsigned)((cb * 32 + l31) * XR + (ks * 16 + half * 8) * 2); });
+    const auto zfrag = [&](int ks, int cb) { return (unsigned)((cb * 32 + l31) * XR + (ks * 16 + half * 8) * 2); };
+    if (deadx)
+        gemm_x3_skip<S, X_KS2, NB, XV_PF2>(acc[0][1], rw, lane16, (unsigned)(x_n1<S>() * 2 + w * X_KS2 * 2 * 2 * 1024), lds, xv_zpiece<NB>(), zfrag);
+    else
+        gemm_x3<S, X_KS2, 1, NB, XV_PF2>(acc, rw, lane16, (unsigned)(x_n1<S>() * 2 + w * X_KS2 * 2 * 2 * 1024), (unsigned)(X_KS2 * 2 * 2 * 1024), lds,
+                                         xv_zpiece<NB>(), zfrag);
     X3V_PHASE(9)
     const bool first = a.first != 0;
     float sk[NB][16];
@@ -897,12 +944,14 @@
             for (int r = 0; r < 16; ++r) sk[cb][r] = buf_load_nt(rsk, vo4[cb], (unsigned)(32 * w + urow(r)) * T4);
         }
     }
-#pragma unroll
-    for (int cb = 0; cb < NB; ++cb) {
-        if (tv[cb]) {
-            const rsrc_t rxo = make_rsrc(a.xout + ub[cb]);
-#pragma unroll
-            for (int r = 0; r < 16; ++r) buf_store_agent((acc[0][0][cb][r] * is2) * RSQRT2, rxo, vo4[cb], (unsigned)(32 * w + urow(r)) * T4);
+    if (!deadx) {
+#pragma unroll
+        for (int cb = 0; cb < NB; ++cb) {
+            if (tv[cb]) {
+                const rsrc_t rxo = make_rsrc(a.xout + ub[cb]);
+#pragma unroll
+                for (int r = 0; r < 16; ++r) buf_store_agent((acc[0][0][cb][r] * is2) * RSQRT2, rxo, vo4[cb], (unsigned)(32 * w + urow(r)) * T4);
+            }
         }
     }
     X3V_TS(17)
@@ -934,7 +983,7 @@
 #define X3V_KTS(p)
 #endif
 template <int NB>
-__global__ void __launch_bounds__(512, 1) diffnet_stack_x3v_kernel(SetDiffnetStackArgs a, int ntiles, int ntasks, int fault_tile) {
+__global__ void __launch_bounds__(512, 1) diffnet_stack_x3v_kernel(SetDiffnetStackArgs a, int ntiles, int ntasks, int fault_tile, int dead_x) {
     typedef SplitF16x2 S;
     extern __shared__ __attribute__((aligned(16))) unsigned char lds[];
     int *s_task = reinterpret_cast<int *>(lds + xv_tile<NB>() + NB * XC * sizeof(float));
@@ -1025,7 +1074,7 @@
         }
         const int n_next = __builtin_amdgcn_readfirstlane(s_task[0]);
         X3V_KTS(4)
-        x3v_main<NB>(lt, PQ, lds, dbg, tprev, ts);
+        x3v_main<NB>(lt, dead_x && l == a.L - 1, PQ, lds, dbg, tprev, ts);
 #if SET_X3_PROBE == 2
         if (++n_mine == X3V_TL_TASK && (tid == 0 || tid == 448) && g_x3_phase_buf) {
             const rsrc_t rt = make_rsrc(g_x3_phase_buf);
@@ -1055,7 +1104,7 @@
 }
 
 template <int NB>
-int launch_x3v(const SetDiffnetStackArgs &a, int n_cu, int fault_tile, hipStream_t s) {
+int launch_x3v(const SetDiffnetStackArgs &a, int n_cu, int fault_tile, int flags, hipStream_t s) {
     static SetDeviceOnce lds_once;
     if (int rc = set_lds_optin(lds_once, 160 * 1024, "set_diffnet_stack(x3v attr)", diffnet_stack_x3v_kernel<NB>)) return rc;
     const int Q = a.B * ((a.T + 31) / 32);
@@ -1065,13 +1114,15 @@
     SET_REQUIRE((int64_t)2 * XC * a.T * 4 < ((int64_t)1 << 31), "set_diffnet_stack(split-operand kernel: T too large)");
     SET_REQUIRE(a.dilation_cycle_length == 1 && a.T % 2 == 0, "set_diffnet_stack(x3v: dilation 1 and even T only)");
     const size_t ldsz = (size_t)xv_tile<NB>() + NB * XC * sizeof(float) + 16;
-    SET_HIP(set_zero_async(a.sync_ws, (size_t)(4 + ntiles) * sizeof(int32_t), s), "set_diffnet_stack(memset)");
+    if (!(flags & SET_STACK_SYNC_CLEAR))
+        SET_HIP(set_zero_async(a.sync_ws, (size_t)(4 + ntiles) * sizeof(int32_t), s), "set_diffnet_stack(memset)");
     int grid = n_cu;
     if (NB == 2 && grid > ntiles * 4 / 5) grid = ntiles * 4 / 5;
     if (const char *e = getenv("SET_AMD_STACK_GRID")) grid = atoi(e) > 0 ? atoi(e) : grid;
     if ((int64_t)grid > ntasks64) grid = (int)ntasks64;
     if (grid < 1) grid = 1;
-    hipLaunchKernelGGL(diffnet_stack_x3v_kernel<NB>, dim3(grid), dim3(512), ldsz, s, a, ntiles, (int)ntasks64, fault_tile);
+    hipLaunchKernelGGL(diffnet_stack_x3v_kernel<NB>, dim3(grid), dim3(512), ldsz, s, a, ntiles, (int)ntasks64, fault_tile,
+                       (flags & SET_STACK_DEAD_X) ? 1 : 0);
     return set_check_launch("set_diffnet_stack");
 }
 
@@ -1414,7 +1465,7 @@
     return tiles96 >= (int64_t)n_cu ? 3 : 2;
 }
 
-int set_launch_diffnet_stack_x3(const SetDiffnetStackArgs &a, int n_cu, int fault_tile, hipStream_t s) {
+int set_launch_diffnet_stack_x3(const SetDiffnetStackArgs &a, int n_cu, int fault_tile, int flags, hipStream_t s) {
     SET_REQUIRE(a.x3_mode == 2 || a.x3_mode == 3, "set_diffnet_stack(x3_mode must be 2 = f16x2 or 3 = bf16x3)");
     const int64_t tiles64 = (int64_t)a.B * ((a.T + 63) / 64);
     bool narrow = 5 * tiles64 < 3 * (int64_t)n_cu;
@@ -1422,8 +1473,8 @@
     const bool al8 = ((reinterpret_cast<uintptr_t>(a.condproj) | reinterpret_cast<uintptr_t>(a.xa) | reinterpret_cast<uintptr_t>(a.xb)) & 7) == 0 &&
                      ((a.cp_bs | a.cp_ls) & 1) == 0;
     const int wino = al8 ? set_x3_winograd_selected(a.x3_mode, a.B, a.T, a.dilation_cycle_length, n_cu) : 0;
-    if (wino == 3) return launch_x3v<3>(a, n_cu, fault_tile, s);
-    if (wino == 2) return launch_x3v<2>(a, n_cu, fault_tile, s);
+    if (wino == 3) return launch_x3v<3>(a, n_cu, fault_tile, flags, s);
+    if (wino == 2) return launch_x3v<2>(a, n_cu, fault_tile, flags, s);
     if (a.x3_mode == 2)
         return narrow ? launch_x3<SplitF16x2, 1, 1>(a, n_cu, fault_tile, s) : launch_x3<SplitF16x2, 1, 2>(a, n_cu, fault_tile, s);
     return narrow ? launch_x3<SplitBf16x3, 1, 1>(a, n_cu, fault_tile, s) : launch_x3<SplitBf16x3, 1, 2>(a, n_cu, fault_tile, s);
```
